# geobacter-rs/rav1e

Hardware: AMD Instinct MI355X
Metric: encoded frames/sec + Mpixels/sec, 4K 8-bit speed=10, 1/2/4/8 GPU vs host CPU (higher is better)
Workload: dtype u8

## Files before the change

### include/rav1e_hip.h

```cpp
#ifndef RAV1E_HIP_H
#define RAV1E_HIP_H

#include <stddef.h>
#include <stdint.h>

#ifdef __cplusplus
extern "C" {
#endif

#define RV_OK 0
#define RV_EINVAL (-1)
#define RV_EHIP (-2)
#define RV_ENOTSUP (-3)

typedef enum rv_cpu_feature_level {
  RV_CPU_NATIVE = 0,
  RV_CPU_SSE2 = 1,
  RV_CPU_SSSE3 = 2,
  RV_CPU_AVX2 = 3,
  RV_CPU_HIP = 4,
  RV_CPU_LEVELS = 5
} rv_cpu_feature_level;

int rv_cpu_feature_level_default(void);
// ... 293 lines not shown
} rv_fs_result;

typedef struct rv_mv_blk {
  int8_t ref[2];
  uint8_t n4_w, n4_h, newmv, pad[3];
  rv_mv mv[2];
} rv_mv_blk;
typedef struct rv_mv_cand {
  rv_mv this_mv, comp_mv;
  uint32_t weight;
} rv_mv_cand;
typedef struct rv_mvref_tile {
  int32_t cols, rows, mi_x, mi_y;
} rv_mvref_tile;
typedef struct rv_mvref_geom {
  int32_t n_tiles, grid_w, grid_h, frame_cols, frame_rows;
  uint32_t sign_bias;
} rv_mvref_geom;
typedef struct rv_mvref_query {
  int32_t tile, bx, by, bw4, bh4, ref[2], reserved;
} rv_mvref_query;
typedef struct rv_mvref_result {
  int32_t mode_context, n;
  rv_mv_cand stack[9];
} rv_mvref_result;
size_t rv_mvref_paint_scratch_bytes(rv_mvref_geom geom);
int rv_mvref_grid_paint(const rv_ec_mode_job *d_jobs, int n, rv_mvref_geom geom,
                        const rv_mvref_tile *d_tiles, rv_mv_blk *d_grid, void *d_scratch,
                        uint32_t *d_status, void *stream);
int rv_find_mvrefs_batch(const rv_mvref_query *d_queries, int n, rv_mvref_geom geom,
                         const rv_mvref_tile *d_tiles, const rv_mv_blk *d_grid,
                         rv_mvref_result *d_results, uint32_t *d_status, void *stream);
int rv_ec_mode_fill_stacks(rv_ec_mode_job *d_jobs, int n, rv_mvref_geom geom,
                           const rv_mvref_tile *d_tiles, const rv_mv_blk *d_grid,
                           rv_mvref_result *d_stacks, uint32_t *d_status, void *stream);

size_t rv_propagate_importances_scratch(int w_imp, int h_imp);
int rv_propagate_importances(const rv_plane *org, const rv_plane *ref, const rv_mv *d_mvs,
                             const uint32_t *d_intra_costs, const float *d_importances,
                             int n_unique, float *d_ref_importances, void *d_scratch,
                             size_t scratch_bytes, void *stream);
int rv_full_search_batch(const rv_plane *org, const rv_plane *ref,
                         const rv_fs_job *d_jobs, int n, int blk_w,
                         int blk_h, int step, int allow_hp,
                         rv_fs_result *d_out, void *stream);

int rv_plane_box_sums(const rv_plane *p, uint32_t *d_box, void *stream);

int rv_full_search_sea_batch(const rv_plane *org, const rv_plane *ref,
                             const uint32_t *d_ref_box, const rv_fs_job *d_jobs,
                             int n, int allow_hp, rv_fs_result *d_out,
                             void *stream);

#define RV_DS_MAX_PRED 17
#define RV_MAX_REFS 8
typedef struct rv_ds_job {
  int32_t po_x, po_y;
  int32_t mvx_min, mvx_max;
  int32_t mvy_min, mvy_max;
  rv_mv pmv[2];
  uint32_t lambda;
  int32_t n_pred;
  rv_mv pred[RV_DS_MAX_PRED];
} rv_ds_job;
int rv_diamond_search_batch(const rv_plane *org, const rv_plane *ref,
                            const rv_ds_job *d_jobs, int n, int blk_w,
                            int blk_h, int subpixel, int use_satd,
                            int allow_hp, int bit_depth,
                            rv_fs_result *d_out, void *stream);

int rv_telescopic_subpel_batch(const rv_plane *org, const rv_plane *ref,
                               const rv_ds_job *d_jobs,
                               const rv_fs_result *d_start, int n, int blk_w,
                               int blk_h, int use_satd, int allow_hp,
                               int bit_depth, rv_fs_result *d_out,
                               void *stream);

typedef struct rv_replay_cfg {
  int32_t width, height;
  int32_t xdec, ydec;
  int32_t bit_depth;
  int32_t tile_x0, tile_y0;
  int32_t tile_w, tile_h;
  int32_t n_refs;
  int32_t tile_w_sb, tile_h_sb;
  int32_t n_inputs;
  int32_t flags;
} rv_replay_cfg;
#define RV_REPLAY_EXHAUSTIVE_FS 4
#define RV_REPLAY_SPEED6 8
#define RV_REPLAY_DEBLOCK 16
#define RV_REPLAY_CDEF 32
#define RV_REPLAY_NO_INTRA 64
#define RV_REPLAY_ENTROPY 128
#define RV_REPLAY_MVREF_STANDIN 256
#define RV_REPLAY_LRF 512
typedef struct rv_replay_frame_info {
  int32_t display;
  int32_t me_range_scale;
  int32_t level;
  int32_t is_key;
  int32_t ref_display[2];
  int32_t compound;
} rv_replay_frame_info;
typedef struct rv_replay_level_params {
  int32_t base_q_idx;
  int32_t dc_delta_q[3];
  int32_t ac_delta_q[3];
  int32_t cdef_strengths;
  double lambda, me_lambda;
  double dist_scale[3];
} rv_replay_level_params;
typedef struct rv_replay rv_replay;
rv_replay *rv_replay_create(const rv_replay_cfg *cfg, void *stream);
void rv_replay_destroy(rv_replay *r);
rv_replay *rv_replay_create_twin(rv_replay *primary, void *stream);
int rv_replay_seek(rv_replay *r, long n);
void *rv_replay_stream(rv_replay *r);
int rv_replay_set_level_params(rv_replay *r, int level, const rv_replay_level_params *p);
int rv_replay_synth_inputs(rv_replay *r, int t0);
int rv_replay_set_input(rv_replay *r, int idx, const void *host_yuv);
int rv_replay_get_input(rv_replay *r, int idx, void *host_yuv);
int rv_replay_get_recon(rv_replay *r, int display, void *host_yuv);
int rv_replay_set_importances(rv_replay *r, const float *host, int n);
int rv_replay_set_imp_window(rv_replay *r, int window, long limit);
int rv_replay_set_inputs_ready(rv_replay *r, long displays);
typedef struct rv_la_hub rv_la_hub;
rv_la_hub *rv_la_hub_create(int n_groups);
void rv_la_hub_destroy(rv_la_hub *hub);
int rv_replay_set_la_exchange(rv_replay *r, void *comm, rv_la_hub *hub);
int rv_replay_get_importances(rv_replay *r, float *host, int n);
int rv_replay_frame(rv_replay *r, rv_replay_frame_info *info);
int rv_replay_set_groups(rv_replay *r, int n_groups, const int32_t *rects, int my_group,
                         void *comm);
int rv_replay_exchange_buffers(rv_replay *r, void **send, void **recv, size_t *bytes_per_group);
int rv_replay_import(rv_replay *r);
int rv_comm_unique_id(uint8_t *out, int cap);
void *rv_comm_create(const uint8_t *id, int nranks, int rank);
void rv_comm_destroy(void *comm);
int rv_replay_results(rv_replay *r, uint64_t *host_out, int cap);
int rv_replay_entropy_stats(rv_replay *r, uint64_t *out, int cap);
int rv_replay_set_timing(rv_replay *r, int stride, int block);
int rv_replay_stage_times(rv_replay *r, float *ms_out, int cap);
int rv_replay_stage_times_sum(rv_replay *r, int last_frames, float *ms_out,
                              int cap);
int rv_replay_set_kernel_probe(rv_replay *r, int on);
int rv_round_ring_slots(uint32_t q, int32_t *out, int cap);
int rv_replay_lrf_units(rv_replay *r, int plane, int8_t *out, int cap);
int rv_replay_la_refs(long m, int R, int32_t *out);
int rv_replay_kernel_probe(rv_replay *r, double *out, int cap);
int rv_ds_phase_dump(void);
int rv_rdo_phase_dump(void);
int rv_replay_counters(rv_replay *r, uint64_t *out, int cap);

int rv_replay_dpb_slots(void);


void rv_shims_release(void);
void rv_shims_shutdown(void);

#define RV_DIST_SIZES(X) \
  X(4, 4) X(4, 8) X(8, 4) X(8, 8) X(8, 16) X(16, 8) X(16, 16) X(16, 32) \
  X(32, 16) X(32, 32) X(32, 64) X(64, 32) X(64, 64) X(64, 128) X(128, 64) \
  X(128, 128) X(4, 16) X(16, 4) X(8, 32) X(32, 8) X(16, 64) X(64, 16)

#define RV_DECL_DIST(W, H)                                                   \
  uint32_t rav1e_sad##W##x##H##_hip(const uint8_t *src, ptrdiff_t src_stride, \
                                    const uint8_t *dst, ptrdiff_t dst_stride); \
  uint32_t rav1e_sad##W##x##H##_hbd_hip(const uint16_t *src,                  \
                                        ptrdiff_t src_stride,                 \
                                        const uint16_t *dst,                  \
                                        ptrdiff_t dst_stride);                \
  uint32_t rav1e_satd_##W##x##H##_hip(const uint8_t *src,                     \
                                      ptrdiff_t src_stride,                   \
                                      const uint8_t *dst,                     \
                                      ptrdiff_t dst_stride);                  \
  uint32_t rav1e_satd_##W##x##H##_hbd_hip(const uint16_t *src,                \
                                          ptrdiff_t src_stride,               \
                                          const uint16_t *dst,                \
                                          ptrdiff_t dst_stride);
RV_DIST_SIZES(RV_DECL_DIST)
#undef RV_DECL_DIST

#define RV_FILTER_PAIRS(X)                                                  \
  X(regular, regular, 0, 0) X(smooth, regular, 1, 0)                       \
  X(sharp, regular, 2, 0) X(bilinear, regular, 3, 0)                       \
  X(regular, smooth, 0, 1) X(smooth, smooth, 1, 1) X(sharp, smooth, 2, 1)  \
  X(bilinear, smooth, 3, 1) X(regular, sharp, 0, 2) X(smooth, sharp, 1, 2) \
  X(sharp, sharp, 2, 2) X(bilinear, sharp, 3, 2)                           \
  X(regular, bilinear, 0, 3) X(smooth, bilinear, 1, 3)                     \
  X(sharp, bilinear, 2, 3) X(bilinear, bilinear, 3, 3)

#define RV_DECL_MC(NX, NY, MX, MY)                                            \
  void rav1e_put_8tap_##NX##_##NY##_hip(                                      \
      uint8_t *dst, ptrdiff_t dst_stride, const uint8_t *src,                 \
      ptrdiff_t src_stride, int32_t w, int32_t h, int32_t mx, int32_t my);    \
  void rav1e_put_8tap_##NX##_##NY##_16bpc_hip(                                \
      uint16_t *dst, ptrdiff_t dst_stride, const uint16_t *src,               \
      ptrdiff_t src_stride, int32_t w, int32_t h, int32_t mx, int32_t my,     \
      int32_t bit_depth);                                                     \
  void rav1e_prep_8tap_##NX##_##NY##_hip(int16_t *tmp, const uint8_t *src,    \
                                         ptrdiff_t src_stride, int32_t w,     \
                                         int32_t h, int32_t mx, int32_t my);  \
  void rav1e_prep_8tap_##NX##_##NY##_16bpc_hip(                               \
      int16_t *tmp, const uint16_t *src, ptrdiff_t src_stride, int32_t w,     \
      int32_t h, int32_t mx, int32_t my, int32_t bit_depth);
RV_FILTER_PAIRS(RV_DECL_MC)
#undef RV_DECL_MC

void rav1e_avg_hip(uint8_t *dst, ptrdiff_t dst_stride, const int16_t *tmp1,
                   const int16_t *tmp2, int32_t w, int32_t h);
void rav1e_avg_16bpc_hip(uint16_t *dst, ptrdiff_t dst_stride,
                         const int16_t *tmp1, const int16_t *tmp2, int32_t w,
                         int32_t h, int32_t bit_depth);

int rav1e_fwd_txfm_hip(const int16_t *residual, int32_t *coeffs,
                       int32_t tx_size, int32_t tx_type, int32_t bit_depth);
int rav1e_inv_txfm_add_hip(const int32_t *coeffs, void *dst,
                           ptrdiff_t dst_stride, int32_t tx_size,
                           int32_t tx_type, int32_t bit_depth);

typedef uint32_t (*rv_dist_fn)(const void *src, ptrdiff_t src_stride,
                               const void *dst, ptrdiff_t dst_stride);
rv_dist_fn rv_sad_fn(int cpu_level, int bsize, int hbd);
rv_dist_fn rv_satd_fn(int cpu_level, int bsize, int hbd);
typedef void (*rv_put_fn)(void *dst, ptrdiff_t dst_stride, const void *src,
                          ptrdiff_t src_stride, int32_t w, int32_t h,
                          int32_t mx, int32_t my);
rv_put_fn rv_put_fn_get(int cpu_level, int mode_x, int mode_y);

#ifdef __cplusplus
}
#endif
#endif
```

### rav1e_amd/__init__.py

```python
from __future__ import annotations

import ctypes as C
import enum
import os

import numpy as np

_ROOT = os.path.dirname(os.path.abspath(__file__))
LIB_PATH = os.environ.get("RAV1E_HIP_LIB") or os.path.join(_ROOT, "lib", "librav1e_hip.so")
HEADER_PATH = os.path.join(os.path.dirname(_ROOT), "include", "rav1e_hip.h")

RV_OK, RV_EINVAL, RV_EHIP, RV_ENOTSUP = 0, -1, -2, -3


class Rav1eHipError(RuntimeError):
    pass


class RvPlane(C.Structure):
    _fields_ = [("data", C.c_void_p), ("stride", C.c_int32),
                ("alloc_height", C.c_int32), ("width", C.c_int32),
                ("height", C.c_int32), ("xorigin", C.c_int32),
                ("yorigin", C.c_int32), ("xdec", C.c_int32),
                ("ydec", C.c_int32), ("hbd", C.c_int32),
# ... 130 lines not shown
        return int(self.name.split("_")[1].split("X")[0])

    def height(self) -> int:
        return int(self.name.split("X")[-1])


class TxType(enum.IntEnum):
    DCT_DCT = 0
    ADST_DCT = 1
    DCT_ADST = 2
    ADST_ADST = 3
    FLIPADST_DCT = 4
    DCT_FLIPADST = 5
    FLIPADST_FLIPADST = 6
    ADST_FLIPADST = 7
    FLIPADST_ADST = 8
    IDTX = 9
    V_DCT = 10
    H_DCT = 11
    V_ADST = 12
    H_ADST = 13
    V_FLIPADST = 14
    H_FLIPADST = 15


class FilterMode(enum.IntEnum):
    REGULAR = 0
    SMOOTH = 1
    SHARP = 2
    BILINEAR = 3


_lib = None


class RvEcModeParams(C.Structure):
    _fields_ = [(n, C.c_int32) for n in ("frame_type", "reference_mode", "force_integer_mv",
                                         "allow_high_precision_mv", "seg_enabled",
                                         "last_active_segid")]


class RvMvrefGeom(C.Structure):
    _fields_ = [(n, C.c_int32) for n in ("n_tiles", "grid_w", "grid_h", "frame_cols",
                                         "frame_rows")] + [("sign_bias", C.c_uint32)]


def _declare(L):
    vp, i32, sz = C.c_void_p, C.c_int, C.c_size_t
    P = C.POINTER(RvPlane)
    sig = {
        "rv_cpu_feature_level_default": (i32, []),
        "rv_cpu_feature_level_index": (i32, [i32]),
        "rv_device_count": (i32, []),
        "rv_set_device": (i32, [i32]),
        "rv_last_error": (C.c_char_p, []),
        "rv_version": (C.c_char_p, []),
        "rv_malloc": (vp, [sz]),
        "rv_free": (None, [vp]),
        "rv_host_alloc": (vp, [sz]),
        "rv_host_free": (None, [vp]),
        "rv_memcpy_h2d": (i32, [vp, vp, sz, vp]),
        "rv_memcpy_d2h": (i32, [vp, vp, sz, vp]),
        "rv_memcpy_d2d": (i32, [vp, vp, sz, vp]),
        "rv_memset": (i32, [vp, i32, sz, vp]),
        "rv_stream_create": (vp, []),
        "rv_stream_create_priority": (vp, [i32]),
        "rv_stream_destroy": (i32, [vp]),
        "rv_stream_sync": (i32, [vp]),
        "rv_device_sync": (i32, []),
        "rv_trace_marker": (i32, [vp]),
        "rv_event_create": (vp, []),
        "rv_event_destroy": (i32, [vp]),
        "rv_event_record": (i32, [vp, vp]),
        "rv_event_sync": (i32, [vp]),
        "rv_stream_wait_event": (i32, [vp, vp]),
        "rv_event_elapsed_ms": (C.c_float, [vp, vp]),
        "rv_plane_geometry": (sz, [P, i32, i32, i32, i32, i32, i32, i32]),
        "rv_plane_pad": (i32, [P, vp]),
        "rv_plane_downsample": (i32, [P, P, vp]),
        "rv_sad_batch": (i32, [P, P, vp, i32, i32, i32, vp, vp]),
        "rv_satd_batch": (i32, [P, P, vp, i32, i32, i32, vp, vp]),
        "rv_sse_batch": (i32, [P, P, vp, i32, i32, i32, vp, vp]),
        "rv_lookahead_intra_costs": (i32, [P, i32, vp, vp]),
        "rv_propagate_importances_scratch": (sz, [i32, i32]),
        "rv_propagate_importances": (i32, [P, P, vp, vp, vp, i32, vp, vp, sz, vp]),
        "rv_cdef_moments_batch": (i32, [P, P, vp, i32, i32, i32, vp, vp]),
        "rv_put_8tap_batch": (i32, [P, P, vp, i32, i32, i32, i32, i32, i32, vp]),
        "rv_predict_intra_batch": (i32, [P, vp, vp, i32, i32, i32, vp]),
        "rv_intra_edges_batch": (i32, [P, vp, i32, vp, i32, i32, i32, i32, i32, vp, vp]),
        "rv_intra_screen_batch": (i32, [P, P, vp, i32, vp, i32, i32, i32, vp, i32, i32, vp, vp, vp,
                                        vp]),
        "rv_cfl_luma_ac_batch": (i32, [P, vp, i32, i32, i32, i32, vp, vp]),
        "rv_predict_cfl_batch": (i32, [P, vp, vp, vp, vp, i32, i32, i32, vp]),
        "rv_cfl_alpha_search_batch": (i32, [P, P, vp, i32, i32, i32, vp, vp, vp]),
        "rv_frame_delta_batch": (i32, [P, i32, i32, vp, i32, vp, vp]),
        "rv_deblock_plane": (i32, [P, i32, i32, i32, vp, vp, i32, vp, i32, vp]),
        "rv_deblock_fast_level": (i32, [i32, i32, i32]),
        "rv_deblock_sse": (i32, [P, P, i32, i32, vp, vp, i32, vp, vp, i32, vp]),
        "rv_deblock_frame": (i32, [P, i32, i32, vp, vp, i32, vp, i32, vp]),
        "rv_cdef_find_dirs": (i32, [P, i32, i32, vp, i32, vp, vp, i32, vp]),
        "rv_lrf_stripe_filter": (i32, [P, P] + [i32] * 10 + [vp, vp]),
        "rv_y4m_parse_header": (i32, [C.c_char_p, vp]),
        "rv_y4m_open": (vp, [C.c_char_p]),
        "rv_y4m_get_info": (i32, [vp, vp]),
        "rv_y4m_frame_bytes": (sz, [vp]),
        "rv_y4m_read_frame": (i32, [vp, vp]),
        "rv_y4m_close": (None, [vp]),
        "rv_ivf_create": (vp, [C.c_char_p, i32, i32, i32, i32]),
        "rv_ivf_write_frame": (i32, [vp, C.c_uint64, vp, sz]),
        "rv_ivf_close": (i32, [vp]),
        "rv_cdef_filter_plane": (i32, [P, P, i32, i32, i32, vp, i32, vp, vp, vp, vp, vp, i32, i32,
                                       vp]),
        "rv_prep_8tap_batch": (i32, [vp, P, vp, i32, i32, i32, i32, i32, i32, vp]),
        "rv_mc_avg_batch": (i32, [P, vp, vp, vp, i32, i32, i32, i32, vp]),
        "rv_mc_dist_batch": (i32, [P, P, vp, i32, i32, i32, i32, i32, i32, i32, vp, vp]),
        "rv_fwd_txfm_batch": (i32, [vp, vp, i32, i32, i32, i32, vp]),
        "rv_diff_fwd_txfm_batch": (i32, [P, P, vp, i32, i32, i32, i32, vp, vp]),
        "rv_inv_txfm_add_batch": (i32, [vp, P, vp, i32, i32, i32, i32, vp]),
        "rv_quantize_batch": (i32, [vp, i32, i32, i32, i32, i32, i32, i32, i32, i32, vp, vp, vp,
                                    vp]),
        "rv_dequantize_batch": (i32, [vp, i32, i32, i32, i32, i32, i32, vp, vp]),
        "rv_estimate_rate_batch": (i32, [vp, i32, i32, i32, vp, vp]),
        "rv_full_search_batch": (i32, [P, P, vp, i32, i32, i32, i32, i32, vp, vp]),
        "rv_full_search_sea_batch": (i32, [P, P, vp, vp, i32, i32, vp, vp]),
        "rv_plane_box_sums": (i32, [P, vp, vp]),
        "rv_replay_create": (vp, [C.POINTER(RvReplayCfg), vp]),
        "rv_replay_create_twin": (vp, [vp, vp]),
        "rv_replay_seek": (i32, [vp, C.c_long]),
        "rv_replay_stream": (vp, [vp]),
        "rv_replay_destroy": (None, [vp]),
        "rv_q_lookup": (i32, [i32, i32, i32]),
        "rv_replay_synth_inputs": (i32, [vp, i32]),
        "rv_replay_set_level_params": (i32, [vp, i32, C.POINTER(RvReplayLevelParams)]),
        "rv_replay_set_input": (i32, [vp, i32, vp]),
        "rv_replay_get_input": (i32, [vp, i32, vp]),
        "rv_replay_get_recon": (i32, [vp, i32, vp]),
        "rv_replay_set_importances": (i32, [vp, vp, i32]),
        "rv_replay_set_imp_window": (i32, [vp, i32, C.c_long]),
        "rv_replay_set_inputs_ready": (i32, [vp, C.c_long]),
        "rv_replay_get_importances": (i32, [vp, vp, i32]),
        "rv_replay_frame": (i32, [vp, C.POINTER(RvReplayFrameInfo)]),
        "rv_replay_set_groups": (i32, [vp, i32, vp, i32, vp]),
        "rv_replay_exchange_buffers": (i32, [vp, C.POINTER(C.c_void_p), C.POINTER(C.c_void_p),
                                             C.POINTER(C.c_size_t)]),
        "rv_replay_import": (i32, [vp]),
        "rv_comm_unique_id": (i32, [vp, i32]),
        "rv_comm_create": (vp, [vp, i32, i32]),
        "rv_comm_destroy": (None, [vp]),
        "rv_replay_results": (i32, [vp, vp, i32]),
        "rv_replay_entropy_stats": (i32, [vp, vp, i32]),
        "rv_replay_stage_times": (i32, [vp, vp, i32]),
        "rv_replay_stage_times_sum": (i32, [vp, i32, vp, i32]),
        "rv_replay_counters": (i32, [vp, vp, i32]),
        "rv_replay_dpb_slots": (i32, []),
        "rv_replay_set_kernel_probe": (i32, [vp, i32]),
        "rv_replay_kernel_probe": (i32, [vp, vp, i32]),
        "rv_round_ring_slots": (i32, [C.c_uint32, vp, i32]),
        "rv_replay_lrf_units": (i32, [vp, i32, vp, i32]),
        "rv_replay_la_refs": (i32, [C.c_long, i32, vp]),
        "rv_la_hub_create": (vp, [i32]),
        "rv_la_hub_destroy": (None, [vp]),
        "rv_replay_set_la_exchange": (i32, [vp, vp, vp]),
        "rv_replay_set_timing": (i32, [vp, i32, i32]),
        "rv_diamond_search_batch": (i32, [P, P, vp, i32, i32, i32, i32, i32, i32, i32, vp, vp]),
        "rv_telescopic_subpel_batch": (i32, [P, P, vp, vp, i32, i32, i32, i32, i32, i32, vp, vp]),
        "rv_tx_dist_batch": (i32, [vp, i32, vp, i32, i32, vp, vp]),
        "rav1e_fwd_txfm_hip": (i32, [vp, vp, i32, i32, i32]),
        "rav1e_inv_txfm_add_hip": (i32, [vp, vp, C.c_ssize_t, i32, i32, i32]),
        "rv_ec_scratch_bytes": (C.c_size_t, [i32]),
        "rv_ec_tokenize": (i32, [vp, i32, i32, i32, i32, i32, i32, vp, vp, vp, vp, C.c_uint32, vp,
                                 vp]),
        "rv_ec_code_tokens": (C.c_long, [vp, C.c_size_t, vp, vp, C.c_size_t]),
        "rv_ec_count_tokens": (C.c_long, [vp, C.c_size_t, vp, vp]),
        "rv_ec_rate_batch": (i32, [vp, vp, vp, i32, vp, i32, vp, vp, vp, vp, vp]),
        "rv_ec_cdf_total": (i32, []),
        "rv_ec_default_cdf": (i32, [i32, vp]),
        "rv_ec_reset_counts": (None, [vp]),
        "rv_ec_mode_scratch_bytes": (C.c_size_t, [i32]),
        "rv_ec_mode_tokenize": (i32, [vp, i32, RvEcModeParams, i32, vp, i32, i32, vp, vp, vp, vp,
                                      C.c_uint32, vp, vp]),
        "rv_ec_code_stream": (C.c_long, [vp, C.c_size_t, vp, vp, C.c_size_t]),
        "rv_ec_count_stream": (C.c_long, [vp, C.c_size_t, vp, vp]),
        "rv_ec_cdf_total_all": (i32, []),
        "rv_ec_default_cdf_all": (i32, [i32, vp]),
        "rv_ec_reset_counts_all": (None, [vp]),
        "rv_ec_partition_gather": (i32, [vp, i32]),
        "rv_ec_rate_stream_batch": (i32, [vp, vp, vp, i32, vp, i32, vp, vp, vp, vp, vp]),
        "rv_ec_rate_stream_batch_waves": (i32, [vp, vp, vp, i32, vp, i32, vp, vp, vp, vp, i32, vp]),
        "rv_ec_cand_scratch_bytes": (C.c_size_t, [i32, i32]),
        "rv_ec_cand_tokenize": (i32, [vp, i32, vp, i32, vp, i32, RvEcModeParams, i32, vp, i32, i32,
                                      i32, i32, vp, i32, i32, vp, vp, vp, vp, C.c_uint32, vp, vp]),
        "rv_ec_cand_rates": (i32, [vp, i32, vp, i32, vp, i32, RvEcModeParams, i32, vp, i32, i32,
                                   i32, i32, vp, i32, i32, vp, vp, vp, vp, C.c_uint32, vp, i32, vp,
                                   vp, vp, vp, vp]),
        "rv_mvref_paint_scratch_bytes": (C.c_size_t, [RvMvrefGeom]),
        "rv_mvref_grid_paint": (i32, [vp, i32, RvMvrefGeom, vp, vp, vp, vp, vp]),
        "rv_find_mvrefs_batch": (i32, [vp, i32, RvMvrefGeom, vp, vp, vp, vp, vp]),
        "rv_ec_mode_fill_stacks": (i32, [vp, i32, RvMvrefGeom, vp, vp, vp, vp, vp]),
        "rv_sad_fn": (vp, [i32, i32, i32]),
        "rv_satd_fn": (vp, [i32, i32, i32]),
        "rv_put_fn_get": (vp, [i32, i32, i32]),
    }
    for name, (res, args) in sig.items():
        f = getattr(L, name)
        f.restype = res
        f.argtypes = args


def lib():
    global _lib
    if _lib is None:
        if not os.path.exists(LIB_PATH):
            raise Rav1eHipError(
                f"{LIB_PATH} missing: run `python -c 'import __graft_entry__ as g; g.build()'`")
        L = C.CDLL(LIB_PATH, mode=C.RTLD_GLOBAL)
        _declare(L)
        _lib = L
    return _lib


def _check(rc, what):
    if rc != RV_OK:
        raise Rav1eHipError(f"{what} failed ({rc}): {lib().rv_last_error().decode()}")


def require_device(device: int = 0):
    L = lib()
    if L.rv_device_count() <= device:
        raise Rav1eHipError("no HIP device visible: the HIP level needs a gfx950 GPU")
    _check(L.rv_set_device(device), "rv_set_device")


class DeviceBuffer:

    def __init__(self, nbytes: int):
        self.nbytes = int(nbytes)
        self.ptr = lib().rv_malloc(max(1, self.nbytes))
        if not self.ptr:
            raise Rav1eHipError(f"rv_malloc({nbytes}): {lib().rv_last_error().decode()}")

    @classmethod
    def from_array(cls, a: np.ndarray) -> "DeviceBuffer":
        a = np.ascontiguousarray(a)
        b = cls(a.nbytes)
        b.upload(a)
        return b

    def upload(self, a: np.ndarray, stream=None):
        a = np.ascontiguousarray(a)
        assert a.nbytes <= self.nbytes
        if a.nbytes:
            _check(lib().rv_memcpy_h2d(self.ptr, a.ctypes.data, a.nbytes, stream), "rv_memcpy_h2d")

    def download(self, dtype, count=None, stream=None) -> np.ndarray:
        dt = np.dtype(dtype)
        n = self.nbytes // dt.itemsize if count is None else int(count)
        out = np.empty(n, dtype=dt)
        if out.nbytes:
            _check(lib().rv_memcpy_d2h(out.ctypes.data, self.ptr, out.nbytes, stream),
                   "rv_memcpy_d2h")
        return out

    def zero(self, stream=None):
        _check(lib().rv_memset(self.ptr, 0, self.nbytes, stream), "rv_memset")
        _check(lib().rv_stream_sync(stream), "rv_stream_sync")

    def free(self):
        if self.ptr:
            lib().rv_free(self.ptr)
            self.ptr = None

    def __del__(self):
        try:
            self.free()
        except Exception:
            pass


class DevicePlane:

    def __init__(self, width, height, xdec=0, ydec=0, xpad=0, ypad=0, hbd=False,
                 bit_depth=None):
        self.desc = RvPlane()
        nbytes = lib().rv_plane_geometry(C.byref(self.desc), width, height, xdec, ydec,
                                         xpad, ypad, 1 if hbd else 0)
        if bit_depth is not None:
            self.desc.bit_depth = int(bit_depth)
        self.buf = DeviceBuffer(nbytes)
        self.desc.data = self.buf.ptr
        self.dtype = np.uint16 if hbd else np.uint8

    @classmethod
    def from_array(cls, a: np.ndarray, xpad=0, ypad=0, xdec=0, ydec=0, pad=True,
                   bit_depth=None):
        p = cls(a.shape[1], a.shape[0], xdec, ydec, xpad, ypad, a.dtype == np.uint16,
                bit_depth)
        p.upload_visible(a, pad=pad)
        return p

    @classmethod
    def from_full(cls, full: np.ndarray, xorigin, yorigin, width, height, bit_depth=None):
        p = cls.__new__(cls)
        p.desc = RvPlane()
        p.desc.stride, p.desc.alloc_height = full.shape[1], full.shape[0]
        p.desc.width, p.desc.height = width, height
        p.desc.xorigin, p.desc.yorigin = xorigin, yorigin
# ... 1846 lines not shown
```

### rav1e_amd/csrc/rv_rdo.h

```cpp
#pragma once

#include "rv_chain.h"
#include "rv_device.h"
#include "rv_quant.h"

namespace rv {

struct RdoPlane {
  rv_plane org;
  rv_plane ref[2];
  rv_plane dst;
  int32_t *levels;
  uint64_t *out;
  QCtx q;
};

struct RdoWinner {
  int32_t c;
  int32_t skip;
  double cost;
  uint64_t dist;
};

struct RdoArgs {
  RdoPlane p[2];
  CandGeo g;
  const rv_fs_result *sub;
  const RdoWinner *win;
  const float *imp;
  int w_in_b, h_in_b, w_imp;
  int n_tx;
  int cand_base;
  const int32_t *list;
  const int32_t *count;
  int commit;
  int ntx_per_cand;
  int bd;
  int bsize;
  int mb_w, mb_h;
  int sub_w, sub_h;
  int xdec, ydec;
  int q_tx_index;
  int tx_size, qindex;
  const void *iedges;
  const uint8_t *imodes;
  const uint8_t *iwin;
};

}

int rv_quant_ctx(int qindex, int tx_area, int is_intra, int bit_depth, int dc_delta_q,
                 int ac_delta_q, rv::QCtx *out);

int rv_rdo_candidates(const rv::RdoArgs &luma, const rv::RdoArgs &chroma, int hbd,
                      hipStream_t s, bool compound = false);

int rv_rdo_blocks2(const rv::RdoArgs &l, const rv::RdoArgs &c, int nl, int nc, int hbd,
                   hipStream_t s, int mode);
int rv_rdo_blocks(const rv::RdoArgs &a, bool luma, int nplanes, int n_tx_size, int hbd,
                  hipStream_t s, int mode);

int rv_rdo_args_put(const rv::RdoArgs *h, int n, rv::RdoArgs *dev, hipStream_t s);
int rv_rdo_candidates_list(const rv::RdoArgs *h, const rv::RdoArgs *dev, int nsets, int mode_a,
                           int hbd, hipStream_t s, int max_grid = 0, uint32_t *kp_cnt = nullptr,
                           unsigned long long *kp_t = nullptr);

int rv_rdo_intra(const rv::RdoArgs &luma, const rv::RdoArgs &chroma, int hbd, hipStream_t s);
```

### rav1e_amd/csrc/rv_rdo.hip

```cpp
#include <stdio.h>
#include <stdlib.h>
#include <string.h>

#include <type_traits>

#include "rv_distortion.h"
#include "rv_intra.h"
#include "rv_rdo.h"
#include "rv_tx.h"

namespace rv {


__constant__ int8_t kRdoReg[2][16][8] = {
    {{0, 0, 0, 127, 0, 0, 0, 0}, {0, 2, -6, 126, 8, -2, 0, 0},
     {0, 2, -10, 122, 18, -4, 0, 0}, {0, 2, -12, 116, 28, -8, 2, 0},
     {0, 2, -14, 110, 38, -10, 2, 0}, {0, 2, -14, 102, 48, -12, 2, 0},
     {0, 2, -16, 94, 58, -12, 2, 0}, {0, 2, -14, 84, 66, -12, 2, 0},
     {0, 2, -14, 76, 76, -14, 2, 0}, {0, 2, -12, 66, 84, -14, 2, 0},
     {0, 2, -12, 58, 94, -16, 2, 0}, {0, 2, -12, 48, 102, -14, 2, 0},
     {0, 2, -10, 38, 110, -14, 2, 0}, {0, 2, -8, 28, 116, -12, 2, 0},
     {0, 0, -4, 18, 122, -10, 2, 0}, {0, 0, -2, 8, 126, -6, 2, 0}},
    {{0, 0, 0, 127, 0, 0, 0, 0}, {0, 0, -4, 126, 8, -2, 0, 0},
     {0, 0, -8, 122, 18, -4, 0, 0}, {0, 0, -10, 116, 28, -6, 0, 0},
// ... 59 lines not shown
    mode = (kc & 1) ? 0 : a.imodes[sb * 4 + 1 + (kc >> 1)];
    j.oi = sb * 6 + kc;
  }
  const int sx = sb % a.g.tw, sy = sb / a.g.tw;
  const int fx = a.g.tx0 + sx, fy = a.g.ty0 + sy;
  const int tsx = fx % a.g.tws, tsy = fy % a.g.ths;
  j.ivar = tsx == 0 && tsy == 0 ? 0 : tsy == 0 ? 1 : tsx == 0 ? 2 : 3;
  j.imode = mode;
  j.iedge = (const uint8_t *)a.iedges + ((size_t)sb * 3 + plane) * kIntraEdge * sizeof(Px);
  j.bx = (fx * a.bsize) >> a.xdec;
  j.by = (fy * a.bsize) >> a.ydec;
  j.ox = j.oy = 0;
  j.src_x = j.src_y = j.cf = j.rf = j.ref = 0;
  j.src2_x = j.src2_y = j.cf2 = j.rf2 = 0;
  j.comp = false;
  j.zero = false;
  return j;
}

template <typename Px, int N, int G>
__device__ __forceinline__ void intra_fill(const RdoJob &jb, int32_t *e, Px *pred, int bd, int lane) {
  const Px *eg = (const Px *)jb.iedge;
  for (int i = lane; i < kIntraEdge; i += G) e[i] = eg[i];
  wave_sync();
  IntraSetup st = intra_setup(jb.imode, jb.ivar);
  if (st.mode == 0) st.dcv = intra_dc<G>(e, jb.ivar, N, N, bd, lane);
  const int maxv = (1 << bd) - 1;
  for (int i = lane; i < N * N; i += G) {
    const int r = i / N, c = i - r * N;
    pred[i] = (Px)intra_px(st, e, N, N, r, c, maxv);
  }
  wave_sync();
}

__device__ __forceinline__ int rdo_ntx(const RdoArgs &a) {
  return a.count ? __builtin_amdgcn_readfirstlane(*a.count) * a.ntx_per_cand : a.n_tx;
}

template <int N>
__device__ __forceinline__ RdoJob rdo_job(const RdoArgs &a, const RdoPlane &pl, int t) {
  const int ci = t / a.ntx_per_cand, sub = t - ci * a.ntx_per_cand;
  const int cand = a.list ? a.list[ci] : a.cand_base + ci;
  int sb, c;
  RdoJob j;
  j.zero = false;
  j.oi = cand * a.ntx_per_cand + sub;
  if (a.commit) {
    sb = cand;
    c = a.win[sb].c;
    j.zero = a.win[sb].skip != 0;
  } else {
    c = cand / a.g.nsb;
    sb = cand - c * a.g.nsb;
  }
  rv_mv mv, mv1{0, 0};
  j.comp = c >= a.g.R * a.g.M;
  if (j.comp) {
    comp_mvs(a.g, a.sub, sb, c - a.g.R * a.g.M, &mv, &mv1);
    j.ref = 0;
  } else {
    (void)cand_mv(a.g, a.sub, sb, c, &mv);
    j.ref = c / a.g.M;
  }
  const int sx = sb % a.g.tw, sy = sb / a.g.tw;
  j.bx = ((a.g.tx0 + sx) * a.bsize) >> a.xdec;
  j.by = ((a.g.ty0 + sy) * a.bsize) >> a.ydec;
  const int txc = a.mb_w / N;
  j.ox = (sub % txc) * N;
  j.oy = (sub / txc) * N;
  const rv_mc_job m = mc_job_for(pl.ref[j.ref], j.bx, j.by, mv, 0, 0);
  j.src_x = m.src_x;
  j.src_y = m.src_y;
  j.cf = m.col_frac;
  j.rf = m.row_frac;
  j.src2_x = j.src2_y = j.cf2 = j.rf2 = 0;
  if (j.comp) {
    const rv_mc_job m1 = mc_job_for(pl.ref[1], j.bx, j.by, mv1, 0, 0);
    j.src2_x = m1.src_x;
    j.src2_y = m1.src_y;
    j.cf2 = m1.col_frac;
    j.rf2 = m1.row_frac;
  }
  return j;
}

struct McF {
  uint32_t xp[3];
  int xsum;
  int yt[8];
  int cf, rf;
};
template <typename Px>
__device__ __forceinline__ McF mc_setup(int cf, int rf, int w, int h) {
  McF f;
  f.cf = cf;
  f.rf = rf;
  const int8_t *xf = kRdoReg[w <= 4][cf];
  const int8_t *yf = kRdoReg[h <= 4][rf];
#pragma unroll
  for (int k = 0; k < 8; k++) f.yt[k] = yf[k];
  f.xsum = 0;
  if constexpr (sizeof(Px) == 1) {
#pragma unroll
    for (int q = 0; q < 2; q++)
      f.xp[q] = (uint32_t)(uint8_t)xf[4 * q] | ((uint32_t)(uint8_t)xf[4 * q + 1] << 8) |
                ((uint32_t)(uint8_t)xf[4 * q + 2] << 16) | ((uint32_t)(uint8_t)xf[4 * q + 3] << 24);
#pragma unroll
    for (int k = 0; k < 8; k++) f.xsum += xf[k];
    f.xp[2] = 0;
  } else {
#pragma unroll
    for (int q = 0; q < 3; q++)
      f.xp[q] = (uint32_t)(uint16_t)(int16_t)xf[2 * q + 1] |
                ((uint32_t)(uint16_t)(int16_t)xf[2 * q + 2] << 16);
  }
  return f;
}
template <typename Px>
__device__ __forceinline__ int32_t mc_h(const McF &f, const uint32_t *row, int col, int ib) {
  if constexpr (sizeof(Px) == 1) {
    const int d0 = col >> 2, sh = col & 3;
    const uint32_t w0 = row[d0], w1 = row[d0 + 1], w2 = row[d0 + 2];
    const uint32_t lo = __builtin_amdgcn_alignbyte(w1, w0, sh);
    const uint32_t hi = __builtin_amdgcn_alignbyte(w2, w1, sh);
    if (!f.cf) return (int32_t)((lo >> 24) ^ 0x80u);
    int32_t s = dot4_i8(lo, f.xp[0], 128 * f.xsum);
    s = dot4_i8(hi, f.xp[1], s);
    return (int32_t)(int16_t)round_shift(s, 7 - ib);
  } else {
    const int c1 = col + 1, d0 = c1 >> 1, sh = (c1 & 1) * 2;
    uint32_t w[4];
#pragma unroll
    for (int k = 0; k < 4; k++) w[k] = row[d0 + k];
    uint32_t pp[3];
#pragma unroll
    for (int k = 0; k < 3; k++) pp[k] = __builtin_amdgcn_alignbyte(w[k + 1], w[k], sh);
    if (!f.cf) return (int32_t)(pp[1] & 0xffffu);
    int32_t s = 0;
#pragma unroll
    for (int k = 0; k < 3; k++) s = dot2_i16(pp[k], f.xp[k], s);
    return (int32_t)(int16_t)round_shift(s, 7 - ib);
  }
}
__device__ __forceinline__ int32_t mc_prep_v(const McF &f, const int32_t *ring, int u, int ib) {
  if (f.rf) {
    int32_t s = 0;
#pragma unroll
    for (int k = 1; k < 7; k++) s += __mul24(f.yt[k], ring[(u + k) & 7]);
    return round_shift(s, f.cf ? 7 : 7 - ib);
  }
  return f.cf ? ring[(u + 3) & 7] : ring[(u + 3) & 7] << ib;
}

template <typename Px, int N, int RB>
__device__ __forceinline__ void mc_compound(const RdoArgs &a, const RdoPlane &pl, const RdoJob &jb,
                                            uint32_t *win, Px *pred) {
  constexpr int B = (int)sizeof(Px);
  constexpr int P = B == 1 ? ((N + 8 + 15) / 16) * 16 : ((2 * (N + 8) + 15) / 16) * 16;
  constexpr int kRowDw = ((N + 7) * B + 3) / 4, kTot = (RB + 7) * kRowDw;
  static_assert((RB % 8 == 0 || RB < 8) && N % RB == 0, "bands of whole 8-row groups");
  constexpr int U = RB < 8 ? RB : 8;
  const int col = rv_tid() & (N - 1);
  const int ib = a.bd == 12 ? 2 : 4, maxv = (1 << a.bd) - 1;
  const McF f0 = mc_setup<Px>(jb.cf, jb.rf, a.mb_w, a.mb_h);
  const McF f1 = mc_setup<Px>(jb.cf2, jb.rf2, a.mb_w, a.mb_h);
  uint32_t *w0 = win, *w1 = win + (RB + 7) * (P / 4);
  const uint8_t *sp0 = (const uint8_t *)plane_ptr<Px>(pl.ref[0], jb.src_x + jb.ox - 3, jb.src_y + jb.oy - 3);
  const uint8_t *sp1 =
      (const uint8_t *)plane_ptr<Px>(pl.ref[1], jb.src2_x + jb.ox - 3, jb.src2_y + jb.oy - 3);
  const int64_t rs0 = (int64_t)pl.ref[0].stride * B, rs1 = (int64_t)pl.ref[1].stride * B;
#pragma unroll 1
  for (int band = 0; band < N / RB; band++) {
    if (band) wave_sync();
#pragma unroll 2
    for (int i = col; i < kTot; i += N) {
      const int r = i / kRowDw, d = i - r * kRowDw;
      uint32_t v0, v1;
      __builtin_memcpy(&v0, sp0 + (band * RB + r) * rs0 + 4 * d, 4);
      __builtin_memcpy(&v1, sp1 + (band * RB + r) * rs1 + 4 * d, 4);
      w0[r * (P / 4) + d] = B == 1 ? v0 ^ 0x80808080u : v0;
      w1[r * (P / 4) + d] = B == 1 ? v1 ^ 0x80808080u : v1;
    }
    wave_sync();
    int32_t g0[8], g1[8];
#pragma unroll
    for (int k = 1; k < 6; k++) {
      g0[k] = mc_h<Px>(f0, w0 + k * (P / 4), col, ib);
      g1[k] = mc_h<Px>(f1, w1 + k * (P / 4), col, ib);
    }
    g0[0] = g0[6] = g0[7] = g1[0] = g1[6] = g1[7] = 0;
#pragma unroll 1
    for (int r0 = 0; r0 < RB; r0 += U) {
#pragma unroll
      for (int u = 0; u < U; u++) {
        const int r = r0 + u;
        g0[(u + 6) & 7] = mc_h<Px>(f0, w0 + (r + 6) * (P / 4), col, ib);
        g1[(u + 6) & 7] = mc_h<Px>(f1, w1 + (r + 6) * (P / 4), col, ib);
        const int32_t t = mc_prep_v(f0, g0, u, ib) + mc_prep_v(f1, g1, u, ib);
        pred[(band * RB + r) * N + col] = (Px)clamp_med3(round_shift(t, ib + 1), 0, maxv);
      }
    }
  }
  wave_sync();
}

__device__ __forceinline__ double rdo_bias(const RdoArgs &a, int mi_x, int mi_y, int m = 2) {
  return distortion_bias(a.imp, a.w_imp, a.w_in_b, a.h_in_b, mi_x, mi_y, m);
}

template <typename Px>
__device__ __forceinline__ uint64_t rdo_cdef_8x8(const Px *o, int64_t os, const Px *d, int dp,
                                                 int bd) {
  int32_t ss = 0, sd = 0;
  uint32_t ss2 = 0, sd2 = 0, ssd = 0;
#pragma unroll
  for (int j = 0; j < 8; j++)
#pragma unroll
    for (int i = 0; i < 8; i++) {
      const int32_t s = o[(int64_t)j * os + i];
      const int32_t e = d[j * dp + i];
      ss += s;
      sd += e;
      ss2 += (uint32_t)wmul24(s, s);
      sd2 += (uint32_t)wmul24(e, e);
      ssd += (uint32_t)wmul24(s, e);
    }
  return cdef_dist_finish(ss, sd, ss2, sd2, ssd, bd);
}

template <typename Px, int N, int LPB>
__device__ __forceinline__ uint64_t rdo_sse_biased(const RdoArgs &a, const RdoJob &j, const Px *o,
                                                   int64_t os, const Px *d) {
  const int bw = a.sub_w, bh = a.sub_h, nbx = N / bw, nby = N / bh;
  const int lane = rv_tid() & (LPB - 1);
  uint64_t acc = 0;
  for (int k = lane; k < nbx * nby; k += LPB) {
    const int by = k / nbx, bx = k - by * nbx;
    uint64_t value = 0;
    for (int jj = 0; jj < bh; jj++) {
      uint32_t row = 0;
      for (int i = 0; i < bw; i++) {
        const int32_t c = (int32_t)(int16_t)o[(int64_t)(by * bh + jj) * os + bx * bw + i] -
                          (int32_t)(int16_t)d[(by * bh + jj) * N + bx * bw + i];
        row += (uint32_t)wmul24(c, c);
      }
      value += row;
    }
    const int px = j.bx + j.ox + bx * bw, py = j.by + j.oy + by * bh;
    acc += distortion_biased(
        value, rdo_bias(a, (px << a.xdec) >> 2, (py << a.ydec) >> 2, (N < 8 ? N : 8) / 4));
  }
  return acc;
}

template <typename Px, int N, int LPB, bool LUMA>
__device__ __forceinline__ uint64_t rdo_dist_biased(const RdoArgs &a, const RdoJob &j, const Px *o,
                                                    int64_t os, const Px *d) {
  if constexpr (LUMA) {
    constexpr int NB = N / 8, ROWS = NB * NB * 8;
    static_assert(LPB % 8 == 0 && ROWS % LPB == 0, "rows of 8x8 blocks over the lanes");
    const int lane = rv_tid() & (LPB - 1);
    uint64_t acc = 0;
#pragma unroll
    for (int k0 = 0; k0 < ROWS; k0 += LPB) {
      const int k = k0 + lane, blk = k >> 3, row = k & 7;
      const int by = blk / NB, bx = blk - by * NB;
      const Px *op = o + (int64_t)(by * 8 + row) * os + bx * 8;
      const Px *dp = d + (by * 8 + row) * N + bx * 8;
      int32_t ss = 0, sd = 0;
      uint32_t ss2 = 0, sd2 = 0, ssd = 0;
#pragma unroll
      for (int i = 0; i < 8; i++) {
        const int32_t sv = op[i], e = dp[i];
        ss += sv;
        sd += e;
        ss2 += (uint32_t)wmul24(sv, sv);
        sd2 += (uint32_t)wmul24(e, e);
        ssd += (uint32_t)wmul24(sv, e);
      }
#pragma unroll
      for (int m = 1; m < 8; m <<= 1) {
        ss += __shfl_xor(ss, m, 64);
        sd += __shfl_xor(sd, m, 64);
        ss2 += __shfl_xor(ss2, m, 64);
        sd2 += __shfl_xor(sd2, m, 64);
        ssd += __shfl_xor(ssd, m, 64);
      }
      if (row == 0) {
        const uint64_t v = cdef_dist_finish(ss, sd, ss2, sd2, ssd, a.bd);
        const int px = j.bx + j.ox + bx * 8, py = j.by + j.oy + by * 8;
        acc += distortion_biased(v, rdo_bias(a, px >> 2, py >> 2));
      }
    }
    return acc;
  } else {
    return rdo_sse_biased<Px, N, LPB>(a, j, o, os, d);
  }
}

template <typename Px, int N>
__host__ __device__ constexpr int rdo_slab_bytes() {
  constexpr int B = (int)sizeof(Px);
  constexpr int P = B == 1 ? ((N + 8 + 15) / 16) * 16 : ((2 * (N + 8) + 15) / 16) * 16;
  constexpr int RB = N < 16 ? N : 16;
  constexpr int a = N * (N + 1) * 4, b = (N + 7) * P, c = 2 * (RB + 7) * P;
  return ((a > b ? a : b) > c ? (a > b ? a : b) : c);
}

template <typename Px, int N, int LPB, int MODE, bool LUMA = false>
__device__ __forceinline__ void rdo_cand_body(const RdoArgs &a, const RdoPlane &pl, int t,
                                              bool valid, int32_t *buf, Px *pred,
                                              const uint16_t *scan) {
  constexpr int B = (int)sizeof(Px);
  constexpr int S = N + 1;
  constexpr int G = LPB / N, RG = N / G;
  constexpr int U = RG < 8 ? RG : 8;
  constexpr int P = B == 1 ? ((N + 8 + 15) / 16) * 16 : ((2 * (N + 8) + 15) / 16) * 16;
  constexpr int C32 = N < 32 ? N : 32;
  static_assert(!LUMA || N >= 8, "cdef distortion runs on 8x8 blocks");
  const int lane = rv_tid() & (LPB - 1);
  RdoJob jb;
  if constexpr (MODE == 3)
    jb = rdo_job_intra<Px, N>(a, &pl == &a.p[1] ? 2 : 1, t);
  else
    jb = rdo_job<N>(a, pl, t);
  const rv_plane &ref = pl.ref[jb.ref];
  const int ox = jb.ox, oy = jb.oy;
  const int bd = a.bd, ib = bd == 12 ? 2 : 4, maxv = (1 << bd) - 1;
  const int sx0 = jb.bx + ox, sy0 = jb.by + oy;
  auto wave_sync = [] {
    __builtin_amdgcn_fence(__ATOMIC_RELEASE, "wavefront");
    __builtin_amdgcn_wave_barrier();
    __builtin_amdgcn_fence(__ATOMIC_ACQUIRE, "wavefront");
  };

  if constexpr (MODE == 3) {
    intra_fill<Px, N, LPB>(jb, buf, pred, a.bd, lane);
  } else if (MODE == 1 || (MODE == 2 && jb.comp)) {
    static_assert(2 * (16 + 7) * (sizeof(Px) == 1 ? 48 : 80) <= N * (N + 1) * 4 || N != 32,
                  "compound windows must fit the coefficient slab");
    mc_compound<Px, N, (N < 16 ? N : 16)>(a, pl, jb, reinterpret_cast<uint32_t *>(buf), pred);
  } else
  {
    uint32_t *win = reinterpret_cast<uint32_t *>(buf);
    const uint8_t *sp = (const uint8_t *)plane_ptr<Px>(ref, jb.src_x + ox - 3, jb.src_y + oy - 3);
    const int64_t rs = (int64_t)ref.stride * B;
    constexpr int kRowDw = ((N + 7) * B + 3) / 4;
    constexpr int kTot = (N + 7) * kRowDw;
#pragma unroll 4
    for (int i = lane; i < kTot; i += LPB) {
      const int r = i / kRowDw, d = i - r * kRowDw;
      uint32_t v;
// ... 77 lines not shown
      }
    }
    wave_sync();
  }
  const Px *o = plane_ptr<Px>(pl.org, sx0, sy0);
  const int64_t ost = pl.org.stride;
  if (!a.commit) {
    const uint64_t d = group_sum<LPB>(rdo_dist_biased<Px, N, LPB, LUMA>(a, jb, o, ost, pred));
    if (valid && lane == 0) pl.out[(int64_t)jb.oi * 3 + 0] = d;
  }

  int s0, s1, s2;
  fwd_shifts<N>((bd - 8) / 2, s0, s1, s2);
  {
    constexpr int PPD = 4 / B;
    constexpr int DPR = N / PPD;
    const uint8_t *op = (const uint8_t *)o;
    const int64_t os = (int64_t)pl.org.stride * B;
#pragma unroll 8
    for (int i = lane; i < N * DPR; i += LPB) {
      const int r = i / DPR, c = (i - r * DPR) * PPD;
      uint32_t ov, pv;
      __builtin_memcpy(&ov, op + r * os + c * B, 4);
      __builtin_memcpy(&pv, pred + r * N + c, 4);
#pragma unroll
      for (int k = 0; k < PPD; k++) {
        const int sh = 8 * B * k, m = B == 1 ? 0xff : 0xffff;
        const int16_t d = (int16_t)((int16_t)((ov >> sh) & m) - (int16_t)((pv >> sh) & m));
        buf[r * S + c + k] = rdo_rsa((int32_t)d, -s0);
      }
    }
    wave_sync();
  }
  if (lane < N) {
    int32_t v[N];
#pragma unroll
    for (int r = 0; r < N; r++) v[r] = buf[r * S + lane];
    tx::fwd1d<1, N>(v, v);
#pragma unroll
    for (int r = 0; r < N; r++) buf[r * S + lane] = rdo_rsa(v[r], -s1);
  }
  wave_sync();
  constexpr int CA = C32 * C32, RR = CA / N;
  if (lane < RR) {
    int32_t v[N];
#pragma unroll
    for (int c = 0; c < N; c++) v[c] = buf[lane * S + c];
    tx::fwd1d<1, N>(v, v);
#pragma unroll
    for (int c = 0; c < N; c++) buf[lane * S + c] = rdo_rsa(v[c], -s2);
  }
  wave_sync();
  uint64_t txd = 0;
  quantize_block<CA, LPB>(
      pl.q, scan, [&](int pos) { return buf[(pos / N) * S + (pos % N)]; },
      [&](int pos, int32_t q, int32_t r) {
        int32_t *e = buf + (pos / N) * S + (pos % N);
        const int32_t dd = wsub(*e, r);
        txd += (uint64_t)(int64_t)wmul(dd, dd);
        *e = jb.zero ? 0 : q;
      });
  wave_sync();
  if (!a.commit) {
    txd = group_sum<LPB>(txd);
    const int bits = 2 * (3 - pl.q.log_tx_scale);
    if (valid && lane == 0)
      pl.out[(int64_t)jb.oi * 3 + 2] =
          q_estimate_rate(a.qindex, a.tx_size, (txd + (1ull << (bits - 1))) >> bits);
  }
  {
    int32_t *pk = pl.levels + (int64_t)jb.oi * CA;
#pragma unroll 4
    for (int i = lane; i < CA; i += LPB) {
      int32_t *e = buf + (i / N) * S + (i % N);
      const int32_t q = *e;
      if (valid && a.commit) pk[i] = q;
      *e = q_dequant(pl.q, q, i);
    }
  }
  wave_sync();
  const int range = bd + 8;
  {
    int32_t v[N];
    if (lane < C32) {
#pragma unroll
      for (int c = 0; c < N; c++) {
        const int i = lane * C32 + c;
        v[c] = c < C32 ? tx::clampv(buf[(i / N) * S + (i % N)], range) : 0;
      }
    }
    wave_sync();
    if (lane < C32) {
      tx::inv1d<1, N>(v, range);
#pragma unroll
      for (int c = 0; c < N; c++) buf[lane * S + c] = v[c];
    }
  }
  wave_sync();
  if (lane < N) {
    const int crange = bd + 6 > 16 ? bd + 6 : 16;
    int32_t v[N];
#pragma unroll
    for (int r = 0; r < N; r++)
      v[r] = r < C32 ? tx::clampv(round_shift(buf[r * S + lane], inv_mid_shift<N>()), crange) : 0;
    tx::inv1d<1, N>(v, crange);
#pragma unroll
    for (int r = 0; r < N; r++) {
      Px *q = pred + r * N + lane;
      *q = (Px)clamp_med3(wadd((int32_t)*q, round_shift(v[r], 4)), 0, maxv);
    }
  }
  wave_sync();
  if (a.commit) {
    constexpr int PPD = 4 / B, DPR = N / PPD;
    uint8_t *dp = (uint8_t *)plane_ptr_mut<Px>(pl.dst, sx0, sy0);
    const int64_t ds = (int64_t)pl.dst.stride * B;
#pragma unroll 8
    for (int i = lane; i < N * DPR; i += LPB) {
      const int r = i / DPR, c = (i - r * DPR) * PPD;
      uint32_t v;
      __builtin_memcpy(&v, pred + r * N + c, 4);
      if (valid) __builtin_memcpy(dp + r * ds + c * B, &v, 4);
    }
    return;
  }
  const uint64_t d = group_sum<LPB>(rdo_dist_biased<Px, N, LPB, LUMA>(a, jb, o, ost, pred));
  if (valid && lane == 0) pl.out[(int64_t)jb.oi * 3 + 1] = d;
}

__host__ __device__ constexpr int cmax(int a, int b) { return a > b ? a : b; }

template <typename Px, typename Mid, int NPART>
struct LumaLds {
  static constexpr int kWinP = sizeof(Px) == 1 ? 80 : 144;
  static constexpr int kWinRows = 64 / NPART + 7;
  static constexpr int kCompRows = sizeof(Px) == 1 ? 16 : 8;
  static constexpr int kScr =
      cmax(cmax(cmax(kWinRows * kWinP, 16 * 65 * 4), 32 * 66 * (int)sizeof(Mid)),
           2 * (kCompRows + 7) * kWinP);
  static constexpr int kSlot = (kScr + 64 * 64 * (int)sizeof(Px) + 15) / 16 * 16;
};


template <typename Px>
__device__ __forceinline__ uint64_t luma_dist(const RdoArgs &a, const RdoJob &j, const Px *o,
                                              int64_t os, const Px *pred) {
  const int lane = rv_tid() & 63, by = lane >> 3, bx = lane & 7;
  const uint64_t v =
      rdo_cdef_8x8<Px>(o + (int64_t)(by * 8) * os + bx * 8, os, pred + by * 8 * 64 + bx * 8, 64, a.bd);
  const int px = j.bx + bx * 8, py = j.by + by * 8;
  return group_sum<64>(distortion_biased(v, rdo_bias(a, px >> 2, py >> 2)));
}

template <typename Px, int NPART, int MODE>
__device__ __forceinline__ void luma_front(const RdoArgs &a, const RdoPlane &pl, int t,
                                           const RdoJob &jb, bool valid, uint8_t *scr, Px *pred,
                                           bool skip_dist = true) {
  constexpr int N = 64, B = (int)sizeof(Px);
  constexpr int P = LumaLds<Px, int16_t, NPART>::kWinP;
  constexpr int RP = N / NPART;
  static_assert(RP % 8 == 0, "MC rows run in groups of 8");
  const int lane = rv_tid() & 63;
  const rv_plane &ref = pl.ref[jb.ref];
  const int ox = 0, oy = 0;
  const int bd = a.bd, ib = bd == 12 ? 2 : 4, maxv = (1 << bd) - 1;

  if constexpr (MODE == 3) {
    intra_fill<Px, 64, 64>(jb, reinterpret_cast<int32_t *>(scr), pred, bd, lane);
  } else if (MODE == 1 || (MODE == 2 && jb.comp)) {
    mc_compound<Px, 64, LumaLds<Px, int16_t, NPART>::kCompRows>(
        a, pl, jb, reinterpret_cast<uint32_t *>(scr), pred);
  } else
  {
    uint32_t *win = reinterpret_cast<uint32_t *>(scr);
    const int cf = jb.cf, rf = jb.rf;
    const int8_t *xf = kRdoReg[a.mb_w <= 4][cf];
    const int8_t *yf = kRdoReg[a.mb_h <= 4][rf];
    int yt[8];
#pragma unroll
    for (int k = 0; k < 8; k++) yt[k] = yf[k];
    uint32_t xp[4];
    int xsum = 0;
    if constexpr (B == 1) {
#pragma unroll
      for (int h = 0; h < 2; h++)
        xp[h] = (uint32_t)(uint8_t)xf[4 * h] | ((uint32_t)(uint8_t)xf[4 * h + 1] << 8) |
                ((uint32_t)(uint8_t)xf[4 * h + 2] << 16) | ((uint32_t)(uint8_t)xf[4 * h + 3] << 24);
#pragma unroll
      for (int k = 0; k < 8; k++) xsum += xf[k];
      xp[2] = xp[3] = 0;
    } else {
#pragma unroll
      for (int h = 0; h < 3; h++)
        xp[h] = (uint32_t)(uint16_t)(int16_t)xf[2 * h + 1] |
                ((uint32_t)(uint16_t)(int16_t)xf[2 * h + 2] << 16);
      xp[3] = 0;
    }
    const int col = lane;
    auto hval = [&](int tr) __attribute__((always_inline)) -> int32_t {
      const uint32_t *row = win + tr * (P / 4);
      if constexpr (B == 1) {
        const int d0 = col >> 2, sh = col & 3;
        const uint32_t w0 = row[d0], w1 = row[d0 + 1], w2 = row[d0 + 2];
        const uint32_t lo = __builtin_amdgcn_alignbyte(w1, w0, sh);
        const uint32_t hi = __builtin_amdgcn_alignbyte(w2, w1, sh);
        if (!cf) return (int32_t)((lo >> 24) ^ 0x80u);
        int32_t s = dot4_i8(lo, xp[0], 128 * xsum);
        s = dot4_i8(hi, xp[1], s);
        return (int32_t)(int16_t)round_shift(s, 7 - ib);
      } else {
        const int c1 = col + 1, d0 = c1 >> 1, sh = (c1 & 1) * 2;
        uint32_t w[4];
#pragma unroll
        for (int k = 0; k < 4; k++) w[k] = row[d0 + k];
        uint32_t pp[3];
#pragma unroll
        for (int k = 0; k < 3; k++) pp[k] = __builtin_amdgcn_alignbyte(w[k + 1], w[k], sh);
        if (!cf) return (int32_t)(pp[1] & 0xffffu);
        int32_t s = 0;
#pragma unroll
        for (int k = 0; k < 3; k++)
          s = dot2_i16(pp[k], xp[k], s);
        return (int32_t)(int16_t)round_shift(s, 7 - ib);
      }
    };
    const int vshift = cf ? 7 + ib : 7;
    constexpr int kRowDw = ((N + 7) * B + 3) / 4;
    constexpr int kTot = (RP + 7) * kRowDw;
    const int64_t rs = (int64_t)ref.stride * B;
#pragma unroll 1
    for (int half = 0; half < NPART; half++) {
      const uint8_t *sp =
          (const uint8_t *)plane_ptr<Px>(ref, jb.src_x + ox - 3, jb.src_y + oy - 3 + RP * half);
      if (half) wave_sync();
#pragma unroll 4
      for (int i = lane; i < kTot; i += 64) {
        const int r = i / kRowDw, d = i - r * kRowDw;
        uint32_t v;
        __builtin_memcpy(&v, sp + r * rs + 4 * d, 4);
        win[r * (P / 4) + d] = B == 1 ? v ^ 0x80808080u : v;
      }
      wave_sync();
      int32_t ring[8];
#pragma unroll
      for (int k = 1; k < 6; k++) ring[k] = hval(k);
      ring[0] = ring[6] = ring[7] = 0;
#pragma unroll 1
      for (int r0 = 0; r0 < RP; r0 += 8) {
#pragma unroll
        for (int u = 0; u < 8; u++) {
          const int r = r0 + u;
          ring[(u + 6) & 7] = hval(r + 6);
          int32_t v;
          if (rf) {
            int32_t s = 0;
#pragma unroll
            for (int k = 1; k < 7; k++) s += __mul24(yt[k], ring[(u + k) & 7]);
            v = round_shift(s, vshift);
          } else {
            v = cf ? round_shift(ring[(u + 3) & 7], ib) : ring[(u + 3) & 7];
          }
          pred[(RP * half + r) * N + col] = (Px)clamp_med3(v, 0, maxv);
        }
      }
    }
    wave_sync();
  }

  const Px *o = plane_ptr<Px>(pl.org, jb.bx, jb.by);
  if (!a.commit && skip_dist) {
    const uint64_t d = luma_dist<Px>(a, jb, o, pl.org.stride, pred);
    if (valid && lane == 0) pl.out[(int64_t)jb.oi * 3 + 0] = d;
  }
  int s0, s1, s2;
  fwd_shifts<N>((bd - 8) / 2, s0, s1, s2);
  int32_t *fmid = reinterpret_cast<int32_t *>(scr);
  {
    int32_t v[N];
#pragma unroll
    for (int r = 0; r < N; r++) {
      const int16_t d = (int16_t)((int16_t)o[(int64_t)r * pl.org.stride + lane] -
                                  (int16_t)pred[r * N + lane]);
      v[r] = rdo_rsa((int32_t)d, -s0);
    }
    tx::fwd1d<1, N>(v, v);
#pragma unroll
    for (int r = 0; r < 16; r++) fmid[r * 65 + lane] = rdo_rsa(v[r], -s1);
  }
}

__device__ __forceinline__ void luma_fwd_row(int32_t *row, int bd) {
  int s0, s1, s2;
  fwd_shifts<64>((bd - 8) / 2, s0, s1, s2);
  int32_t v[64];
#pragma unroll
  for (int c = 0; c < 64; c++) v[c] = row[c];
  tx::fwd1d<1, 64>(v, v);
#pragma unroll
  for (int c = 0; c < 64; c++) row[c] = rdo_rsa(v[c], -s2);
}

__device__ __forceinline__ void luma_quantize(const RdoArgs &a, const RdoPlane &pl, int t,
                                              const RdoJob &jb, bool valid, int32_t *fmid,
                                              const uint16_t *scan) {
  uint64_t txd = 0;
  quantize_block<1024, 64>(
      pl.q, scan, [&](int pos) { return fmid[(pos >> 6) * 65 + (pos & 63)]; },
      [&](int pos, int32_t q, int32_t r) {
        int32_t *e = fmid + (pos >> 6) * 65 + (pos & 63);
        const int32_t dd = wsub(*e, r);
        txd += (uint64_t)(int64_t)wmul(dd, dd);
        *e = jb.zero ? 0 : q;
      });
  const int lane = rv_tid() & 63;
  if (!a.commit) {
    txd = group_sum<64>(txd);
    const int bits = 2 * (3 - pl.q.log_tx_scale);
    if (valid && lane == 0)
      pl.out[(int64_t)jb.oi * 3 + 2] =
          q_estimate_rate(a.qindex, a.tx_size, (txd + (1ull << (bits - 1))) >> bits);
  }
  wave_sync();
  int32_t *pk = pl.levels + (int64_t)jb.oi * 1024;
#pragma unroll 4
  for (int i = lane; i < 1024; i += 64) {
    int32_t *e = fmid + (i >> 6) * 65 + (i & 63);
    const int32_t q = *e;
    if (a.commit) pk[i] = q;
    *e = q_dequant(pl.q, q, i);
  }
}

__device__ __forceinline__ void luma_inv_row_load(const int32_t *fmid, int rr, int32_t *v,
                                                  int range, int32_t *pk) {
  const int32_t *src = fmid + (rr >> 1) * 65 + (rr & 1) * 32;
#pragma unroll
  for (int c = 0; c < 32; c++) {
    const int32_t x = src[c];
    if (pk) pk[c] = x;
    v[c] = tx::clampv(x, range);
  }
#pragma unroll
  for (int c = 32; c < 64; c++) v[c] = 0;
}
template <typename Mid>
__device__ __forceinline__ void luma_inv_row_tx(int32_t *v, Mid *dst, int range, int crange) {
  tx::inv1d<1, 64>(v, range);
#pragma unroll
  for (int c = 0; c < 64; c++) dst[c] = (Mid)tx::clampv(round_shift(v[c], 2), crange);
}

template <typename Px, typename Mid>
__device__ __forceinline__ void luma_back(const RdoArgs &a, const RdoPlane &pl, int t,
                                          const RdoJob &jb, bool valid, const Mid *imid,
                                          Px *pred) {
  constexpr int N = 64, B = (int)sizeof(Px);
  const int lane = rv_tid() & 63;
  const int bd = a.bd, maxv = (1 << bd) - 1;
  const int crange = bd + 6 > 16 ? bd + 6 : 16;
  {
    int32_t v[N];
#pragma unroll
    for (int r = 0; r < N; r++) v[r] = r < 32 ? (int32_t)imid[r * 66 + lane] : 0;
    tx::inv1d<1, N>(v, crange);
#pragma unroll
    for (int r = 0; r < N; r++) {
      Px *q = pred + r * N + lane;
      *q = (Px)clamp_med3(wadd((int32_t)*q, round_shift(v[r], 4)), 0, maxv);
    }
  }
  wave_sync();
  if (a.commit) {
    constexpr int PPD = 4 / B, DPR = N / PPD;
    uint8_t *dp = (uint8_t *)plane_ptr_mut<Px>(pl.dst, jb.bx, jb.by);
    const int64_t ds = (int64_t)pl.dst.stride * B;
#pragma unroll 8
    for (int i = lane; i < N * DPR; i += 64) {
      const int r = i / DPR, c = (i - r * DPR) * PPD;
      uint32_t v;
      __builtin_memcpy(&v, pred + r * N + c, 4);
      if (valid) __builtin_memcpy(dp + r * ds + c * B, &v, 4);
    }
    return;
  }
  const uint64_t d = luma_dist<Px>(a, jb, plane_ptr<Px>(pl.org, jb.bx, jb.by), pl.org.stride, pred);
  if (valid && lane == 0) pl.out[(int64_t)jb.oi * 3 + 1] = d;
}

template <typename Px, typename Mid, int NPART, int MODE>
__device__ __forceinline__ void rdo_luma_body(const RdoArgs &a, const RdoPlane &pl, int t,
                                              uint8_t *scr, Px *pred, const uint16_t *scan) {
  const int lane = rv_tid() & 63;
  RdoJob jb;
  if constexpr (MODE == 3)
    jb = rdo_job_intra<Px, 64>(a, 0, t);
  else
    jb = rdo_job<64>(a, pl, t);
  luma_front<Px, NPART, MODE>(a, pl, t, jb, true, scr, pred);
  wave_sync();
  int32_t *fmid = reinterpret_cast<int32_t *>(scr);
  if (lane < 16) luma_fwd_row(fmid + lane * 65, a.bd);
  wave_sync();
  luma_quantize(a, pl, t, jb, true, fmid, scan);
  wave_sync();
  const int range = a.bd + 8, crange = a.bd + 6 > 16 ? a.bd + 6 : 16;
  Mid *imid = reinterpret_cast<Mid *>(scr);
  {
    int32_t v[64];
    if (lane < 32) luma_inv_row_load(fmid, lane, v, range, nullptr);
    wave_sync();
    if (lane < 32) luma_inv_row_tx(v, imid + lane * 66, range, crange);
  }
  wave_sync();
  luma_back<Px, Mid>(a, pl, t, jb, true, imid, pred);
}

template <typename Px, int MODE>
__device__ __forceinline__ void rdo_chroma_pair(const RdoArgs &chroma, int b, int32_t *buf,
                                                Px *pred, const uint16_t *scan, int pairs = -1) {
  if (pairs < 0) pairs = (chroma.n_tx + 1) / 2;
  const int plane = b / pairs;
  const int half = (rv_tid() & 63) >> 5;
  const int n = rdo_ntx(chroma);
  int i = 2 * (b - plane * pairs) + half;
  if (i - half >= n) return;
  const bool valid = i < n;
  if (!valid) i -= 1;
  rdo_cand_body<Px, 32, 32, MODE>(chroma, chroma.p[plane], i, valid, buf + half * 32 * 33,
                            pred + half * 32 * 32, scan);
}

__device__ __forceinline__ void stage_scan(uint16_t *dst, int tx_index) {
  const uint16_t *src = RV_SCANS + RV_SCAN_OFF[tx_index];
  for (int i = rv_tid(); i < 1024; i += blockDim.x) dst[i] = src[i];
  __syncthreads();
}

template <typename Px>
using SingleLds = LumaLds<Px, typename std::conditional<sizeof(Px) == 1, int16_t, int32_t>::type, 2>;
constexpr int kChromaPair(int pxb) { return 2 * 32 * 33 * 4 + 2 * 32 * 32 * pxb; }

template <typename Px, int MODE>
__global__ __launch_bounds__(64) __attribute__((amdgpu_waves_per_eu(4))) void rdo_frame_kernel(
    RdoArgs luma, RdoArgs chroma) {
  using L = SingleLds<Px>;
  using Mid = typename std::conditional<sizeof(Px) == 1, int16_t, int32_t>::type;
  __shared__ __align__(16) uint8_t lds[cmax(L::kSlot, kChromaPair(sizeof(Px)))];
  __shared__ uint16_t scan[1024];
  const int b = blockIdx.x;
  stage_scan(scan, b < luma.n_tx ? luma.q_tx_index : chroma.q_tx_index);
  if (b < luma.n_tx && b >= rdo_ntx(luma)) return;
  if (b < luma.n_tx)
    rdo_luma_body<Px, Mid, 2, MODE>(luma, luma.p[0], b, lds,
                              reinterpret_cast<Px *>(lds + L::kScr), scan);
  else
    rdo_chroma_pair<Px, MODE>(chroma, b - luma.n_tx, reinterpret_cast<int32_t *>(lds),
                        reinterpret_cast<Px *>(lds + 2 * 32 * 33 * 4), scan);
}

template <typename Px>
struct QuadLds {
  using L = LumaLds<Px, int16_t, sizeof(Px) == 1 ? 2 : 4>;
  static constexpr int kBytes = cmax(4 * L::kSlot, 3 * kChromaPair(sizeof(Px)));
};

#ifndef RV_RDO_PHASES
#define RV_RDO_PHASES 0
#endif
__device__ unsigned long long g_rdo_ph[3][8];
struct QuadPh {
  unsigned long long t[5];
};

template <typename Px, int MODE>
__device__ __forceinline__ void rdo_quad_luma(const RdoArgs &luma, int b, int n, int var,
                                              uint8_t *lds, const uint16_t *scan,
                                              QuadPh *ph = nullptr) {
  using L = typename QuadLds<Px>::L;
  constexpr int NPART = sizeof(Px) == 1 ? 2 : 4;
  const int wave = __builtin_amdgcn_readfirstlane(rv_tid() >> 6), lane = rv_tid() & 63;
  auto slot = [&](int q) __attribute__((always_inline)) { return lds + q * L::kSlot; };
  auto fmid = [&](int q) __attribute__((always_inline)) {
    return reinterpret_cast<int32_t *>(slot(q));
  };
  auto imid = [&](int q) __attribute__((always_inline)) {
    return reinterpret_cast<int16_t *>(slot(q));
  };
  auto pred = [&](int q) __attribute__((always_inline)) {
    return reinterpret_cast<Px *>(slot(q) + L::kScr);
  };
  const int t0 = 4 * b, t = t0 + wave;
  if (t0 >= n) return;
  const bool valid = t < n;
  RdoJob jb;
  if constexpr (MODE == 3)
    jb = rdo_job_intra<Px, 64>(luma, 0, valid ? t : n - 1);
  else
    jb = rdo_job<64>(luma, luma.p[0], valid ? t : n - 1);
  const bool late_dist = (var & 1) && !luma.commit;
  const bool prio = (var & 2) != 0;
  if (valid)
    luma_front<Px, NPART, MODE>(luma, luma.p[0], t, jb, true, slot(wave), pred(wave), !late_dist);
  __syncthreads();
  if (RV_RDO_PHASES && ph) ph->t[1] = wall_clock64();
  if (wave == 0) {
    if (prio) __builtin_amdgcn_s_setprio(2);
    const int q = lane >> 4;
    if (t0 + q < n) luma_fwd_row(fmid(q) + (lane & 15) * 65, luma.bd);
    if (prio) __builtin_amdgcn_s_setprio(0);
  } else if (late_dist && valid) {
    const uint64_t d = luma_dist<Px>(luma, jb, plane_ptr<Px>(luma.p[0].org, jb.bx, jb.by),
                                     luma.p[0].org.stride, pred(wave));
    if (lane == 0) luma.p[0].out[(int64_t)jb.oi * 3 + 0] = d;
  }
  __syncthreads();
  if (RV_RDO_PHASES && ph) ph->t[2] = wall_clock64();
  if (valid) luma_quantize(luma, luma.p[0], t, jb, true, fmid(wave), scan);
  __syncthreads();
  if (RV_RDO_PHASES && ph) ph->t[3] = wall_clock64();
  if (wave < 2) {
    if (prio) __builtin_amdgcn_s_setprio(2);
    const int q = 2 * wave + (lane >> 5), rr = lane & 31;
    const bool vq = t0 + q < n;
    const int range = luma.bd + 8, crange = luma.bd + 6 > 16 ? luma.bd + 6 : 16;
    int32_t v[64];
    if (vq) luma_inv_row_load(fmid(q), rr, v, range, nullptr);
    wave_sync();
    if (vq) luma_inv_row_tx(v, imid(q) + rr * 66, range, crange);
    if (prio) __builtin_amdgcn_s_setprio(0);
  } else if (wave == 2 && late_dist) {
    RdoJob j0;
    if constexpr (MODE == 3)
      j0 = rdo_job_intra<Px, 64>(luma, 0, t0);
    else
      j0 = rdo_job<64>(luma, luma.p[0], t0);
    const uint64_t d = luma_dist<Px>(luma, j0, plane_ptr<Px>(luma.p[0].org, j0.bx, j0.by),
                                     luma.p[0].org.stride, pred(0));
    if (lane == 0) luma.p[0].out[(int64_t)j0.oi * 3 + 0] = d;
  }
  __syncthreads();
  if (RV_RDO_PHASES && ph) ph->t[4] = wall_clock64();
  if (valid) luma_back<Px, int16_t>(luma, luma.p[0], t, jb, true, imid(wave), pred(wave));
}

template <typename Px, int MODE>
__device__ __forceinline__ void rdo_quad_chroma(const RdoArgs &chroma, int c, int pairs,
                                                uint8_t *lds, const uint16_t *scan) {
  const int wave = __builtin_amdgcn_readfirstlane(rv_tid() >> 6);
  const int pair = 3 * c + wave;
  if (wave == 3 || pair >= 2 * pairs) return;
  uint8_t *w = lds + wave * kChromaPair(sizeof(Px));
  rdo_chroma_pair<Px, MODE>(chroma, pair, reinterpret_cast<int32_t *>(w),
                            reinterpret_cast<Px *>(w + 2 * 32 * 33 * 4), scan, pairs);
}

template <typename Px, int MODE>
__device__ __forceinline__ void rdo_quad_chroma4(const RdoArgs &chroma, int c, int n, uint8_t *lds,
                                                 const uint16_t *scan) {
  constexpr int kSlab = rdo_slab_bytes<Px, 32>();
  static_assert(4 * (kSlab + 32 * 32 * (int)sizeof(Px)) <= QuadLds<Px>::kBytes, "4 chroma slabs");
  const int wave = __builtin_amdgcn_readfirstlane(rv_tid() >> 6);
  const int k = 4 * c + wave;
  if (k >= 2 * n) return;
  const int plane = k >= n ? 1 : 0, i = k - plane * n;
  uint8_t *w = lds + wave * (kSlab + 32 * 32 * (int)sizeof(Px));
  rdo_cand_body<Px, 32, 64, MODE>(chroma, chroma.p[plane], i, true, reinterpret_cast<int32_t *>(w),
                                  reinterpret_cast<Px *>(w + kSlab), scan);
}

template <typename Px, int MODE>
__device__ __forceinline__ void rdo_quad_wg(RdoArgs luma, RdoArgs chroma, int nquads,
                                            int var, int b, uint8_t *lds, uint16_t *scan) {
  if (b >= nquads) {
    const int pairs = (chroma.n_tx + 1) / 2, nc = rdo_ntx(chroma);
    bool any = false;
    for (int w = 0; w < 3; w++) {
      const int p = 3 * (b - nquads) + w;
      if (p < 2 * pairs) any |= 2 * (p - (p / pairs) * pairs) < nc;
    }
    if (!any) return;
  } else if (4 * b >= rdo_ntx(luma)) {
    return;
  }
  stage_scan(scan, b >= nquads ? chroma.q_tx_index : luma.q_tx_index);
  if (b >= nquads)
    rdo_quad_chroma<Px, MODE>(chroma, b - nquads, (chroma.n_tx + 1) / 2, lds, scan);
  else
    rdo_quad_luma<Px, MODE>(luma, b, rdo_ntx(luma), var, lds, scan);
}

template <typename Px, int MODE>
__global__ __launch_bounds__(256) __attribute__((amdgpu_waves_per_eu(4))) void rdo_quad_kernel(
    RdoArgs luma, RdoArgs chroma, int nquads, int var) {
  __shared__ __align__(16) uint8_t lds[QuadLds<Px>::kBytes];
  __shared__ uint16_t scan[1024];
  rdo_quad_wg<Px, MODE>(luma, chroma, nquads, var, blockIdx.x, lds, scan);
}

template <typename Px, int MA, int MB>
__global__ __launch_bounds__(256) __attribute__((amdgpu_waves_per_eu(4))) void rdo_quad_list_kernel(
    const RdoArgs *__restrict__ A, int nsets, int var, uint32_t *kp_cnt, unsigned long long *kp_t) {
  __shared__ __align__(16) uint8_t lds[QuadLds<Px>::kBytes];
  __shared__ uint16_t scan[1024];
  if (kp_t && threadIdx.x == 0) atomicMin(kp_t, (unsigned long long)wall_clock64());
  const RdoArgs &la = A[0], &ca = A[1], &lb = A[2], &cb = A[3];
  const int na = rdo_ntx(la), ma = rdo_ntx(ca);
  const int nb = nsets > 1 ? rdo_ntx(lb) : 0, mb = nsets > 1 ? rdo_ntx(cb) : 0;
  if (kp_cnt && blockIdx.x == 0 && threadIdx.x == 0) {
    atomicAdd(kp_cnt + (MA ? 1 : 0), (uint32_t)na);
    atomicAdd(kp_cnt + (MA ? 3 : 2), (uint32_t)ma);
    if (nsets > 1) {
      atomicAdd(kp_cnt + (MB ? 1 : 0), (uint32_t)nb);
      atomicAdd(kp_cnt + (MB ? 3 : 2), (uint32_t)mb);
    }
  }
  const int pa = (ma + 1) / 2, pb = (mb + 1) / 2;
  const bool c4 = (var & 32) != 0;
  const int e0 = (na + 3) / 4, e1 = e0 + (c4 ? (2 * ma + 3) / 4 : (2 * pa + 2) / 3);
  const int e2 = e1 + (nb + 3) / 4, e3 = e2 + (c4 ? (2 * mb + 3) / 4 : (2 * pb + 2) / 3);
  const bool phd = RV_RDO_PHASES && (var & 16) && rv_tid() == 0;
  for (int b = blockIdx.x; b < e3; b += gridDim.x) {
    QuadPh ph;
    ph.t[0] = phd ? wall_clock64() : 0;
    QuadPh *pp = phd ? &ph : nullptr;
    int set = 2;
    if (b < e0) {
      stage_scan(scan, la.q_tx_index);
      rdo_quad_luma<Px, MA>(la, b, na, var, lds, scan, pp);
      set = MA;
    } else if (b < e1) {
      stage_scan(scan, ca.q_tx_index);
      if (c4)
        rdo_quad_chroma4<Px, MA>(ca, b - e0, ma, lds, scan);
      else
        rdo_quad_chroma<Px, MA>(ca, b - e0, pa, lds, scan);
    } else if (b < e2) {
      stage_scan(scan, lb.q_tx_index);
      rdo_quad_luma<Px, MB>(lb, b - e1, nb, var, lds, scan, pp);
      set = MB;
    } else {
      stage_scan(scan, cb.q_tx_index);
      if (c4)
        rdo_quad_chroma4<Px, MB>(cb, b - e2, mb, lds, scan);
      else
        rdo_quad_chroma<Px, MB>(cb, b - e2, pb, lds, scan);
    }
    __syncthreads();
    if (phd) {
      const unsigned long long te = wall_clock64();
      if (set < 2) {
        for (int k = 0; k < 4; k++) atomicAdd(&g_rdo_ph[set][k], ph.t[k + 1] - ph.t[k]);
        atomicAdd(&g_rdo_ph[set][4], te - ph.t[4]);
      } else {
        atomicAdd(&g_rdo_ph[2][0], te - ph.t[0]);
      }
      atomicAdd(&g_rdo_ph[set][5], 1ull);
    }
  }
  if (kp_t && threadIdx.x == 0) atomicMax(kp_t + 1, (unsigned long long)wall_clock64());
}

__global__ __launch_bounds__(256) void rdo_args_store_kernel(RdoArgs a0, RdoArgs a1, RdoArgs a2,
                                                              RdoArgs a3, int n, RdoArgs *out) {
  static_assert(sizeof(RdoArgs) % 4 == 0, "word copy");
  constexpr int W = (int)(sizeof(RdoArgs) / 4);
  for (int i = threadIdx.x; i < n * W; i += blockDim.x) {
    const int k = i / W, w = i - k * W;
    const RdoArgs *s = k == 0 ? &a0 : k == 1 ? &a1 : k == 2 ? &a2 : &a3;
    uint32_t v;
    __builtin_memcpy(&v, reinterpret_cast<const uint8_t *>(s) + 4 * w, 4);
    __builtin_memcpy(reinterpret_cast<uint8_t *>(out + k) + 4 * w, &v, 4);
  }
}

constexpr unsigned kF4Pool = 1024;
constexpr int kRdoVariant = 3;

}

using namespace rv;

template <typename Px, int N, int MODE, bool LUMA>
__global__ __launch_bounds__(256) void rdo_small_kernel(RdoArgs a, int nplanes) {
  constexpr int TPW = 64 / N;
  constexpr int SLAB = rdo_slab_bytes<Px, N>();
  constexpr int PER = (SLAB + N * N * (int)sizeof(Px) + 15) / 16 * 16;
  __shared__ __align__(16) uint8_t lds[4 * TPW * PER];
  __shared__ uint16_t scan[1024];
  stage_scan(scan, a.q_tx_index);
  const int wave = rv_tid() >> 6, g = (rv_tid() & 63) / N;
  const int n = rdo_ntx(a), total = n * nplanes;
  const int w0 = (blockIdx.x * 4 + wave) * TPW;
  if (w0 >= total) return;
  const int i = w0 + g;
  const bool valid = i < total;
  const int ii = valid ? i : total - 1;
  const int plane = ii / n, t = ii - plane * n;
  uint8_t *mine = lds + (wave * TPW + g) * PER;
  rdo_cand_body<Px, N, N, MODE, LUMA>(a, a.p[plane], t, valid, reinterpret_cast<int32_t *>(mine),
                                       reinterpret_cast<Px *>(mine + SLAB), scan);
}

template <typename Px, int N, int MODE, bool LUMA>
__device__ __forceinline__ void rdo_small_part(const RdoArgs &a, int nplanes, int blk,
                                               uint8_t *lds, uint16_t *scan) {
  constexpr int TPW = 64 / N;
  constexpr int SLAB = rdo_slab_bytes<Px, N>();
  constexpr int PER = (SLAB + N * N * (int)sizeof(Px) + 15) / 16 * 16;
  stage_scan(scan, a.q_tx_index);
  const int wave = rv_tid() >> 6, g = (rv_tid() & 63) / N;
  const int n = rdo_ntx(a), total = n * nplanes;
  const int w0 = (blk * 4 + wave) * TPW;
  if (w0 >= total) return;
  const int i = w0 + g;
  const bool valid = i < total;
  const int ii = valid ? i : total - 1;
  const int plane = ii / n, t = ii - plane * n;
  uint8_t *mine = lds + (wave * TPW + g) * PER;
  rdo_cand_body<Px, N, N, MODE, LUMA>(a, a.p[plane], t, valid, reinterpret_cast<int32_t *>(mine),
                                       reinterpret_cast<Px *>(mine + SLAB), scan);
}

template <typename Px, int N>
constexpr int rdo_small_lds() {
  return 4 * (64 / N) * ((rdo_slab_bytes<Px, N>() + N * N * (int)sizeof(Px) + 15) / 16 * 16);
}

template <typename Px, int NL, int NC, int MODE>
__global__ __launch_bounds__(256) void rdo_small2_kernel(RdoArgs l, RdoArgs c, int lgrid) {
  constexpr int BL = rdo_small_lds<Px, NL>(), BC = rdo_small_lds<Px, NC>();
  __shared__ __align__(16) uint8_t lds[BL > BC ? BL : BC];
  __shared__ uint16_t scan[1024];
  if ((int)blockIdx.x < lgrid)
    rdo_small_part<Px, NL, MODE, true>(l, 1, blockIdx.x, lds, scan);
  else
    rdo_small_part<Px, NC, MODE, false>(c, 2, blockIdx.x - lgrid, lds, scan);
}

template <int NL, int NC>
static void rdo_small2_launch(const RdoArgs &l, const RdoArgs &c, int hbd, hipStream_t s,
                              int mode) {
  const int lg = (l.n_tx + 4 * (64 / NL) - 1) / (4 * (64 / NL));
  const int cg = (c.n_tx * 2 + 4 * (64 / NC) - 1) / (4 * (64 / NC));
  const unsigned grid = (unsigned)(lg + cg);
  if (grid == 0) return;
#define RV_SMALL2(PX, M) rdo_small2_kernel<PX, NL, NC, M><<<grid, 256, 0, s>>>(l, c, lg)
  if (hbd) {
    if (mode == 0) RV_SMALL2(uint16_t, 0); else if (mode == 1) RV_SMALL2(uint16_t, 1); else RV_SMALL2(uint16_t, 2);
  } else {
    if (mode == 0) RV_SMALL2(uint8_t, 0); else if (mode == 1) RV_SMALL2(uint8_t, 1); else RV_SMALL2(uint8_t, 2);
  }
#undef RV_SMALL2
}

template <int N, bool LUMA>
static void rdo_small_launch(const RdoArgs &a, int nplanes, int hbd, hipStream_t s, int mode) {
  constexpr int TPW = 64 / N;
  const unsigned grid = (unsigned)((a.n_tx * nplanes + 4 * TPW - 1) / (4 * TPW));
  if (grid == 0) return;
#define RV_SMALL(PX, M) rdo_small_kernel<PX, N, M, LUMA><<<grid, 256, 0, s>>>(a, nplanes)
  if (hbd) {
    if (mode == 0) RV_SMALL(uint16_t, 0); else if (mode == 1) RV_SMALL(uint16_t, 1); else RV_SMALL(uint16_t, 2);
  } else {
    if (mode == 0) RV_SMALL(uint8_t, 0); else if (mode == 1) RV_SMALL(uint8_t, 1); else RV_SMALL(uint8_t, 2);
  }
#undef RV_SMALL
}

template <int MODE>
static void rdo_launch(const RdoArgs &luma, const RdoArgs &chroma, int hbd, hipStream_t s,
                       unsigned cpairs) {
  if (luma.bd == 12) {
    const unsigned grid = (unsigned)luma.n_tx + cpairs;
    if (grid == 0) return;
    if (hbd)
      rdo_frame_kernel<uint16_t, MODE><<<grid, 64, 0, s>>>(luma, chroma);
    else
      rdo_frame_kernel<uint8_t, MODE><<<grid, 64, 0, s>>>(luma, chroma);
    return;
  }
  const int nquads = (luma.n_tx + 3) / 4;
  const unsigned grid = (unsigned)nquads + (cpairs + 2) / 3;
  if (grid == 0) return;
  if (hbd)
    rdo_quad_kernel<uint16_t, MODE><<<grid, 256, 0, s>>>(luma, chroma, nquads, kRdoVariant);
  else
    rdo_quad_kernel<uint8_t, MODE><<<grid, 256, 0, s>>>(luma, chroma, nquads, kRdoVariant);
}

int rv_rdo_candidates(const RdoArgs &luma, const RdoArgs &chroma, int hbd, hipStream_t s,
                      bool compound) {
  const unsigned cpairs = (unsigned)(2 * ((chroma.n_tx + 1) / 2));
  if (luma.commit)
    rdo_launch<2>(luma, chroma, hbd, s, cpairs);
  else if (compound)
    rdo_launch<1>(luma, chroma, hbd, s, cpairs);
  else
    rdo_launch<0>(luma, chroma, hbd, s, cpairs);
  RV_HIP_CHECK_LAUNCH();
  return RV_OK;
}

int rv_rdo_args_put(const RdoArgs *h, int n, RdoArgs *dev, hipStream_t s) {
  if (!h || !dev || n < 1 || n > 4) return rv_set_error(RV_EINVAL, "rv_rdo_args_put: bad arguments");
  rdo_args_store_kernel<<<1, 256, 0, s>>>(h[0], h[n > 1 ? 1 : 0], h[n > 2 ? 2 : 0], h[n > 3 ? 3 : 0],
                                          n, dev);
  RV_HIP_CHECK_LAUNCH();
  return RV_OK;
}

int rv_rdo_candidates_list(const RdoArgs *h, const RdoArgs *dev, int nsets, int mode_a, int hbd,
                           hipStream_t s, int max_grid, uint32_t *kp_cnt, unsigned long long *kp_t) {
  if (!h || !dev || nsets < 1 || nsets > 2 || mode_a < 0 || mode_a > 1 || (nsets == 2 && mode_a) ||
      h[0].commit || h[0].bd == 12)
    return rv_set_error(RV_EINVAL, "rv_rdo_candidates_list: bad arguments");
  for (int k = 0; k < 2 * nsets; k++)
    if (!h[k].list || !h[k].count)
      return rv_set_error(RV_EINVAL, "rv_rdo_candidates_list: the sets must be list-driven");
  static const bool phases = getenv("RAV1E_HIP_RDO_PHASES") && getenv("RAV1E_HIP_RDO_PHASES")[0] == '1';
  const int var = kRdoVariant | (phases && max_grid > 0 ? 16 : 0) | (max_grid > 0 ? 32 : 0);
  unsigned full = 0;
  for (int k = 0; k < nsets; k++)
    full += (unsigned)((h[2 * k].n_tx + 3) / 4) +
            ((var & 32) ? (unsigned)(2 * h[2 * k + 1].n_tx + 3) / 4
                        : (unsigned)(2 * ((h[2 * k + 1].n_tx + 1) / 2) + 2) / 3);
  unsigned grid = std::min(full, kF4Pool);
  if (max_grid > 0) grid = std::min(grid, (unsigned)max_grid);
  if (grid == 0) return RV_OK;
#define RV_LIST(PX, MA, MB) \
  rdo_quad_list_kernel<PX, MA, MB><<<grid, 256, 0, s>>>(dev, nsets, var, kp_cnt, kp_t)
  if (hbd) {
    if (nsets == 2) RV_LIST(uint16_t, 0, 1); else if (mode_a) RV_LIST(uint16_t, 1, 1); else RV_LIST(uint16_t, 0, 0);
  } else {
    if (nsets == 2) RV_LIST(uint8_t, 0, 1); else if (mode_a) RV_LIST(uint8_t, 1, 1); else RV_LIST(uint8_t, 0, 0);
  }
#undef RV_LIST
  RV_HIP_CHECK_LAUNCH();
  return RV_OK;
}

int rv_rdo_intra(const RdoArgs &luma, const RdoArgs &chroma, int hbd, hipStream_t s) {
  const unsigned cpairs = (unsigned)(2 * ((chroma.n_tx + 1) / 2));
  rdo_launch<3>(luma, chroma, hbd, s, cpairs);
  RV_HIP_CHECK_LAUNCH();
  return RV_OK;
}

int rv_rdo_blocks2(const RdoArgs &l, const RdoArgs &c, int nl, int nc, int hbd, hipStream_t s,
                   int mode) {
  if (nl == 32 && nc == 16) rdo_small2_launch<32, 16>(l, c, hbd, s, mode);
  else if (nl == 16 && nc == 8) rdo_small2_launch<16, 8>(l, c, hbd, s, mode);
  else if (nl == 8 && nc == 4) rdo_small2_launch<8, 4>(l, c, hbd, s, mode);
  else if (nl == 32 && nc == 32) rdo_small2_launch<32, 32>(l, c, hbd, s, mode);
  else if (nl == 16 && nc == 16) rdo_small2_launch<16, 16>(l, c, hbd, s, mode);
  else if (nl == 8 && nc == 8) rdo_small2_launch<8, 8>(l, c, hbd, s, mode);
  else return rv_set_error(RV_EINVAL, "rv_rdo_blocks2: sizes");
  RV_HIP_CHECK_LAUNCH();
  return RV_OK;
}

int rv_rdo_blocks(const RdoArgs &a, bool luma, int nplanes, int n_tx_size, int hbd,
                  hipStream_t s, int mode) {
  if (luma) {
    if (n_tx_size == 32) rdo_small_launch<32, true>(a, nplanes, hbd, s, mode);
    else if (n_tx_size == 16) rdo_small_launch<16, true>(a, nplanes, hbd, s, mode);
    else if (n_tx_size == 8) rdo_small_launch<8, true>(a, nplanes, hbd, s, mode);
    else return rv_set_error(RV_EINVAL, "rv_rdo_blocks: luma size");
  } else {
    if (n_tx_size == 32) rdo_small_launch<32, false>(a, nplanes, hbd, s, mode);
    else if (n_tx_size == 16) rdo_small_launch<16, false>(a, nplanes, hbd, s, mode);
    else if (n_tx_size == 8) rdo_small_launch<8, false>(a, nplanes, hbd, s, mode);
    else if (n_tx_size == 4) rdo_small_launch<4, false>(a, nplanes, hbd, s, mode);
    else return rv_set_error(RV_EINVAL, "rv_rdo_blocks: chroma size");
  }
  RV_HIP_CHECK_LAUNCH();
  return RV_OK;
}

extern "C" int rv_rdo_phase_dump(void) {
  unsigned long long h[3][8];
  if (hipDeviceSynchronize() != hipSuccess || hipMemcpyFromSymbol(h, HIP_SYMBOL(g_rdo_ph), sizeof(h)) != hipSuccess)
    return rv_set_error(RV_EHIP, "rv_rdo_phase_dump");
  const double us = 0.01;
  static const char *kName[2] = {"single", "compound"};
  for (int m = 0; m < 2; m++) {
    const double n = h[m][5] ? (double)h[m][5] : 1.0;
    fprintf(stderr,
            "[f4 phases] %s luma quads %llu: front %.2f, row DCT %.2f, quantize %.2f, inverse rows %.2f, "
            "back %.2f us per quad\n",
            kName[m], h[m][5], h[m][0] * us / n, h[m][1] * us / n, h[m][2] * us / n, h[m][3] * us / n,
            h[m][4] * us / n);
  }
  fprintf(stderr, "[f4 phases] chroma triples %llu: %.2f us each\n", h[2][5],
          h[2][0] * us / (h[2][5] ? (double)h[2][5] : 1.0));
  memset(h, 0, sizeof(h));
  return hipMemcpyToSymbol(HIP_SYMBOL(g_rdo_ph), h, sizeof(h)) == hipSuccess ? RV_OK
                                                                           : rv_set_error(RV_EHIP, "rv_rdo_phase_dump");
}
```

### rav1e_amd/csrc/rv_replay.h

```cpp
#pragma once
#include <string.h>

#include <chrono>
#include <condition_variable>
#include <algorithm>
#include <deque>
#include <mutex>
#include <thread>
#include <vector>

#include "rv_cdef.h"
#include "rv_chain.h"
#include "rv_deblock.h"
#include "rv_device.h"
#include "rv_ec.h"
#include "rv_frame.h"
#include "rv_intra.h"
#include "rv_intra_pass.h"
#include "rv_me.h"
#include "rv_mvref.h"
#include "rv_owned.h"
#include "rv_impwin.h"
#include "rv_lrf.h"
#include "rv_rdo.h"
// ... 176 lines not shown
  int n = 0;
  std::mutex mu;
  std::condition_variable cv;
  std::vector<long> posted;
  std::vector<uint8_t *> buf[kRing];
  std::vector<hipEvent_t> ev[kRing];
};

struct RvLaEngine {
  static constexpr int kLaSlack = 28;
  int W = 0, RW = 0, dev = 0;
  long limit = 0;
  Owned own;
  hipStream_t las = nullptr;
  RoundRing rr;
  int32_t *la_list = nullptr;
  void *scratch = nullptr;
  size_t scratch_bytes = 0;
  struct Entry {
    LaOut o;
    ImpFrame f;
    long m = -1;
    long used_by = -1;
    rv_replay_frame_info fi{};
    LaRefs lr{};
    hipEvent_t ev_imp = nullptr, ev_used = nullptr;
    hipEvent_t ev_data = nullptr, ev_xchg = nullptr;
  };
  std::vector<Entry> ring;
  std::vector<long> pyr_display;
  std::thread th;
  std::mutex mu;
  std::condition_variable cv;
  long requested = 0;
  long inputs_ready = 0;
  long imp_ready = 0;
  long imp_next = 1;
  bool stop = false;
  int err = 0;
  std::string msg;
  long la_round_sum = 0, la_reeval = 0, la_frames = 0;
  void *comm = nullptr;
  uint8_t *psend = nullptr, *precv = nullptr;
  size_t pbytes = 0;
  long data_ready = 0, xchg_done = 0, xchg_next = 1;
  rv_la_hub *hub = nullptr;
  int hub_k = -1;
  Entry &at(long m) { return ring[(size_t)(m % RW)]; }
};

struct rv_replay {
  rv_replay_cfg cfg{};
  Geo g{};
  int RA = 1;
  CandGeo cg{};
  Owned own;
  hipStream_t stream = nullptr;
  template <class T>
  T *dev(size_t n, Fill fill = Fill::None) { return own.dev<T>(n, fill, stream); }
  hipEvent_t ev_ielig = nullptr;
  bool overlap = false;
  bool own_stream = false;
  bool sea = false;
  struct Level {
    bool set = false;
    int qidx = 0;
    QCtx ql{}, qu{}, qv{};
    QCtx qil{}, qiu{}, qiv{};
    QCtx qs[kLevels][3] = {};
    double lambda = 0.0, me_lambda = 0.0, ds[3] = {0.0, 0.0, 0.0};
  } lv[3] = {};
  struct PLevel {
    int B = 0, n = 0, gw = 0, gh = 0, bc = 0, bch = 0, txl = 0, txc = 0;
    CandGeo cg{};
    rv_ds_job *jobs_full[3] = {nullptr, nullptr, nullptr}, *jobs_sub[3] = {nullptr, nullptr, nullptr};
    rv_fs_result *full = nullptr, *sub = nullptr;
    uint64_t *l_out = nullptr, *c_out = nullptr;
    RdoWinner *win = nullptr;
    int32_t *cand_list = nullptr, *cand_count = nullptr;
    int32_t *l_lev = nullptr, *c_lev = nullptr;
    int32_t *leaf = nullptr;
    size_t woff = 0;
  } pl[kLevels] = {};
  bool s6 = false;
  bool lvl = false;
  int ex0 = 0, ey0 = 0, ew = 0, eh = 0;
  bool lv_used[kLevels] = {false, false, false, false};
  bool lv_me[kLevels] = {false, false, false, false};
  hipStream_t edge[kLevels] = {nullptr, nullptr, nullptr, nullptr};
  hipEvent_t ev_efork = nullptr, ev_l1me = nullptr, ev_epart = nullptr;
  hipEvent_t ev_ejoin[kLevels] = {nullptr, nullptr, nullptr, nullptr};
  hipEvent_t ev_ecommit[kLevels] = {nullptr, nullptr, nullptr, nullptr};
  bool deblock = false;
  uint8_t *mi_lg = nullptr, *mi_skip = nullptr;
  int mi_stride = 0, mi_cols = 0, mi_rows = 0;
  uint8_t db_level[3] = {0, 0, 0};
  int64_t *db_tally = nullptr;
  uint8_t *db_dlev = nullptr;
  bool cdef = false;
  bool lrf = false;
  uint64_t *lrf_err = nullptr;
  int8_t *lrf_xqd = nullptr, *lrf_units = nullptr;
  int lrf_fix_passes = 1 << 30;
  RvInput lrf_out{};
  RvInput cdef_pre{};
  uint8_t *cdef_dir = nullptr, *cdef_idx = nullptr;
  int32_t *cdef_var = nullptr;
  uint8_t cdef_str[3][2] = {};
  int32_t *leaf_count = nullptr;
  bool entropy = false;
  EcFrameBufs ecb{};
  EcHost *ech = nullptr;
  long ec_frames = 0;
  bool intra = false;
  uint8_t *i_elig = nullptr, *i_was = nullptr, *i_win = nullptr, *i_modes = nullptr;
  int32_t *i_mark = nullptr, *i_list[2] = {nullptr, nullptr}, *i_commit = nullptr,
          *i_revert = nullptr;
  int32_t *i_cnt = nullptr;
  int32_t *h_cnt = nullptr;
  void *i_edges = nullptr;
  uint64_t *i_lout = nullptr, *i_cout = nullptr;
  uint32_t *i_stats = nullptr;
  bool exact = false;
  MvStack *stk = nullptr;
  BlkDec *dec_lv[3] = {nullptr, nullptr, nullptr};
  uint8_t *mv_active = nullptr;
  static constexpr int kRoundsAhead = 2;
  RoundRing rr;
  int32_t *mv_list = nullptr;
  bool edge_tr = false;
  long mv_round_sum = 0, mv_reeval = 0, mv_run_sum = 0;
  long mv_frames = 0;
  size_t nwords = 0, wpart = 0;
  bool jobs_built = false;
  std::mutex jobs_mu;
  std::vector<RvSlot> slots;
  std::vector<RvInput> inputs;
  rv_fs_job *fs_jobs[3] = {nullptr, nullptr, nullptr};
  rv_fs_result *coarse = nullptr, *half = nullptr, *full = nullptr, *sub = nullptr, *look = nullptr;
  rv_fs_result *half_l = nullptr;
  rv_ds_job *jobs_half[3] = {}, *jobs_full[3] = {}, *jobs_sub[3] = {}, *jobs_look[3] = {};
  rv_ds_job *jobs_half_l[3] = {nullptr, nullptr, nullptr};
  int32_t *la_list = nullptr;
  long la_round_sum = 0, la_reeval = 0;
  long la_frames = 0;
  RvLaEngine *eng = nullptr;
  bool eng_owned = false;
  const float *imp_last = nullptr;
  int32_t *src_half = nullptr, *src_full = nullptr, *src_look = nullptr;
  uint64_t *l_out = nullptr, *c_out = nullptr;
  RdoWinner *win = nullptr;
  int32_t *cand_list = nullptr, *cand_count = nullptr;
  RdoArgs *f4_args = nullptr;
  CandKey *cand_key = nullptr;
  uint8_t *f3dirty = nullptr;
  uint8_t *f2dirty = nullptr;
  uint32_t *cand_evals = nullptr;
  int32_t *l_lev = nullptr, *c_lev = nullptr;
  uint64_t *words = nullptr;
  unsigned long long *tail = nullptr;
  float *imp = nullptr;
  int n_imp = 0, imp_bx = 0, imp_by = 0, ntx_c = 0;
  long coded = 0;
  rv_replay_frame_info last{};
  int n_groups = 1, my_group = 0;
  int32_t grects[4 * kMaxGroups] = {};
  size_t xbytes = 0;
  uint8_t *xsend = nullptr, *xrecv = nullptr;
  void *comm = nullptr;
  static constexpr int kRing = 64;
  hipEvent_t evs[kRing][kEvCount] = {};
  int timing_stride = 1, timing_block = 1;
  long timed = 0;
  uint32_t *ds_evals = nullptr;
  static constexpr int kProbes = 2, kKpCnt = 4;
  bool kprobe = false;
  static constexpr int kKp = 512;
  std::vector<hipEvent_t> kp_ev[kProbes];
  long kp_n[kProbes] = {0, 0}, kp_done[kProbes] = {0, 0}, kp_base[kProbes] = {0, 0};
  long kp_init[kProbes] = {0, 0};
  static constexpr int kKpInit = 256;
  double kp_ms[kProbes] = {0.0, 0.0}, kp_dev_ms[kProbes] = {0.0, 0.0};
  uint32_t *kp_cnt[kProbes] = {nullptr, nullptr};
  unsigned long long *kp_ts[kProbes] = {nullptr, nullptr};
  double kp_tick_ms = 0.0;
};

template <typename Check, typename Eval>
int run_rounds(RoundRing &rr, hipStream_t xs, int budget, Check &&check, Eval &&eval,
               long *nrounds, long *nre, bool *changed, const char *what, long frame, int level) {
  static const bool mv_trace = getenv("RAV1E_HIP_MV_TRACE") != nullptr;
  if (changed) *changed = false;
  rr.last_count = -1;
  const uint32_t first = rr.seq++;
  RV_R(check(first));
  int queued = 0;
  for (int seen = 0;; seen++) {
    while (queued < budget && queued < seen + rv_replay::kRoundsAhead) {
      RV_R(eval(first + (uint32_t)queued));
      RV_R(check(rr.seq++));
      queued++;
    }
    const uint32_t q = first + (uint32_t)seen;
    volatile unsigned long long *pub = rr.h_pub + q % RoundRing::kPub;
    const auto t0 = std::chrono::steady_clock::now();
    unsigned long long v;
    for (long spin = 0;; spin++) {
      v = *pub;
      if ((uint32_t)(v >> 32) == q) break;
      if ((spin & 1023) == 1023) {
        const hipError_t he = hipStreamQuery(xs);
        if (he != hipSuccess && he != hipErrorNotReady)
          return rv_set_error(RV_EHIP, "rv_replay_frame: a round failed");
        if (std::chrono::steady_clock::now() - t0 > std::chrono::seconds(30))
          return rv_set_error(RV_EHIP, "rv_replay_frame: a round's count never arrived");
        std::this_thread::yield();
      }
    }
    const int c = (int)(uint32_t)v;
    rr.last_count = c;
    if (mv_trace) fprintf(stderr, "%s frame %ld level %d check %d: %d\n", what, frame, level, seen, c);
    if (c == 0) return RV_OK;
    if (seen >= budget)
      return rv_set_error(RV_EHIP, "rv_replay_frame: rounds beyond the chain's dependency "
                                   "depth (internal error)");
    *nre += c;
    (*nrounds)++;
    if (changed) *changed = true;
  }
}

namespace rv {

inline bool groups_active(const rv_replay *r) { return r->n_groups >= 2 || r->comm; }

hipError_t kp_harvest(rv_replay *r, int p, long upto);
size_t plane_bytes(const rv_plane &p);
void round_ring_alloc(Owned &dev, Owned &host, RoundRing &q, hipStream_t st);
int ensure_jobs(rv_replay *r);
int group_rects(const rv_replay *r, int k, XRect out[9], int *n);
int xcopy(rv_replay *r, const RvSlot &s, const XRect *rects, int n, int to_plane, uint8_t *buf);
int lrf_decide_slot(rv_replay *r, const RvSlot &s, const RvInput &in, int lv, const LrfGeo &lg,
                    const int32_t *rect);
int filter_slot(rv_replay *r, const RvSlot &s, const RvInput &in, int lv);
void frame_info(long n, int R, rv_replay_frame_info *f);
LaRefs la_refs_of(long m, int R);

int lookahead_frame(rv_replay *r, RoundRing &rr, hipStream_t xs, const rv_replay_frame_info &fi,
                    const LaRefs &lr, long frame, const LaOut &o, int32_t *la_list, bool pyramid,
                    long *nrounds, long *nre, hipEvent_t *e);
void la_engine_destroy(rv_replay *r);
int la_encode_exchange(rv_replay *r, long n, hipStream_t st);
int la_engine_take(rv_replay *r, long n, hipStream_t st, const float **imp);
int la_engine_release(rv_replay *r, long n, hipStream_t st);

}
```

### rav1e_amd/csrc/rv_replay.hip

```cpp
#include "rv_replay.h"

namespace rv {

__global__ void coeff_checksum(const int32_t *packed, int64_t total, int per_block,
                               unsigned long long *out) {
  uint64_t s = 0;
  for (int64_t i = (int64_t)blockIdx.x * blockDim.x + threadIdx.x; i < total;
       i += (int64_t)gridDim.x * blockDim.x)
    s += (uint64_t)(int64_t)packed[i] * (uint64_t)(i % per_block + 1);
  block_atomic_add(s, out);
}

template <typename Px>
__global__ void sum_rect(rv_plane p, int x0, int y0, int w, int h, unsigned long long *out) {
  uint64_t s = 0;
  for (int64_t i = (int64_t)blockIdx.x * blockDim.x + threadIdx.x; i < (int64_t)w * h;
       i += (int64_t)gridDim.x * blockDim.x) {
    const int y = (int)(i / w), x = (int)(i - (int64_t)y * w);
    s += *plane_ptr<Px>(p, x0 + x, y0 + y);
  }
  block_atomic_add(s, out);
}

struct XArgs {
// ... 633 lines not shown
  P0.gh = g.th;
  for (int l = 1; l < kLevels; l++) {
    rv_replay::PLevel &P = r->pl[l];
    const int k = 1 << l;
    P.B = kSb >> l;
    P.gw = r->ew * k;
    P.gh = r->eh * k;
    P.n = P.gw * P.gh;
    P.bc = P.B >> g.xdec;
    P.bch = P.B >> g.ydec;
    P.txl = 4 - l;
    P.txc = P.bc == 32 ? 3 : P.bc == 16 ? 2 : P.bc == 8 ? 1 : 0;
    P.cg = CandGeo{P.n, P.gw, P.gh, (g.tx0 + r->ex0) * k, (g.ty0 + r->ey0) * k, g.tws * k,
                   g.ths * k, g.R, g.M, 0};
    P.woff = r->nwords;
    r->nwords += (size_t)P.n * (4 * g.R + 4);
  }
  r->wpart = r->nwords;
  r->nwords += (size_t)g.nsb;
  return RV_OK;
}

static int configure_stages(rv_replay *r) {
  const Geo &g = r->g;
  const uint32_t flags = r->cfg.flags;
  r->intra = !r->s6 && !(flags & RV_REPLAY_NO_INTRA) && g.xdec == 1 && g.ydec == 1;
  r->exact = !r->s6 && !(flags & RV_REPLAY_MVREF_STANDIN);
  for (int sb = 0; sb < g.nsb && r->exact && r->lvl; sb++) {
    const int fsx = g.tx0 + sb % g.tw, fsy = g.ty0 + sb / g.tw;
    const int t0x = fsx - fsx % g.tws;
    const int cols = std::min(g.tws * 16, g.w_in_b - t0x * 16);
    if ((fsx + 1) * 64 <= g.W && (fsy + 1) * 64 <= g.H && fsy % g.ths != 0 &&
        (fsx - t0x) * 16 + 16 < cols && (fsx + 2) * 64 > g.W)
      r->edge_tr = true;
  }
  if (flags & RV_REPLAY_CDEF) {
    if (!(flags & RV_REPLAY_DEBLOCK) || (g.W & 7) || (g.H & 7))
      return rv_set_error(RV_EINVAL, "rv_replay_create: RV_REPLAY_CDEF needs RV_REPLAY_DEBLOCK and a "
                                     "frame size that is a multiple of 8");
    r->cdef = true;
  }
  if (flags & RV_REPLAY_LRF) {
    LrfGeo lg;
    if (!r->cdef || g.xdec != g.ydec ||
        lrf_geometry(g.W, g.H, g.xdec, g.ydec, g.bd, 100, g.tws, g.ths, &lg) != RV_OK)
      return rv_set_error(RV_EINVAL, "rv_replay_create: RV_REPLAY_LRF needs RV_REPLAY_CDEF, 4:2:0 or 4:4:4 "
                                     "(rav1e's enable_restoration is off in 4:2:2) and units of one superblock");
    r->lrf = true;
    const char *fe = getenv("RAV1E_LRF_FIX"), *fp = getenv("RAV1E_LRF_FIX_PASSES");
    r->lrf_fix_passes = (fe && fe[0] == '0') ? 0 : fp ? std::max(atoi(fp), 1) : 1 << 30;
  }
  r->entropy = (flags & RV_REPLAY_ENTROPY) != 0;
  if (r->entropy && g.xdec != g.ydec)
    return rv_set_error(RV_EINVAL, "rv_replay_create: RV_REPLAY_ENTROPY needs xdec == ydec");
  r->deblock = (flags & RV_REPLAY_DEBLOCK) != 0;
  if (r->deblock || r->entropy) {
    r->mi_cols = (g.W + 3) / 4;
    r->mi_rows = (g.H + 3) / 4;
    r->mi_stride = (r->mi_cols + 15) / 16 * 16;
  }
  if (r->entropy) {
    EcFrameBufs &b = r->ecb;
    b.ntiles = ((g.tw + g.tws - 1) / g.tws) * ((g.th + g.ths - 1) / g.ths);
    b.max_jobs = ec_max_jobs(g.nsb, b.ntiles);
    b.map_w4 = g.tws * 16;
    b.map_h4 = g.ths * 16;
    b.cap = (uint32_t)((size_t)g.nsb * (1024 + 2 * r->ntx_c * 1024) + (size_t)b.max_jobs * 4);
  }
  const char *e = getenv("RAV1E_HIP_REPLAY_SERIAL");
  r->overlap = !(e && e[0] == '1');
  return RV_OK;
}

static int replay_configure(const rv_replay_cfg *cfg, rv_replay *r) {
  if (!cfg || cfg->width <= 0 || cfg->height <= 0 || (cfg->width & 7) || (cfg->height & 7) ||
      (cfg->bit_depth != 8 && cfg->bit_depth != 10 && cfg->bit_depth != 12) || cfg->xdec < 0 ||
      cfg->xdec > 1 || cfg->ydec < 0 || cfg->ydec > 1 || cfg->n_refs < 1 || cfg->n_refs > 2 ||
      cfg->n_inputs < 1 || cfg->tile_w_sb < 0 || cfg->tile_h_sb < 0)
    return rv_set_error(RV_EINVAL, "rv_replay_create: bad config");
  r->cfg = *cfg;
  Geo &g = r->g;
  g.W = cfg->width;
  g.H = cfg->height;
  g.xdec = cfg->xdec;
  g.ydec = cfg->ydec;
  g.bd = cfg->bit_depth;
  g.hbd = cfg->bit_depth > 8;
  g.w_in_b = 2 * ((g.W + 7) >> 3);
  g.h_in_b = 2 * ((g.H + 7) >> 3);
  const int sbc = (g.W + kSb - 1) / kSb, sbr = (g.H + kSb - 1) / kSb;
  g.tx0 = cfg->tile_x0;
  g.ty0 = cfg->tile_y0;
  g.tw = cfg->tile_w > 0 ? cfg->tile_w : sbc - g.tx0;
  g.th = cfg->tile_h > 0 ? cfg->tile_h : sbr - g.ty0;
  g.tws = cfg->tile_w_sb > 0 ? cfg->tile_w_sb : sbc;
  g.ths = cfg->tile_h_sb > 0 ? cfg->tile_h_sb : sbr;
  if (g.tx0 < 0 || g.ty0 < 0 || g.tw <= 0 || g.th <= 0 || g.tx0 + g.tw > sbc ||
      g.ty0 + g.th > sbr || g.tx0 % g.tws || g.ty0 % g.ths ||
      ((g.tx0 + g.tw) % g.tws && g.tx0 + g.tw != sbc) ||
      ((g.ty0 + g.th) % g.ths && g.ty0 + g.th != sbr))
    return rv_set_error(RV_EINVAL,
                        "rv_replay_create: the tile group is not a rectangle of whole tiles");
  g.vis_w = (g.W - g.tx0 * kSb) < g.tw * kSb ? g.W - g.tx0 * kSb : g.tw * kSb;
  g.vis_h = (g.H - g.ty0 * kSb) < g.th * kSb ? g.H - g.ty0 * kSb : g.th * kSb;
  g.nsb = g.tw * g.th;
  g.R = cfg->n_refs;
  r->RA = g.R == 2 ? kImpMaxRefs : g.R;
  g.M = kCandModes;
  g.C = g.R * g.M + (g.R == 2 ? kCompModes : 0);
  g.cw = kSb >> g.xdec;
  g.ch = kSb >> g.ydec;
  g.w_imp = g.w_in_b / 2;
  g.h_imp = g.h_in_b / 2;
  r->cg = CandGeo{g.nsb, g.tw, g.th, g.tx0, g.ty0, g.tws, g.ths, g.R, g.M, 0};
  r->sea = g.bd <= 10 && (cfg->flags & RV_REPLAY_EXHAUSTIVE_FS) == 0;
  r->ntx_c = (g.cw / 32) * (g.ch / 32);
  r->imp_bx = g.vis_w / 8;
  r->imp_by = g.vis_h / 8;
  r->n_imp = r->imp_bx * r->imp_by;
  const int32_t me[4] = {g.tx0, g.ty0, g.tw, g.th};
  memcpy(r->grects, me, sizeof(me));
  RV_R(configure_levels(r));
  return configure_stages(r);
}

static void alloc_dpb(rv_replay *r, const rv_replay *share) {
  r->slots = share ? share->slots : std::vector<RvSlot>(kSlots);
  r->inputs = share ? share->inputs : std::vector<RvInput>(r->cfg.n_inputs);
  if (share) return;
  for (auto &s : r->slots) alloc_slot(r, s);
  for (auto &in : r->inputs) alloc_input(r, in, true);
}

static void alloc_superblocks(rv_replay *r) {
  const Geo &g = r->g;
  const size_t nsb = (size_t)g.nsb, nr = nsb * g.R, nc = nsb * g.C;
  r->coarse = r->dev<rv_fs_result>(nr);
  r->half = r->dev<rv_fs_result>(nr * 4);
  r->look = r->dev<rv_fs_result>(nr * 16, Fill::Zero);
  r->half_l = r->dev<rv_fs_result>(nr * 4, Fill::Zero);
  r->la_list = r->dev<int32_t>(nr * 20);
  r->full = r->dev<rv_fs_result>(nr);
  r->sub = r->dev<rv_fs_result>(nr);
  r->ds_evals = r->dev<uint32_t>((size_t)rv_replay::kRing * 2 * nr, Fill::Zero);
  r->l_out = r->dev<uint64_t>(nc * 3);
  r->c_out = r->dev<uint64_t>(nc * r->ntx_c * 3 * 2);
  r->win = r->dev<RdoWinner>(nsb);
  r->cand_list = r->dev<int32_t>(nc);
  r->cand_key = r->dev<CandKey>(nsb * (g.R * g.M + kCompModes), Fill::Zero);
  r->f3dirty = r->dev<uint8_t>(nsb * g.R);
  r->f2dirty = r->dev<uint8_t>(nsb * g.R * 4);
  r->cand_count = r->dev<int32_t>(2, Fill::Zero);
  r->f4_args = r->dev<RdoArgs>(4);
  r->cand_evals = r->dev<uint32_t>((size_t)rv_replay::kRing * 2 * kLevels, Fill::Zero);
  r->l_lev = r->dev<int32_t>(nsb * 1024, Fill::Zero);
  r->c_lev = r->dev<int32_t>(nsb * r->ntx_c * 1024 * 2, Fill::Zero);
  r->words = r->dev<uint64_t>(r->nwords, Fill::Zero);
  r->tail = r->dev<unsigned long long>(5, Fill::Zero);
}

static void alloc_levels(rv_replay *r) {
  if (!r->lvl) return;
  size_t nleaf = (size_t)r->g.nsb;
  for (int l = 1; l < kLevels; l++) {
    rv_replay::PLevel &P = r->pl[l];
    const size_t n = (size_t)P.n, nr = n * r->g.R, nc = n * r->g.C;
    P.full = r->dev<rv_fs_result>(nr);
    P.sub = r->dev<rv_fs_result>(nr);
    P.l_out = r->dev<uint64_t>(nc * 3);
    P.c_out = r->dev<uint64_t>(nc * 3 * 2);
    P.win = r->dev<RdoWinner>(n);
    P.cand_list = r->dev<int32_t>(nc);
    P.cand_count = r->dev<int32_t>(2, Fill::Zero);
    P.l_lev = r->dev<int32_t>(n * P.B * P.B, Fill::Zero);
    P.c_lev = r->dev<int32_t>(n * P.bc * P.bch * 2, Fill::Zero);
    nleaf += n;
  }
  int32_t *lf = r->dev<int32_t>(nleaf);
  r->leaf_count = r->dev<int32_t>(kLevels, Fill::Zero);
  for (int l = 0; l < kLevels && lf; l++) {
    r->pl[l].leaf = lf;
    lf += r->pl[l].n;
  }
}

static void alloc_intra(rv_replay *r) {
  r->i_stats = r->dev<uint32_t>((size_t)rv_replay::kRing * 3, Fill::Zero);
  if (!r->intra) return;
  const size_t n = (size_t)r->g.nsb;
  r->i_elig = r->dev<uint8_t>(n);
  r->i_was = r->dev<uint8_t>(n, Fill::Zero);
  r->i_win = r->dev<uint8_t>(2 * n, Fill::Zero);
  r->i_modes = r->dev<uint8_t>(4 * n);
  for (int32_t **list : {&r->i_mark, &r->i_list[0], &r->i_list[1], &r->i_commit, &r->i_revert})
    *list = r->dev<int32_t>(n);
  r->i_cnt = r->dev<int32_t>(4);
  r->i_edges = r->dev<uint8_t>(n * 3 * kIntraEdge * (r->g.hbd ? 2 : 1));
  r->i_lout = r->dev<uint64_t>(n * 3 * 3);
  r->i_cout = r->dev<uint64_t>(n * 6 * 3 * 2);
  r->h_cnt = r->own.pinned<int32_t>(4, hipHostMallocDefault);
  r->ev_ielig = r->own.event(hipEventDisableTiming);
}

static void alloc_mvref(rv_replay *r) {
  round_ring_alloc(r->own, r->own, r->rr, r->stream);
  if (!r->exact) return;
  const size_t n = (size_t)r->g.nsb;
  r->stk = r->dev<MvStack>(n);
  for (int l = 0; l < 3; l++) r->dec_lv[l] = r->dev<BlkDec>(n, Fill::Zero);
  r->mv_active = r->dev<uint8_t>(n);
  r->mv_list = r->dev<int32_t>(2 * n);
}

static void alloc_filters(rv_replay *r) {
  const Geo &g = r->g;
  const size_t n8 = (size_t)(g.W / 8) * (g.H / 8), n64 = (size_t)((g.W + 63) / 64) * ((g.H + 63) / 64);
  if (r->cdef) {
    r->cdef_dir = r->dev<uint8_t>(n8);
    r->cdef_var = r->dev<int32_t>(n8);
    r->cdef_idx = r->dev<uint8_t>(n64, Fill::Zero);
    alloc_input(r, r->cdef_pre, false);
  }
  if (r->lrf) {
    r->lrf_err = r->dev<uint64_t>(3 * n64 * 17);
    r->lrf_xqd = r->dev<int8_t>(3 * n64 * 32);
    r->lrf_units = r->dev<int8_t>(3 * n64 * 3);
    alloc_input(r, r->lrf_out, false);
  }
  if (!r->deblock && !r->entropy) return;
  const size_t mb = (size_t)r->mi_stride * (r->mi_rows + 16);
  r->mi_lg = r->dev<uint8_t>(mb, Byte(4));
  r->mi_skip = r->dev<uint8_t>(mb, Fill::Zero);
  if (r->s6 && r->deblock) {
    r->db_tally = r->dev<int64_t>(3 * 130);
    r->db_dlev = r->dev<uint8_t>(4);
  }
}

static void alloc_sync(rv_replay *r) {
  for (int f = 0; f < rv_replay::kRing; f++)
    for (int i = 0; i < kEvCount; i++) r->evs[f][i] = r->own.event(hipEventDisableSystemFence);
  if (!r->overlap || !r->lvl || r->s6) return;
  for (hipEvent_t *ev : {&r->ev_efork, &r->ev_l1me, &r->ev_epart})
    *ev = r->own.event(hipEventDisableTiming);
  const hipStream_t es = r->own.stream();
  for (int l = 1; l < kLevels; l++) {
    r->edge[l] = es;
    r->ev_ejoin[l] = r->own.event(hipEventDisableTiming);
    r->ev_ecommit[l] = r->own.event(hipEventDisableTiming);
  }
}

static void alloc_entropy(rv_replay *r) {
  if (!r->entropy) return;
  EcFrameBufs &b = r->ecb;
  b.jobs = r->dev<rv_ec_job>((size_t)b.max_jobs);
  b.sb_off = r->dev<uint32_t>((size_t)r->g.nsb + 1);
  b.map = r->dev<uint8_t>((size_t)b.ntiles * 3 * b.map_w4 * b.map_h4);
  b.scratch = r->dev<uint8_t>(rv_ec_scratch_bytes(b.max_jobs));
  b.offsets = r->dev<uint32_t>((size_t)b.max_jobs + 1);
  b.dstat = r->dev<uint32_t>(4);
  EcHost *eh = r->ech = new EcHost();
  eh->ntiles = b.ntiles;
  for (int k = 0; k < 2; k++) {
    eh->tok_h[k] = r->own.pinned<uint32_t>(b.cap, hipHostMallocMapped | hipHostMallocCoherent);
    eh->stat_h[k] = r->own.pinned<uint32_t>((size_t)b.ntiles + 8, hipHostMallocMapped | hipHostMallocCoherent);
    eh->ev[k] = r->own.event(hipEventBlockingSync | hipEventDisableTiming);
  }
  if (!r->own.failed) eh->th = std::thread([eh] { eh->run(); });
}

}

extern "C" {

void rv_replay_destroy(rv_replay *r) {
  if (!r) return;
  la_engine_destroy(r);
  if (r->stream) (void)hipStreamSynchronize(r->stream);
  if (r->ech) {
    {
      std::lock_guard<std::mutex> lk(r->ech->mu);
      r->ech->stop = true;
    }
    r->ech->cv.notify_all();
    if (r->ech->th.joinable()) r->ech->th.join();
    delete r->ech;
  }
  if (r->edge[1]) (void)hipStreamSynchronize(r->edge[1]);
  r->own.release();
  delete r;
}

static rv_replay *create_impl(const rv_replay_cfg *cfg, void *stream, const rv_replay *share) {
  rv_replay *r = new rv_replay();
  if (replay_configure(cfg, r) != RV_OK) {
    delete r;
    return nullptr;
  }
  r->own_stream = !stream;
  r->stream = stream ? (hipStream_t)stream : r->own.stream();
  if (!r->stream) {
    rv_set_error(RV_EHIP, "rv_replay_create: stream");
    delete r;
    return nullptr;
  }
// ... 280 lines not shown
    RV_H(hipEventSynchronize(e[kEvF7]));
    n = 0;
    for (int i = kEvStart; i < kEvF7 && n < cap; i++) {
      float ms = 0.f;
      RV_H(hipEventElapsedTime(&ms, e[i], e[i + 1]));
      ms_out[n++] += ms;
    }
    for (int k = 0; k < nspans && n < cap; k++) {
      float ms = 0.f;
      RV_H(hipEventSynchronize(e[spans[k][1]]));
      RV_H(hipEventElapsedTime(&ms, e[spans[k][0]], e[spans[k][1]]));
      ms_out[n++] += ms;
    }
  }
  return n;
}

int rv_replay_entropy_stats(rv_replay *r, uint64_t *out, int cap) {
  if (!r || !out || cap < 4) return rv_set_error(RV_EINVAL, "rv_replay_entropy_stats: null / cap");
  if (!r->ech) return rv_set_error(RV_EINVAL, "rv_replay_entropy_stats: RV_REPLAY_ENTROPY off");
  r->ech->drain();
  if (r->ech->err) return rv_set_error(r->ech->err, "rv_replay_entropy_stats: token buffer overflow");
  const int n = cap < 5 ? cap : 5;
  for (int i = 0; i < n; i++) out[i] = r->ech->stat[i];
  return n;
}

int rv_replay_set_timing(rv_replay *r, int stride, int block) {
  if (!r || stride < 0 || block < 1)
    return rv_set_error(RV_EINVAL, "rv_replay_set_timing: bad stride / block");
  r->timing_stride = stride;
  r->timing_block = block;
  return RV_OK;
}

int rv_replay_stage_times(rv_replay *r, float *ms_out, int cap) {
  return stage_times(r, ms_out, cap, 1);
}
int rv_replay_stage_times_sum(rv_replay *r, int last_frames, float *ms_out, int cap) {
  return stage_times(r, ms_out, cap, last_frames);
}

int rv_replay_set_kernel_probe(rv_replay *r, int on) {
  if (!r) return rv_set_error(RV_EINVAL, "rv_replay_set_kernel_probe: null");
  constexpr int P = rv_replay::kProbes, C = rv_replay::kKpCnt;
  if (on && r->kp_ev[0].empty()) {
    for (int p = 0; p < P; p++) {
      r->kp_ev[p].assign(2 * rv_replay::kKp, nullptr);
      for (auto &ev : r->kp_ev[p]) ev = r->own.event(hipEventDefault);
      r->kp_cnt[p] = r->dev<uint32_t>(C);
      r->kp_ts[p] = r->dev<unsigned long long>(2 * rv_replay::kKp);
      if (r->own.failed)
        return rv_set_error(RV_EHIP, "rv_replay_set_kernel_probe: allocation failed");
    }
    int dev = 0, khz = 0;
    RV_H(hipGetDevice(&dev));
    RV_H(hipDeviceGetAttribute(&khz, hipDeviceAttributeWallClockRate, dev));
    r->kp_tick_ms = khz > 0 ? 1.0 / (double)khz : 0.0;
  }
  if (!r->kp_ev[0].empty()) {
    for (int p = 0; p < P; p++) RV_H(kp_harvest(r, p, r->kp_n[p]));
    RV_H(hipDeviceSynchronize());
    for (int p = 0; p < P; p++) RV_H(hipMemset(r->kp_cnt[p], 0, C * sizeof(uint32_t)));
    RV_H(hipDeviceSynchronize());
  }
  for (int p = 0; p < P; p++) {
    r->kp_ms[p] = 0.0;
    r->kp_dev_ms[p] = 0.0;
    r->kp_base[p] = r->kp_n[p];
  }
  r->kprobe = on != 0;
  return RV_OK;
}

int rv_replay_kernel_probe(rv_replay *r, double *out, int cap) {
  if (!r || !out || cap < 4) return rv_set_error(RV_EINVAL, "rv_replay_kernel_probe: null / cap");
  const int nout = cap >= 12 ? 12 : cap < 5 ? 4 : 5;
  for (int i = 0; i < nout; i++) out[i] = 0.0;
  if (r->kp_ev[0].empty()) return nout;
  for (int p = 0; p < rv_replay::kProbes; p++) RV_H(kp_harvest(r, p, r->kp_n[p]));
  uint32_t c[2][rv_replay::kKpCnt] = {{0}};
  RV_H(hipDeviceSynchronize());
  for (int p = 0; p < rv_replay::kProbes; p++)
    RV_H(hipMemcpy(c[p], r->kp_cnt[p], sizeof(c[p]), hipMemcpyDeviceToHost));
  out[0] = (double)(r->kp_n[0] - r->kp_base[0]);
  out[1] = r->kp_ms[0];
  out[2] = (double)c[0][0];
  out[3] = (double)c[0][1];
  if (nout > 4) out[4] = r->kp_dev_ms[0];
  if (nout >= 12) {
    out[5] = (double)(r->kp_n[1] - r->kp_base[1]);
    out[6] = r->kp_ms[1];
    out[7] = r->kp_dev_ms[1];
    for (int i = 0; i < 4; i++) out[8 + i] = (double)c[1][i];
  }
  return nout;
}
int rv_replay_dpb_slots(void) { return kSlots; }

int rv_replay_counters(rv_replay *r, uint64_t *out, int cap) {
  if (!r || !out || cap < 3) return rv_set_error(RV_EINVAL, "rv_replay_counters");
  const Geo &g = r->g;
  const int nj = g.nsb * g.R;
  const long nonkey = r->coded > 0 ? r->coded - 1 : 0;
  const int nf = nonkey < rv_replay::kRing ? (int)nonkey : rv_replay::kRing;
  RV_H(hipStreamSynchronize(r->stream));
  std::vector<uint32_t> h((size_t)nf * 2 * nj);
  if (nf) RV_H(hipMemcpy(h.data(), r->ds_evals, h.size() * 4, hipMemcpyDeviceToHost));
  out[0] = out[1] = 0;
  for (int f = 0; f < nf; f++)
    for (int k = 0; k < 2; k++)
      for (int j = 0; j < nj; j++) out[k] += h[((size_t)f * 2 + k) * nj + j];
  out[2] = (uint64_t)nf;
  if (cap < 5) return 3;
  const int nl = cap >= 11 ? kLevels : 1;
  std::vector<uint32_t> ce((size_t)nf * 2 * kLevels);
  if (nf) RV_H(hipMemcpy(ce.data(), r->cand_evals, ce.size() * 4, hipMemcpyDeviceToHost));
  for (int l = 0; l < nl; l++) {
    uint64_t &a = out[l ? 5 + 2 * (l - 1) : 3], &b = out[l ? 6 + 2 * (l - 1) : 4];
    a = b = 0;
    for (int f = 0; f < nf; f++) {
      a += ce[(size_t)(f * kLevels + l) * 2];
      b += ce[(size_t)(f * kLevels + l) * 2 + 1];
    }
  }
  if (cap < 14) return nl == 1 ? 5 : 11;
  std::vector<uint32_t> is((size_t)nf * 3);
  if (nf) RV_H(hipMemcpy(is.data(), r->i_stats, is.size() * 4, hipMemcpyDeviceToHost));
  out[11] = out[12] = out[13] = 0;
  for (int f = 0; f < nf; f++)
    for (int k = 0; k < 3; k++) out[11 + k] += is[(size_t)f * 3 + k];
  if (cap < 17) return 14;
  out[14] = (uint64_t)r->mv_round_sum;
  out[15] = (uint64_t)r->mv_reeval;
  out[16] = (uint64_t)r->mv_frames;
  if (cap < 18) return 17;
  out[17] = (uint64_t)r->mv_run_sum;
  if (cap < 20) return 18;
  const bool own_eng = r->eng && r->eng_owned;
  long er = 0, ere = 0, ef = 0;
  if (own_eng) {
    std::lock_guard<std::mutex> lk(r->eng->mu);
    er = r->eng->la_round_sum;
    ere = r->eng->la_reeval;
    ef = r->eng->la_frames;
  }
  out[18] = (uint64_t)(r->la_round_sum + er);
  out[19] = (uint64_t)(r->la_reeval + ere);
  if (cap < 21) return 20;
  out[20] = (uint64_t)(r->la_frames + ef);
  return 21;
}

int rv_round_ring_slots(uint32_t q, int32_t *out, int cap) {
  if (!out || cap < 6) return rv_set_error(RV_EINVAL, "rv_round_ring_slots: cap");
  static int32_t cnt[2 * RoundRing::kCnt + 1];
  static unsigned long long pub[RoundRing::kPub];
  RoundRing rr;
  rr.cnt = cnt;
  rr.d_pub = pub;
  const RoundPub p = rr.pub(q);
  out[0] = (int32_t)((p.cnt - cnt) / 2);
  out[1] = (int32_t)((p.next - cnt) / 2);
  out[2] = (int32_t)(p.host - pub);
  out[3] = rv_replay::kRoundsAhead;
  out[4] = RoundRing::kCnt;
  out[5] = RoundRing::kPub;
  return 6;
}

int rv_replay_lrf_units(rv_replay *r, int plane, int8_t *out, int cap) {
  if (!r || !out || plane < 0 || plane > 2) return rv_set_error(RV_EINVAL, "rv_replay_lrf_units: bad arguments");
  if (!r->lrf) return rv_set_error(RV_EINVAL, "rv_replay_lrf_units: RV_REPLAY_LRF is off");
  const Geo &g = r->g;
  const int nsb = ((g.W + 63) / 64) * ((g.H + 63) / 64);
  if (cap < 3 * nsb) return rv_set_error(RV_EINVAL, "rv_replay_lrf_units: cap < 3 * superblocks");
  RV_H(hipStreamSynchronize(r->stream));
  RV_H(hipMemcpy(out, r->lrf_units + (size_t)plane * nsb * 3, (size_t)nsb * 3, hipMemcpyDeviceToHost));
  return RV_OK;
}

int rv_replay_la_refs(long m, int R, int32_t *out) {
  if (!out || m < 1 || R < 1 || R > 2) return rv_set_error(RV_EINVAL, "rv_replay_la_refs");
  const LaRefs l = la_refs_of(m, R);
  out[0] = l.n;
  for (int k = 0; k < 3; k++) {
    out[1 + k] = k < l.n ? l.disp[k] : -1;
    out[4 + k] = k < l.n ? l.order[k] : -1;
  }
  return RV_OK;
}

int rv_comm_unique_id(uint8_t *out, int cap) {
#if RV_HAVE_RCCL
  if (!out || cap < (int)sizeof(ncclUniqueId)) return rv_set_error(RV_EINVAL, "rv_comm_unique_id");
  ncclUniqueId id;
  if (ncclGetUniqueId(&id) != ncclSuccess) return rv_set_error(RV_EHIP, "ncclGetUniqueId");
  memcpy(out, &id, sizeof(id));
  return (int)sizeof(id);
#else
  (void)out;
  (void)cap;
  return rv_set_error(RV_EINVAL, "rv_comm_unique_id: built without RCCL");
#endif
}

void *rv_comm_create(const uint8_t *id, int nranks, int rank) {
#if RV_HAVE_RCCL
  if (!id || nranks < 1 || rank < 0 || rank >= nranks) {
    rv_set_error(RV_EINVAL, "rv_comm_create");
    return nullptr;
  }
  ncclUniqueId u;
  memcpy(&u, id, sizeof(u));
  ncclComm_t c = nullptr;
  if (ncclCommInitRank(&c, nranks, u, rank) != ncclSuccess) {
    rv_set_error(RV_EHIP, "ncclCommInitRank");
    return nullptr;
  }
  return c;
#else
  (void)id;
  (void)nranks;
  (void)rank;
  rv_set_error(RV_EINVAL, "rv_comm_create: built without RCCL");
  return nullptr;
#endif
}

void rv_comm_destroy(void *comm) {
#if RV_HAVE_RCCL
  if (comm) (void)ncclCommDestroy((ncclComm_t)comm);
#else
  (void)comm;
#endif
}

}
```

### rav1e_amd/csrc/rv_replay_frame.hip

```cpp
#include "rv_replay.h"

namespace rv {

struct CandCost {
  double rs, rn;
  uint64_t ds, dn;
  int live;
};
__device__ inline CandCost cand_cost(const CandGeo &cg, double lambda, double ds_u, double ds_v,
                                     const rv_fs_result *sub, const uint64_t *lout,
                                     const uint64_t *uout, const uint64_t *vout, int ntx_c, int sb,
                                     int c) {
  CandCost k{0.0, 0.0, 0, 0, 0};
  const int ns = cg.R * cg.M;
  rv_mv mv;
  if (c < ns ? !cand_live(cg, sub, sb, c, &mv) : !comp_live(cg, sub, sb, c - ns)) return k;
  k.live = 1;
  const int64_t o = (int64_t)c * cg.nsb + sb;
  uint64_t su = 0, sv = 0, nu = 0, nv = 0;
  uint32_t rate = (uint32_t)lout[o * 3 + 2];
  for (int j = 0; j < ntx_c; j++) {
    const int64_t t = (o * ntx_c + j) * 3;
    su += uout[t];
    sv += vout[t];
// ... 884 lines not shown
    return lv_decide(st);
  }
  int fork_edge_levels() {
    if (place != LvPlace::kEdge) {
      RV_R(ev(kEvEdgeBegin));
      return ev(kEvEdgeEnd);
    }
    hipStream_t e1 = r->edge[1];
    RV_H(hipEventRecord(r->ev_efork, st));
    for (int l = 1; l < kLevels; l++) RV_H(hipStreamWaitEvent(r->edge[l], r->ev_efork, 0));
    RV_R(ev(kEvEdgeBegin, e1));
    RV_R(lv_me(e1, 1));
    RV_H(hipEventRecord(r->ev_l1me, e1));
    for (int l = 1; l < kLevels; l++) {
      hipStream_t es = r->edge[l];
      if (l > 1 && r->lv_me[l]) {
        RV_H(hipStreamWaitEvent(es, r->ev_l1me, 0));
        RV_R(lv_me(es, l));
      }
      if (!r->lv_used[l]) continue;
      RV_R(lv_decide(es, l));
      RV_H(hipEventRecord(r->ev_ejoin[l], es));
    }
    for (int l : used())
      if (l > 1) RV_H(hipStreamWaitEvent(e1, r->ev_ejoin[l], 0));
    return ev(kEvEdgeEnd, e1);
  }
  int join_edge_scores() {
    if (place != LvPlace::kEdge) return RV_OK;
    for (int l : used()) RV_H(hipStreamWaitEvent(st, r->ev_ejoin[l], 0));
    return RV_OK;
  }

  MvrefArgs mvref_args() const {
    MvrefArgs a;
    memset(&a, 0, sizeof(a));
    a.nsb = g.nsb;
    a.tw = g.tw;
    a.th = g.th;
    a.tx0 = g.tx0;
    a.ty0 = g.ty0;
    a.tws = g.tws;
    a.ths = g.ths;
    a.W = g.W;
    a.H = g.H;
    a.w_in_b = g.w_in_b;
    a.h_in_b = g.h_in_b;
    a.R = g.R;
    a.comp = cg.comp ? 1 : 0;
    for (int k = 0; k < g.R; k++) a.sign_bias |= (uint32_t)(fi.ref_display[k] > fi.display) << k;
    a.dec = r->dec_lv[lv];
    a.stk = r->stk;
    a.active = r->mv_active;
    a.jf = r->jobs_full[lv];
    a.js = r->jobs_sub[lv];
    a.init = 1;
    a.lvl = r->lvl ? 1 : 0;
    if (r->lvl)
      for (int l : used()) {
        a.lwin[l] = r->pl[l].win;
        a.lsub[l] = r->pl[l].sub;
        a.lcg[l] = r->pl[l].cg;
      }
    a.epzs = 1;
    a.eg = eg;
    a.jh = r->jobs_half[lv];
    a.coarse = r->coarse;
    a.hq = r->half_l;
    a.prev = r->slots[fi.ref_display[0] % kSlots].fmv;
    a.edge_ok = 0;
    a.f3dirty = r->f3dirty;
    a.f2dirty = r->f2dirty;
    return a;
  }
  int check(uint32_t q) {
    ma.count = slot_cnt(q);
    ma.pub = r->rr.pub(q);
    ma.list = mvl(q);
    return rv_mvref_round(ma, st);
  }
  int check0() {
    ma = mvref_args();
    if (r->edge_tr) RV_R(join_edge_scores());
    return check(r->rr.seq++);
  }

  int f2() {
    if (r->exact)
      return rv_diamond_search_multi(&cur.hres, refs_h, g.R, r->jobs_half[lv], nr * 4, 16, 16, 0, 0,
                                     0, g.bd, r->half, nullptr, nullptr, st);
    RV_H(hipMemcpyAsync(r->half, r->half_l, (size_t)nr * g.R * 4 * sizeof(rv_fs_result),
                        hipMemcpyDeviceToDevice, st));
    fill_preds_kernel<<<(nr * g.R + 255) / 256, 256, 0, st>>>(r->jobs_full[lv], r->src_full,
                                                              nr * g.R, r->coarse, r->half, 0);
    return RV_OK;
  }

  int round0() {
    const bool with_lv = place == LvPlace::kRound0;
    if (f4_list) RV_R(rv_rdo_args_put(f4h, cg.comp ? 4 : 2, r->f4_args, st));
    RV_R(rv_diamond_search_multi(&cur.y, refs_y, g.R, r->jobs_full[lv], nr, 64, 64, 0, 0, 0, g.bd,
                                 r->full, ev_full, &to_sub, st, act));
    RV_R(ev(kEvF3Full));
    RV_R(kp.open(st));
    RV_R(rv_diamond_search_multi(&cur.y, refs_y, g.R, r->jobs_sub[lv], nr, 64, 64, 1,
                                 r->s6 ? 1 : 0, 0, g.bd, r->sub, ev_sub, nullptr, st, act, nullptr,
                                 nullptr, 1, nullptr, 0, kp.acc(0), kp.ts()));
    RV_R(kp.close(st));
    if (with_lv) RV_R(lv_me(st));
    const CandKeys keys0{r->cand_key, (uint32_t)(r->coded + 1), 0};
    cand_list_kernel<<<(nsingle + 255) / 256, 256, 0, st>>>(cg, r->sub, nsingle, r->cand_list,
                                                            r->cand_count, act, keys0);
    if (with_lv) lv_lists(st, false);
    if (cg.comp) {
      comp_list_kernel<<<(g.nsb * cg.comp + 255) / 256, 256, 0, st>>>(
          cg, r->sub, nsingle, r->cand_list + nsingle, r->cand_count + 1, act, keys0);
      if (with_lv) lv_lists(st, true);
    }
    RV_R(ev(kEvF3Sub));
    if (f4_list) {
      RV_R(kp.open(st, 1));
      RV_R(rv_rdo_candidates_list(f4h, r->f4_args, 1, 0, g.hbd, st, 0, kp.acc(1), kp.ts(1)));
      RV_R(kp.close(st, 1));
    } else
      RV_R(rv_rdo_candidates(f4h[0], f4h[1], g.hbd, st));
    if (with_lv) RV_R(lv_rdo(st));
    RV_R(ev(kEvF4Single));
    if (cg.comp) {
      if (f4_list) {
        RV_R(kp.open(st, 1));
        RV_R(rv_rdo_candidates_list(f4h + 2, r->f4_args + 2, 1, 1, g.hbd, st, 0, kp.acc(1), kp.ts(1)));
        RV_R(kp.close(st, 1));
      } else
        RV_R(rv_rdo_candidates(f4h[2], f4h[3], g.hbd, st, true));
      if (with_lv) RV_R(lv_rdo_comp(st));
    }
    RV_R(ev(kEvF4Comp));
    score_wave_kernel<<<(g.nsb + 3) / 4, 256, 0, st>>>(
        g, cg, L.lambda, L.ds[1], L.ds[2], r->sub, r->l_out, r->c_out, r->c_out + nct * 3, ntx_c,
        r->win, r->coarse, r->half, r->full, r->look, r->half_l, r->words, r->cand_count,
        r->tail + 2, r->cand_evals + 2 * slot * kLevels, r->leaf_count, nullptr, nullptr,
        r->exact ? r->dec_lv[lv] : nullptr, 0);
    return RV_OK;
  }

  int round_of(uint32_t q) {
    const int32_t *acnt = slot_cnt(q);
    int lg = q == q_first ? nr * g.R : 0;
    const int hint = q == q_first ? -1 : r->rr.last_count;
    const int hsb = hint >= 0 ? std::max(2 * hint, 16) : 0;
    int f4_grid = 0;
    if (hsb) {
      lg = std::min(hsb * g.R, 512);
      f4_grid = std::min(6 * hsb, 1024);
    }
    RV_R(kp.open(st));
    RV_R(rv_diamond_f2_f3(&cur.hres, refs_h, r->jobs_half[lv], r->half, ma.f2dirty, &cur.y,
                          refs_y, r->jobs_full[lv], r->full, ma.f3dirty, &to_sub, g.R, nr, g.bd,
                          mvl(q), acnt, lg, st, r->jobs_sub[lv], r->sub, kp.acc(0), kp.ts()));
    RV_R(kp.close(st));
    const int rg = hsb ? std::min(kRoundGrid, std::max((14 * hsb + 255) / 256, (hsb + 3) / 4))
                       : kRoundGrid;
    round_lists_kernel<<<rg, 256, 0, st>>>(
        cg, r->sub, nsingle, r->cand_list, r->cand_count, mvl(q), acnt,
        CandKeys{r->cand_key, (uint32_t)(r->coded + 1), 1});
    if (f4_list) {
      RV_R(kp.open(st, 1));
      RV_R(rv_rdo_candidates_list(f4h, r->f4_args, cg.comp ? 2 : 1, 0, g.hbd, st, f4_grid,
                                  kp.acc(1), kp.ts(1)));
      RV_R(kp.close(st, 1));
    } else {
      RV_R(rv_rdo_candidates(f4h[0], f4h[1], g.hbd, st));
      if (cg.comp) RV_R(rv_rdo_candidates(f4h[2], f4h[3], g.hbd, st, true));
    }
    score_wave_kernel<<<rg, 256, 0, st>>>(
        g, cg, L.lambda, L.ds[1], L.ds[2], r->sub, r->l_out, r->c_out, r->c_out + nct * 3, ntx_c,
        r->win, r->coarse, r->half, r->full, r->look, r->half_l, r->words, r->cand_count, nullptr,
        nullptr, nullptr, mvl(q), acnt, r->dec_lv[lv], 1);
    return RV_OK;
  }

  int mv_rounds_run(const uint8_t *iwas, bool *changed) {
    mv_runs++;
    q_first = r->rr.seq;
    ma.init = 0;
    ma.iwas = iwas;
    return run_rounds(
        r->rr, st, budget, [this](uint32_t q) { return check(q); },
        [this](uint32_t q) { return round_of(q); }, &r->mv_round_sum, &r->mv_reeval, changed,
        "mvref", ncoded, lv);
  }
  int rounds() {
    RV_R(join_edge_scores());
    ma.hq = r->half;
    ma.edge_ok = 1;
    tr.r0 = HostTrace::now();
    RV_R(mv_rounds_run(nullptr, nullptr));
    tr.mv = HostTrace::now();
    return RV_OK;
  }

  PartArgs part_args() const {
    PartArgs pa;
    memset(&pa, 0, sizeof(pa));
    for (int l = 0; l < kLevels; l++) {
      const rv_replay::PLevel &P = r->pl[l];
      pa.win[l] = l ? P.win : r->win;
      pa.gw[l] = P.gw;
      pa.x0[l] = (g.tx0 + (l ? r->ex0 : 0)) * kSb;
      pa.y0[l] = (g.ty0 + (l ? r->ey0 : 0)) * kSb;
      pa.leaf[l] = P.leaf;
    }
    pa.ex0 = r->ex0;
    pa.ey0 = r->ey0;
    pa.ew = r->ew;
    pa.eh = r->eh;
    pa.forced = !r->s6;
    pa.leaf_count = r->leaf_count;
    pa.words = r->words + r->wpart;
    return pa;
  }
  int partition() {
    if (place == LvPlace::kNone) return RV_OK;
    RV_R(join_edge_scores());
    if (place == LvPlace::kRound0) lv_score(st);
    partition_kernel<<<(g.nsb + 63) / 64, 64, 0, st>>>(g, part_args());
    return RV_OK;
  }

  int commit() {
    const bool edge = place == LvPlace::kEdge;
    if (edge) {
      RV_H(hipEventRecord(r->ev_epart, st));
      for (int l : used()) {
        RV_H(hipStreamWaitEvent(r->edge[l], r->ev_epart, 0));
        RV_R(lv_commit(r->edge[l], l));
        RV_H(hipEventRecord(r->ev_ecommit[l], r->edge[l]));
      }
    }
    RV_R(rv_rdo_candidates(la, ca, g.hbd, st));
    if (edge) {
      for (int l : used()) RV_H(hipStreamWaitEvent(st, r->ev_ecommit[l], 0));
    } else if (place != LvPlace::kNone) {
      RV_R(lv_commit(st));
    }
    return RV_OK;
  }

  int intra_fixed_point() {
    int irounds = 0;
    if (r->intra) RV_R(intra_pass(r, la, ca, cur, S, L, slot, &irounds));
    tr.intra = HostTrace::now();
    for (int pass = 0; r->exact && r->intra; pass++) {
      if (pass > g.tws * g.ths)
        return rv_set_error(RV_EHIP, "rv_replay_frame: the MV / intra passes did not settle "
                                     "(internal error)");
      if (pass == 0 && irounds == 0) break;
      bool changed = false;
      RV_R(mv_rounds_run(r->i_was, &changed));
      if (!changed) break;
      RV_R(rv_rdo_candidates(la, ca, g.hbd, st));
      RV_R(intra_begin(r));
      RV_R(intra_pass(r, la, ca, cur, S, L, slot, &irounds));
    }
    return RV_OK;
  }

  int frame_mvs() {
    r->mv_round_sum++;
    r->mv_run_sum += mv_runs;
    r->mv_frames++;
    ma.iwas = r->intra ? r->i_was : nullptr;
    return rv_mvref_field(ma, S.fmv, st);
  }

  int f5_importance() {
    const unsigned nb = (unsigned)((r->n_imp + 255) / 256);
    if (g.hbd)
      importance_kernel<uint16_t><<<nb, 256, 0, st>>>(g, cur.y, refs_o[0], r->look, r->imp_bx,
                                                      r->imp_by, r->tail + 2);
    else
      importance_kernel<uint8_t><<<nb, 256, 0, st>>>(g, cur.y, refs_o[0], r->look, r->imp_bx,
                                                     r->imp_by, r->tail + 2);
    return RV_OK;
  }

  void block_map() {
    if (!r->lvl) {
      block_map_kernel<<<(g.nsb * 16 + 255) / 256, 256, 0, st>>>(
          nullptr, nullptr, g.nsb, g.tw, g.tx0, g.ty0, 0, r->win, r->mi_lg, r->mi_skip,
          r->mi_stride, r->mi_cols, r->mi_rows);
      return;
    }
    for (int l = 0; l < kLevels; l++) {
      const rv_replay::PLevel &P = r->pl[l];
      const int n4 = 16 >> l;
      block_map_kernel<<<(P.n * n4 + 255) / 256, 256, 0, st>>>(
          P.leaf, r->leaf_count + l, P.n, P.gw, l ? P.cg.tx0 : g.tx0, l ? P.cg.ty0 : g.ty0, l,
          l ? P.win : r->win, r->mi_lg, r->mi_skip, r->mi_stride, r->mi_cols, r->mi_rows);
    }
  }

  EcFrameArgs ec_frame_args() const {
    EcFrameArgs ea;
    ea.tx0 = g.tx0;
    ea.ty0 = g.ty0;
    ea.tw = g.tw;
    ea.th = g.th;
    ea.tws = g.tws;
    ea.ths = g.ths;
    ea.xdec = g.xdec;
    ea.ydec = g.ydec;
    ea.ntx_c = r->ntx_c;
    ea.nsb = g.nsb;
    ea.mi_lg = r->mi_lg;
    ea.mi_skip = r->mi_skip;
    ea.mi_stride = r->mi_stride;
    ea.mi_cols = r->mi_cols;
    ea.mi_rows = r->mi_rows;
    ea.lv[0].l_lev = r->l_lev;
    ea.lv[0].c_lev = r->c_lev;
    ea.lv[0].n = g.nsb;
// ... 138 lines not shown
```

### rav1e_amd/replay.py

```python
from __future__ import annotations

import ctypes as C

import os

import numpy as np

from . import RvReplayCfg, RvReplayFrameInfo, RvReplayLevelParams, _check, lib
from . import rate as _rate

DEFAULT_QUANTIZER = 100

RV_REPLAY_EXHAUSTIVE_FS = 4
RV_REPLAY_SPEED6 = 8
RV_REPLAY_DEBLOCK = 16
RV_REPLAY_CDEF = 32
RV_REPLAY_LRF = 512
RV_REPLAY_NO_INTRA = 64
RV_REPLAY_ENTROPY = 128
RV_REPLAY_MVREF_STANDIN = 256
N_STAGES = 16

GOP_SCALES = (4, 2, 1, 1)

# ... 202 lines not shown
            cfg.tile_x0, cfg.tile_y0, cfg.tile_w, cfg.tile_h = group
        self.cfg = cfg
        self.geom = (width, height, xdec, ydec, bit_depth)
        self.h = lib().rv_replay_create(C.byref(cfg), stream)
        if not self.h:
            raise RuntimeError(f"rv_replay_create: {lib().rv_last_error().decode()}")
        self.speed = 6 if flags & RV_REPLAY_SPEED6 else 10
        self.n_words = result_words(width, height, n_refs, cfg.tile_w, cfg.tile_h,
                                    cfg.tile_x0, cfg.tile_y0, self.speed, xdec, ydec)
        self.levels = _rate.level_params(quantizer, bit_depth)
        for lv, d in enumerate(self.levels):
            p = RvReplayLevelParams.from_dict(d)
            _check(lib().rv_replay_set_level_params(self.h, lv, C.byref(p)),
                   "rv_replay_set_level_params")
        self.imp_window = imp_window
        if imp_window:
            _check(lib().rv_replay_set_imp_window(self.h, int(imp_window), int(imp_limit)),
                   "rv_replay_set_imp_window")
        self.imp_shape = ((height + 7) // 8, (width + 7) // 8)

    def twin(self, stream=None):
        t = HipReplay.__new__(HipReplay)
        t.cfg, t.geom, t.speed, t.n_words, t.levels = self.cfg, self.geom, self.speed, \
            self.n_words, self.levels
        t.imp_window, t.imp_shape = self.imp_window, self.imp_shape
        t.h = lib().rv_replay_create_twin(self.h, stream)
        if not t.h:
            raise RuntimeError(f"rv_replay_create_twin: {lib().rv_last_error().decode()}")
        t.primary = self
        return t

    def seek(self, n: int):
        _check(lib().rv_replay_seek(self.h, int(n)), "rv_replay_seek")

    @property
    def stream(self):
        return lib().rv_replay_stream(self.h)

    def _frame_array(self):
        w, h, xd, yd, bd = self.geom
        n = frame_bytes(w, h, xd, yd, bd) // (2 if bd > 8 else 1)
        return np.zeros(n, dtype=np.uint16 if bd > 8 else np.uint8)

    def synth_inputs(self, t0: int = 0):
        _check(lib().rv_replay_synth_inputs(self.h, t0), "rv_replay_synth_inputs")

    def set_input(self, idx: int, yuv: np.ndarray):
        yuv = np.ascontiguousarray(yuv)
        _check(lib().rv_replay_set_input(self.h, idx, yuv.ctypes.data), "rv_replay_set_input")

    def get_input(self, idx: int) -> np.ndarray:
        out = self._frame_array()
        _check(lib().rv_replay_get_input(self.h, idx, out.ctypes.data), "rv_replay_get_input")
        return out

    def lrf_units(self, plane: int) -> np.ndarray:
        n = ((self.cfg.width + 63) // 64) * ((self.cfg.height + 63) // 64)
        out = np.zeros(3 * n, np.int8)
        _check(lib().rv_replay_lrf_units(self.h, plane, out.ctypes.data, out.size), "rv_replay_lrf_units")
        return out.reshape(n, 3)

    def get_recon(self, display: int) -> np.ndarray:
        out = self._frame_array()
        _check(lib().rv_replay_get_recon(self.h, display, out.ctypes.data), "rv_replay_get_recon")
        return out

    def set_inputs_ready(self, displays: int):
        _check(lib().rv_replay_set_inputs_ready(self.h, int(displays)),
               "rv_replay_set_inputs_ready")

    def set_importances(self, imp):
        if imp is None:
            _check(lib().rv_replay_set_importances(self.h, None, 0), "rv_replay_set_importances")
            return
        imp = np.ascontiguousarray(imp, dtype=np.float32)
        _check(lib().rv_replay_set_importances(self.h, imp.ctypes.data, imp.size),
               "rv_replay_set_importances")

    def importances(self) -> np.ndarray:
        out = np.zeros(self.imp_shape, np.float32)
        _check(lib().rv_replay_get_importances(self.h, out.ctypes.data, out.size),
               "rv_replay_get_importances")
        return out

    def frame(self) -> dict:
        fi = RvReplayFrameInfo()
        _check(lib().rv_replay_frame(self.h, C.byref(fi)), "rv_replay_frame")
        return {"display": fi.display, "me_range_scale": fi.me_range_scale, "level": fi.level,
                "is_key": fi.is_key, "ref_display": list(fi.ref_display),
                "compound": fi.compound}

    def set_la_exchange(self, comm=None, hub=None):
        _check(lib().rv_replay_set_la_exchange(self.h, comm, hub.h if hub else None),
               "rv_replay_set_la_exchange")

    def set_groups(self, rects, my_group, comm=None):
        arr = np.ascontiguousarray(np.asarray(rects, dtype=np.int32).ravel())
        _check(lib().rv_replay_set_groups(self.h, len(rects), arr.ctypes.data, my_group, comm),
               "rv_replay_set_groups")

    def exchange_buffers(self):
        s, r, n = C.c_void_p(), C.c_void_p(), C.c_size_t()
        _check(lib().rv_replay_exchange_buffers(self.h, C.byref(s), C.byref(r), C.byref(n)),
               "rv_replay_exchange_buffers")
        return s.value, r.value, n.value

    def import_(self):
        _check(lib().rv_replay_import(self.h), "rv_replay_import")

    def results(self) -> np.ndarray:
        out = np.zeros(self.n_words, dtype=np.uint64)
        n = lib().rv_replay_results(self.h, out.ctypes.data, out.size)
        if n < 0:
            _check(n, "rv_replay_results")
        return out[:n]

    def entropy_stats(self):
        out = np.zeros(5, np.uint64)
        n = lib().rv_replay_entropy_stats(self.h, out.ctypes.data, 5)
        if n < 0:
            _check(n, "rv_replay_entropy_stats")
        return [int(v) for v in out]

    def set_timing(self, stride: int, block: int = 1):
        _check(lib().rv_replay_set_timing(self.h, stride, block), "rv_replay_set_timing")

    def stage_ms(self) -> np.ndarray:
        out = np.zeros(N_STAGES, dtype=np.float32)
        n = lib().rv_replay_stage_times(self.h, out.ctypes.data, N_STAGES)
        if n < 0:
            _check(n, "rv_replay_stage_times")
        return out[:n]

    def stage_ms_sum(self, last_frames: int) -> np.ndarray:
        out = np.zeros(N_STAGES, dtype=np.float32)
        n = lib().rv_replay_stage_times_sum(self.h, last_frames, out.ctypes.data, N_STAGES)
        if n < 0:
            _check(n, "rv_replay_stage_times_sum")
        return out

    def set_kernel_probe(self, on: bool = True):
        _check(lib().rv_replay_set_kernel_probe(self.h, 1 if on else 0),
               "rv_replay_set_kernel_probe")

    def kernel_probe(self) -> np.ndarray:
        out = np.zeros(12, np.float64)
        _check(lib().rv_replay_kernel_probe(self.h, out.ctypes.data, 12) - 12,
               "rv_replay_kernel_probe")
        return out

    def counters(self) -> np.ndarray:
        out = np.zeros(21, dtype=np.uint64)
        _check(lib().rv_replay_counters(self.h, out.ctypes.data, 21) - 21, "rv_replay_counters")
        return out

    def close(self):
        if self.h:
            lib().rv_replay_destroy(self.h)
            self.h = None

    def __del__(self):
        try:
            self.close()
        except Exception:
            pass


def frame_info(n: int, n_refs: int = 2) -> dict:
    if n == 0:
        return {"display": 0, "me_range_scale": 0, "level": 0, "is_key": 1,
                "ref_display": [0, 0], "compound": 0}
    g, j = (n - 1) // 4, (n - 1) % 4
    rf = ((0, -4), (0, 4), (0, 2), (2, 4))[j]
    refs = [max(0, 4 * g + rf[k]) for k in range(n_refs)] + [0] * (2 - n_refs)
    return {"display": 4 * g + (4, 2, 1, 3)[j], "me_range_scale": (4, 2, 1, 1)[j],
            "level": (0, 1, 2, 2)[j], "is_key": 0, "ref_display": refs,
            "compound": int(n_refs == 2 and j in (1, 3))}


class PairedReplay:

    def __init__(self, primary: "HipReplay", twin_levels: str = None):
        import queue
        import threading
        self.twin_levels = twin_levels or os.environ.get("RAV1E_PAIRED_TWIN", "l2b")
        if self.twin_levels not in ("l2", "l2b", "alt"):
            raise ValueError(f"PairedReplay: twin_levels {self.twin_levels!r}")
        self.p = primary
        self.t = primary.twin()
        self.n = 0
        self.q = queue.Queue()
        self.err = None
        self._thr = threading
        self.ev_p = [lib().rv_event_create() for _ in range(8)]
        self.ev_t = [lib().rv_event_create() for _ in range(8)]
        self.ready_p, self.ready_t = {}, {}
        self.worker = threading.Thread(target=self._run, daemon=True)
        self.worker.start()

    def on_primary(self, f: int) -> bool:
        g, j = f // 4, f % 4
        if j < 2:
            return True
        if j == 3:
            return False
        return self.twin_levels == "l2b" or (self.twin_levels == "alt" and g % 2 == 0)

    def _flag(self, d, g):
        if g not in d:
            d[g] = self._thr.Event()
        return d[g]

    def frame(self) -> dict:
        n = self.n
        self.n += 1
        if n == 0:
            return self.p.frame()
        g, j = (n - 1) // 4, (n - 1) % 4
        if not self.on_primary(n - 1):
            self.q.put(n)
            return frame_info(n, self.p.cfg.n_refs)
        if j == 0 and g >= 2:
            self._flag(self.ready_t, g - 2).wait()
            self._raise()
            _check(lib().rv_stream_wait_event(self.p.stream, self.ev_t[(g - 2) % 8]),
                   "rv_stream_wait_event")
        self.p.seek(n)
        info = self.p.frame()
        if j == 1:
            _check(lib().rv_event_record(self.ev_p[g % 8], self.p.stream), "rv_event_record")
            self._flag(self.ready_p, g).set()
        return info

    def _run(self):
        while True:
            n = self.q.get()
            if n is None:
                self.q.task_done()
                return
            g, j = (n - 1) // 4, (n - 1) % 4
            try:
                if self.err is None:
                    self._flag(self.ready_p, g).wait()
                    _check(lib().rv_stream_wait_event(self.t.stream, self.ev_p[g % 8]),
                           "rv_stream_wait_event")
                    self.t.seek(n)
                    self.t.frame()
                    if j == 3:
                        _check(lib().rv_event_record(self.ev_t[g % 8], self.t.stream),
                               "rv_event_record")
            except Exception as e:
                self.err = e
            finally:
                if j == 3:
                    self._flag(self.ready_t, g).set()
                self.q.task_done()

    def _raise(self):
        if self.err is not None:
            e, self.err = self.err, None
            raise e

    def drain(self):
        self.q.join()
        self._raise()

    def results(self) -> np.ndarray:
        self.drain()
        return self.p.results()

    def set_timing(self, stride: int, block: int = 1):
        self.p.set_timing(stride, block)
        self.t.set_timing(stride, block)

    def entropy_stats(self):
        self.drain()
        a, b = self.p.entropy_stats(), self.t.entropy_stats()
        return [a[0], a[1], a[2], a[3] + b[3], a[4] + b[4]]

    def counters(self) -> np.ndarray:
        self.drain()
        a, b = self.p.counters(), self.t.counters()
        out = a + b
        out[2] = max(a[2], b[2])
        return out

    def stage_ms_sum(self, kp: int, kt: int) -> np.ndarray:
        self.drain()
        s = np.zeros(N_STAGES, np.float32)
        if kp:
            s = s + self.p.stage_ms_sum(kp)
        if kt:
            s = s + self.t.stage_ms_sum(kt)
        return s

    def close(self):
        if self.t is not None:
            self.q.put(None)
            self.worker.join()
            self.t.close()
            self.t = None
            for e in self.ev_p + self.ev_t:
                lib().rv_event_destroy(e)

    def __getattr__(self, name):
        return getattr(self.p, name)
# ... 260 lines not shown
```

Baseline: 178.9.

## Split luma RDO motion compensation across multiple wavefronts per candidate

```diff
diff --git a/include/rav1e_hip.h b/include/rav1e_hip.h
--- a/include/rav1e_hip.h
+++ b/include/rav1e_hip.h
@@ -469,6 +469,7 @@
 int rv_ds_phase_dump(void);
 int rv_rdo_phase_dump(void);
 int rv_replay_counters(rv_replay *r, uint64_t *out, int cap);
+int rv_replay_round_items(rv_replay *r, uint64_t out[4]);
 
 int rv_replay_dpb_slots(void);
 
diff --git a/rav1e_amd/__init__.py b/rav1e_amd/__init__.py
--- a/rav1e_amd/__init__.py
+++ b/rav1e_amd/__init__.py
@@ -306,6 +306,7 @@
         "rv_replay_stage_times": (i32, [vp, vp, i32]),
         "rv_replay_stage_times_sum": (i32, [vp, i32, vp, i32]),
         "rv_replay_counters": (i32, [vp, vp, i32]),
+        "rv_replay_round_items": (i32, [vp, vp]),
         "rv_replay_dpb_slots": (i32, []),
         "rv_replay_set_kernel_probe": (i32, [vp, i32]),
         "rv_replay_kernel_probe": (i32, [vp, vp, i32]),
diff --git a/rav1e_amd/csrc/rv_rdo.h b/rav1e_amd/csrc/rv_rdo.h
--- a/rav1e_amd/csrc/rv_rdo.h
+++ b/rav1e_amd/csrc/rv_rdo.h
@@ -63,6 +63,6 @@
 int rv_rdo_args_put(const rv::RdoArgs *h, int n, rv::RdoArgs *dev, hipStream_t s);
 int rv_rdo_candidates_list(const rv::RdoArgs *h, const rv::RdoArgs *dev, int nsets, int mode_a,
                            int hbd, hipStream_t s, int max_grid = 0, uint32_t *kp_cnt = nullptr,
-                           unsigned long long *kp_t = nullptr);
+                           unsigned long long *kp_t = nullptr, unsigned long long *items = nullptr);
 
 int rv_rdo_intra(const rv::RdoArgs &luma, const rv::RdoArgs &chroma, int hbd, hipStream_t s);
diff --git a/rav1e_amd/csrc/rv_rdo.hip b/rav1e_amd/csrc/rv_rdo.hip
--- a/rav1e_amd/csrc/rv_rdo.hip
+++ b/rav1e_amd/csrc/rv_rdo.hip
@@ -235,13 +235,14 @@
   return f.cf ? ring[(u + 3) & 7] : ring[(u + 3) & 7] << ib;
 }
 
-template <typename Px, int N, int RB>
+template <typename Px, int N, int RB, int NROWS = N>
 __device__ __forceinline__ void mc_compound(const RdoArgs &a, const RdoPlane &pl, const RdoJob &jb,
-                                            uint32_t *win, Px *pred) {
+                                            uint32_t *win, Px *pred, int row0 = 0) {
   constexpr int B = (int)sizeof(Px);
   constexpr int P = B == 1 ? ((N + 8 + 15) / 16) * 16 : ((2 * (N + 8) + 15) / 16) * 16;
   constexpr int kRowDw = ((N + 7) * B + 3) / 4, kTot = (RB + 7) * kRowDw;
-  static_assert((RB % 8 == 0 || RB < 8) && N % RB == 0, "bands of whole 8-row groups");
+  static_assert((RB % 8 == 0 || RB < 8) && NROWS % RB == 0 && NROWS <= N,
+                "bands of whole 8-row groups");
   constexpr int U = RB < 8 ? RB : 8;
   const int col = rv_tid() & (N - 1);
   const int ib = a.bd == 12 ? 2 : 4, maxv = (1 << a.bd) - 1;
@@ -253,14 +254,15 @@
       (const uint8_t *)plane_ptr<Px>(pl.ref[1], jb.src2_x + jb.ox - 3, jb.src2_y + jb.oy - 3);
   const int64_t rs0 = (int64_t)pl.ref[0].stride * B, rs1 = (int64_t)pl.ref[1].stride * B;
 #pragma unroll 1
-  for (int band = 0; band < N / RB; band++) {
+  for (int band = 0; band < NROWS / RB; band++) {
+    const int y0 = row0 + band * RB;
     if (band) wave_sync();
 #pragma unroll 2
     for (int i = col; i < kTot; i += N) {
       const int r = i / kRowDw, d = i - r * kRowDw;
       uint32_t v0, v1;
-      __builtin_memcpy(&v0, sp0 + (band * RB + r) * rs0 + 4 * d, 4);
-      __builtin_memcpy(&v1, sp1 + (band * RB + r) * rs1 + 4 * d, 4);
+      __builtin_memcpy(&v0, sp0 + (y0 + r) * rs0 + 4 * d, 4);
+      __builtin_memcpy(&v1, sp1 + (y0 + r) * rs1 + 4 * d, 4);
       w0[r * (P / 4) + d] = B == 1 ? v0 ^ 0x80808080u : v0;
       w1[r * (P / 4) + d] = B == 1 ? v1 ^ 0x80808080u : v1;
     }
@@ -280,7 +282,7 @@
         g0[(u + 6) & 7] = mc_h<Px>(f0, w0 + (r + 6) * (P / 4), col, ib);
         g1[(u + 6) & 7] = mc_h<Px>(f1, w1 + (r + 6) * (P / 4), col, ib);
         const int32_t t = mc_prep_v(f0, g0, u, ib) + mc_prep_v(f1, g1, u, ib);
-        pred[(band * RB + r) * N + col] = (Px)clamp_med3(round_shift(t, ib + 1), 0, maxv);
+        pred[(y0 + r) * N + col] = (Px)clamp_med3(round_shift(t, ib + 1), 0, maxv);
       }
     }
   }
@@ -664,14 +666,17 @@
   return group_sum<64>(distortion_biased(v, rdo_bias(a, px >> 2, py >> 2)));
 }
 
-template <typename Px, int NPART, int MODE>
-__device__ __forceinline__ void luma_front(const RdoArgs &a, const RdoPlane &pl, int t,
-                                           const RdoJob &jb, bool valid, uint8_t *scr, Px *pred,
-                                           bool skip_dist = true) {
+template <typename Px, int NPART, int MODE, int NROWS = 64>
+__device__ __forceinline__ void luma_mc(const RdoArgs &a, const RdoPlane &pl, const RdoJob &jb,
+                                        uint8_t *scr, Px *pred, int row0 = 0) {
   constexpr int N = 64, B = (int)sizeof(Px);
-  constexpr int P = LumaLds<Px, int16_t, NPART>::kWinP;
-  constexpr int RP = N / NPART;
-  static_assert(RP % 8 == 0, "MC rows run in groups of 8");
+  using L = LumaLds<Px, int16_t, NPART>;
+  constexpr int P = L::kWinP;
+  constexpr int RP = N / NPART < NROWS ? N / NPART : NROWS;
+  static_assert(RP % 8 == 0 && NROWS % RP == 0, "MC rows run in groups of 8");
+  static_assert(NROWS == N || MODE < 2, "a row range: scoring launches only");
+  static_assert((RP + 7) * P <= L::kScr && 2 * (L::kCompRows + 7) * P <= L::kScr,
+                "one wavefront's band windows fit its slot's scratch");
   const int lane = rv_tid() & 63;
   const rv_plane &ref = pl.ref[jb.ref];
   const int ox = 0, oy = 0;
@@ -680,8 +685,8 @@
   if constexpr (MODE == 3) {
     intra_fill<Px, 64, 64>(jb, reinterpret_cast<int32_t *>(scr), pred, bd, lane);
   } else if (MODE == 1 || (MODE == 2 && jb.comp)) {
-    mc_compound<Px, 64, LumaLds<Px, int16_t, NPART>::kCompRows>(
-        a, pl, jb, reinterpret_cast<uint32_t *>(scr), pred);
+    mc_compound<Px, 64, (L::kCompRows < NROWS ? L::kCompRows : NROWS), NROWS>(
+        a, pl, jb, reinterpret_cast<uint32_t *>(scr), pred, row0);
   } else
   {
     uint32_t *win = reinterpret_cast<uint32_t *>(scr);
@@ -741,9 +746,10 @@
     constexpr int kTot = (RP + 7) * kRowDw;
     const int64_t rs = (int64_t)ref.stride * B;
 #pragma unroll 1
-    for (int half = 0; half < NPART; half++) {
+    for (int half = 0; half < NROWS / RP; half++) {
+      const int y0 = row0 + RP * half;
       const uint8_t *sp =
-          (const uint8_t *)plane_ptr<Px>(ref, jb.src_x + ox - 3, jb.src_y + oy - 3 + RP * half);
+          (const uint8_t *)plane_ptr<Px>(ref, jb.src_x + ox - 3, jb.src_y + oy - 3 + y0);
       if (half) wave_sync();
 #pragma unroll 4
       for (int i = lane; i < kTot; i += 64) {
@@ -772,13 +778,21 @@
           } else {
             v = cf ? round_shift(ring[(u + 3) & 7], ib) : ring[(u + 3) & 7];
           }
-          pred[(RP * half + r) * N + col] = (Px)clamp_med3(v, 0, maxv);
+          pred[(y0 + r) * N + col] = (Px)clamp_med3(v, 0, maxv);
         }
       }
     }
     wave_sync();
   }
-
+}
+
+template <typename Px>
+__device__ __forceinline__ void luma_resid_col(const RdoArgs &a, const RdoPlane &pl,
+                                               const RdoJob &jb, bool valid, uint8_t *scr,
+                                               const Px *pred, bool skip_dist) {
+  constexpr int N = 64;
+  const int lane = rv_tid() & 63;
+  const int bd = a.bd;
   const Px *o = plane_ptr<Px>(pl.org, jb.bx, jb.by);
   if (!a.commit && skip_dist) {
     const uint64_t d = luma_dist<Px>(a, jb, o, pl.org.stride, pred);
@@ -799,6 +813,14 @@
 #pragma unroll
     for (int r = 0; r < 16; r++) fmid[r * 65 + lane] = rdo_rsa(v[r], -s1);
   }
+}
+
+template <typename Px, int NPART, int MODE>
+__device__ __forceinline__ void luma_front(const RdoArgs &a, const RdoPlane &pl, int t,
+                                           const RdoJob &jb, bool valid, uint8_t *scr, Px *pred,
+                                           bool skip_dist = true) {
+  luma_mc<Px, NPART, MODE>(a, pl, jb, scr, pred);
+  luma_resid_col<Px>(a, pl, jb, valid, scr, pred, skip_dist);
 }
 
 __device__ __forceinline__ void luma_fwd_row(int32_t *row, int bd) {
@@ -947,6 +969,14 @@
   for (int i = rv_tid(); i < 1024; i += blockDim.x) dst[i] = src[i];
   __syncthreads();
 }
+__device__ __forceinline__ void stage_scan(uint16_t *dst, int tx_index, int &staged) {
+  if (tx_index != staged) {
+    const uint16_t *src = RV_SCANS + RV_SCAN_OFF[tx_index];
+    for (int i = rv_tid(); i < 1024; i += blockDim.x) dst[i] = src[i];
+    staged = tx_index;
+  }
+  __syncthreads();
+}
 
 template <typename Px>
 using SingleLds = LumaLds<Px, typename std::conditional<sizeof(Px) == 1, int16_t, int32_t>::type, 2>;
@@ -979,31 +1009,38 @@
 #ifndef RV_RDO_PHASES
 #define RV_RDO_PHASES 0
 #endif
-__device__ unsigned long long g_rdo_ph[3][8];
+__device__ unsigned long long g_rdo_ph[5][8];
 struct QuadPh {
-  unsigned long long t[5];
+  unsigned long long t[5], mc;
 };
 
-template <typename Px, int MODE>
+template <typename Px, int MODE, int G = 1>
 __device__ __forceinline__ void rdo_quad_luma(const RdoArgs &luma, int b, int n, int var,
                                               uint8_t *lds, const uint16_t *scan,
-                                              QuadPh *ph = nullptr) {
+                                              QuadPh *ph = nullptr, bool split = false) {
   using L = typename QuadLds<Px>::L;
   constexpr int NPART = sizeof(Px) == 1 ? 2 : 4;
+  static_assert(G == 1 || ((G == 2 || G == 4) && MODE < 2), "split items: scoring launches");
+  const int g = G > 1 && split ? G : 1, gsh = g == 4 ? 2 : g == 2 ? 1 : 0;
+  const int K = 4 >> gsh;
   const int wave = __builtin_amdgcn_readfirstlane(rv_tid() >> 6), lane = rv_tid() & 63;
-  auto slot = [&](int q) __attribute__((always_inline)) { return lds + q * L::kSlot; };
-  auto fmid = [&](int q) __attribute__((always_inline)) {
-    return reinterpret_cast<int32_t *>(slot(q));
+  const int q = wave >> gsh, part = wave & (g - 1);
+  auto slot = [&](int c) __attribute__((always_inline)) {
+    return lds + (c << gsh) * L::kSlot;
   };
-  auto imid = [&](int q) __attribute__((always_inline)) {
-    return reinterpret_cast<int16_t *>(slot(q));
+  auto fmid = [&](int c) __attribute__((always_inline)) {
+    return reinterpret_cast<int32_t *>(slot(c));
   };
-  auto pred = [&](int q) __attribute__((always_inline)) {
-    return reinterpret_cast<Px *>(slot(q) + L::kScr);
+  auto imid = [&](int c) __attribute__((always_inline)) {
+    return reinterpret_cast<int16_t *>(slot(c));
   };
-  const int t0 = 4 * b, t = t0 + wave;
+  auto pred = [&](int c) __attribute__((always_inline)) {
+    return reinterpret_cast<Px *>(slot(c) + L::kScr);
+  };
+  const int t0 = K * b, t = t0 + q;
   if (t0 >= n) return;
   const bool valid = t < n;
+  const bool mine = valid && part == 0;
   RdoJob jb;
   if constexpr (MODE == 3)
     jb = rdo_job_intra<Px, 64>(luma, 0, valid ? t : n - 1);
@@ -1011,36 +1048,50 @@
     jb = rdo_job<64>(luma, luma.p[0], valid ? t : n - 1);
   const bool late_dist = (var & 1) && !luma.commit;
   const bool prio = (var & 2) != 0;
-  if (valid)
-    luma_front<Px, NPART, MODE>(luma, luma.p[0], t, jb, true, slot(wave), pred(wave), !late_dist);
+  if (g == 1) {
+    if (valid) luma_mc<Px, NPART, MODE>(luma, luma.p[0], jb, slot(q), pred(q));
+  } else if constexpr (G > 1) {
+    if (valid)
+      luma_mc<Px, NPART, MODE, 64 / G>(luma, luma.p[0], jb, lds + wave * L::kSlot, pred(q),
+                                       part * (64 / G));
+    __syncthreads();
+  }
+  if (RV_RDO_PHASES && ph) ph->mc = wall_clock64();
+  if (mine) {
+    luma_resid_col<Px>(luma, luma.p[0], jb, true, slot(q), pred(q), !late_dist);
+  } else if (valid && part == 1 && late_dist) {
+    const uint64_t d = luma_dist<Px>(luma, jb, plane_ptr<Px>(luma.p[0].org, jb.bx, jb.by),
+                                     luma.p[0].org.stride, pred(q));
+    if (lane == 0) luma.p[0].out[(int64_t)jb.oi * 3 + 0] = d;
+  }
   __syncthreads();
   if (RV_RDO_PHASES && ph) ph->t[1] = wall_clock64();
   if (wave == 0) {
     if (prio) __builtin_amdgcn_s_setprio(2);
-    const int q = lane >> 4;
-    if (t0 + q < n) luma_fwd_row(fmid(q) + (lane & 15) * 65, luma.bd);
+    const int c = lane >> 4;
+    if (c < K && t0 + c < n) luma_fwd_row(fmid(c) + (lane & 15) * 65, luma.bd);
     if (prio) __builtin_amdgcn_s_setprio(0);
-  } else if (late_dist && valid) {
+  } else if (g == 1 && late_dist && valid) {
     const uint64_t d = luma_dist<Px>(luma, jb, plane_ptr<Px>(luma.p[0].org, jb.bx, jb.by),
-                                     luma.p[0].org.stride, pred(wave));
+                                     luma.p[0].org.stride, pred(q));
     if (lane == 0) luma.p[0].out[(int64_t)jb.oi * 3 + 0] = d;
   }
   __syncthreads();
   if (RV_RDO_PHASES && ph) ph->t[2] = wall_clock64();
-  if (valid) luma_quantize(luma, luma.p[0], t, jb, true, fmid(wave), scan);
+  if (mine) luma_quantize(luma, luma.p[0], t, jb, true, fmid(q), scan);
   __syncthreads();
   if (RV_RDO_PHASES && ph) ph->t[3] = wall_clock64();
-  if (wave < 2) {
+  if (wave < (K + 1) / 2) {
     if (prio) __builtin_amdgcn_s_setprio(2);
-    const int q = 2 * wave + (lane >> 5), rr = lane & 31;
-    const bool vq = t0 + q < n;
+    const int c = 2 * wave + (lane >> 5), rr = lane & 31;
+    const bool vq = c < K && t0 + c < n;
     const int range = luma.bd + 8, crange = luma.bd + 6 > 16 ? luma.bd + 6 : 16;
     int32_t v[64];
-    if (vq) luma_inv_row_load(fmid(q), rr, v, range, nullptr);
+    if (vq) luma_inv_row_load(fmid(c), rr, v, range, nullptr);
     wave_sync();
-    if (vq) luma_inv_row_tx(v, imid(q) + rr * 66, range, crange);
+    if (vq) luma_inv_row_tx(v, imid(c) + rr * 66, range, crange);
     if (prio) __builtin_amdgcn_s_setprio(0);
-  } else if (wave == 2 && late_dist) {
+  } else if (g == 1 && wave == 2 && late_dist) {
     RdoJob j0;
     if constexpr (MODE == 3)
       j0 = rdo_job_intra<Px, 64>(luma, 0, t0);
@@ -1052,7 +1103,7 @@
   }
   __syncthreads();
   if (RV_RDO_PHASES && ph) ph->t[4] = wall_clock64();
-  if (valid) luma_back<Px, int16_t>(luma, luma.p[0], t, jb, true, imid(wave), pred(wave));
+  if (mine) luma_back<Px, int16_t>(luma, luma.p[0], t, jb, true, imid(q), pred(q));
 }
 
 template <typename Px, int MODE>
@@ -1109,9 +1160,12 @@
   rdo_quad_wg<Px, MODE>(luma, chroma, nquads, var, blockIdx.x, lds, scan);
 }
 
+constexpr int kSplitSingle = 2, kSplitComp = 4;
 template <typename Px, int MA, int MB>
 __global__ __launch_bounds__(256) __attribute__((amdgpu_waves_per_eu(4))) void rdo_quad_list_kernel(
-    const RdoArgs *__restrict__ A, int nsets, int var, uint32_t *kp_cnt, unsigned long long *kp_t) {
+    const RdoArgs *__restrict__ A, int nsets, int var, uint32_t *kp_cnt, unsigned long long *kp_t,
+    unsigned long long *items) {
+  constexpr int GA = MA ? kSplitComp : kSplitSingle, GB = MB ? kSplitComp : kSplitSingle;
   __shared__ __align__(16) uint8_t lds[QuadLds<Px>::kBytes];
   __shared__ uint16_t scan[1024];
   if (kp_t && threadIdx.x == 0) atomicMin(kp_t, (unsigned long long)wall_clock64());
@@ -1128,30 +1182,40 @@
   }
   const int pa = (ma + 1) / 2, pb = (mb + 1) / 2;
   const bool c4 = (var & 32) != 0;
-  const int e0 = (na + 3) / 4, e1 = e0 + (c4 ? (2 * ma + 3) / 4 : (2 * pa + 2) / 3);
-  const int e2 = e1 + (nb + 3) / 4, e3 = e2 + (c4 ? (2 * mb + 3) / 4 : (2 * pb + 2) / 3);
+  const int ia = c4 ? (2 * ma + 3) / 4 : (2 * pa + 2) / 3;
+  const int ib = c4 ? (2 * mb + 3) / 4 : (2 * pb + 2) / 3;
+  const int sa = (na * GA + 3) / 4, sb = (nb * GB + 3) / 4;
+  const bool split = c4 && sa + ia + sb + ib <= (int)gridDim.x;
+  var |= split ? 64 : 0;
+  if (items && blockIdx.x == 0 && threadIdx.x == 0) {
+    atomicAdd(items + (split ? 0 : 2) + (MA ? 1 : 0), (unsigned long long)na);
+    if (nsets > 1) atomicAdd(items + (split ? 0 : 2) + (MB ? 1 : 0), (unsigned long long)nb);
+  }
+  const int e0 = split ? sa : (na + 3) / 4, e1 = e0 + ia;
+  const int e2 = e1 + (split ? sb : (nb + 3) / 4), e3 = e2 + ib;
   const bool phd = RV_RDO_PHASES && (var & 16) && rv_tid() == 0;
+  int staged = -1;
   for (int b = blockIdx.x; b < e3; b += gridDim.x) {
     QuadPh ph;
     ph.t[0] = phd ? wall_clock64() : 0;
     QuadPh *pp = phd ? &ph : nullptr;
     int set = 2;
     if (b < e0) {
-      stage_scan(scan, la.q_tx_index);
-      rdo_quad_luma<Px, MA>(la, b, na, var, lds, scan, pp);
-      set = MA;
+      stage_scan(scan, la.q_tx_index, staged);
+      rdo_quad_luma<Px, MA, GA>(la, b, na, var, lds, scan, pp, (var & 64) != 0);
+      set = (var & 64) ? 3 + MA : MA;
     } else if (b < e1) {
-      stage_scan(scan, ca.q_tx_index);
+      stage_scan(scan, ca.q_tx_index, staged);
       if (c4)
         rdo_quad_chroma4<Px, MA>(ca, b - e0, ma, lds, scan);
       else
         rdo_quad_chroma<Px, MA>(ca, b - e0, pa, lds, scan);
     } else if (b < e2) {
-      stage_scan(scan, lb.q_tx_index);
-      rdo_quad_luma<Px, MB>(lb, b - e1, nb, var, lds, scan, pp);
-      set = MB;
+      stage_scan(scan, lb.q_tx_index, staged);
+      rdo_quad_luma<Px, MB, GB>(lb, b - e1, nb, var, lds, scan, pp, (var & 64) != 0);
+      set = (var & 64) ? 3 + MB : MB;
     } else {
-      stage_scan(scan, cb.q_tx_index);
+      stage_scan(scan, cb.q_tx_index, staged);
       if (c4)
         rdo_quad_chroma4<Px, MB>(cb, b - e2, mb, lds, scan);
       else
@@ -1160,9 +1224,10 @@
     __syncthreads();
     if (phd) {
       const unsigned long long te = wall_clock64();
-      if (set < 2) {
+      if (set != 2) {
         for (int k = 0; k < 4; k++) atomicAdd(&g_rdo_ph[set][k], ph.t[k + 1] - ph.t[k]);
         atomicAdd(&g_rdo_ph[set][4], te - ph.t[4]);
+        atomicAdd(&g_rdo_ph[set][6], ph.mc - ph.t[0]);
       } else {
         atomicAdd(&g_rdo_ph[2][0], te - ph.t[0]);
       }
@@ -1322,7 +1387,8 @@
 }
 
 int rv_rdo_candidates_list(const RdoArgs *h, const RdoArgs *dev, int nsets, int mode_a, int hbd,
-                           hipStream_t s, int max_grid, uint32_t *kp_cnt, unsigned long long *kp_t) {
+                           hipStream_t s, int max_grid, uint32_t *kp_cnt, unsigned long long *kp_t,
+                           unsigned long long *items) {
   if (!h || !dev || nsets < 1 || nsets > 2 || mode_a < 0 || mode_a > 1 || (nsets == 2 && mode_a) ||
       h[0].commit || h[0].bd == 12)
     return rv_set_error(RV_EINVAL, "rv_rdo_candidates_list: bad arguments");
@@ -1332,15 +1398,17 @@
   static const bool phases = getenv("RAV1E_HIP_RDO_PHASES") && getenv("RAV1E_HIP_RDO_PHASES")[0] == '1';
   const int var = kRdoVariant | (phases && max_grid > 0 ? 16 : 0) | (max_grid > 0 ? 32 : 0);
   unsigned full = 0;
-  for (int k = 0; k < nsets; k++)
-    full += (unsigned)((h[2 * k].n_tx + 3) / 4) +
+  for (int k = 0; k < nsets; k++) {
+    const int gl = (var & 32) ? (k || mode_a ? kSplitComp : kSplitSingle) : 1;
+    full += (unsigned)((h[2 * k].n_tx * gl + 3) / 4) +
             ((var & 32) ? (unsigned)(2 * h[2 * k + 1].n_tx + 3) / 4
                         : (unsigned)(2 * ((h[2 * k + 1].n_tx + 1) / 2) + 2) / 3);
+  }
   unsigned grid = std::min(full, kF4Pool);
   if (max_grid > 0) grid = std::min(grid, (unsigned)max_grid);
   if (grid == 0) return RV_OK;
 #define RV_LIST(PX, MA, MB) \
-  rdo_quad_list_kernel<PX, MA, MB><<<grid, 256, 0, s>>>(dev, nsets, var, kp_cnt, kp_t)
+  rdo_quad_list_kernel<PX, MA, MB><<<grid, 256, 0, s>>>(dev, nsets, var, kp_cnt, kp_t, items)
   if (hbd) {
     if (nsets == 2) RV_LIST(uint16_t, 0, 1); else if (mode_a) RV_LIST(uint16_t, 1, 1); else RV_LIST(uint16_t, 0, 0);
   } else {
@@ -1390,20 +1458,22 @@
 }
 
 extern "C" int rv_rdo_phase_dump(void) {
-  unsigned long long h[3][8];
+  unsigned long long h[5][8];
   if (hipDeviceSynchronize() != hipSuccess || hipMemcpyFromSymbol(h, HIP_SYMBOL(g_rdo_ph), sizeof(h)) != hipSuccess)
     return rv_set_error(RV_EHIP, "rv_rdo_phase_dump");
   const double us = 0.01;
-  static const char *kName[2] = {"single", "compound"};
-  for (int m = 0; m < 2; m++) {
+  static const char *kName[5] = {"single luma quads", "compound luma quads", "",
+                                 "single luma split items", "compound luma split items"};
+  for (int m = 0; m < 5; m++) {
+    if (m == 2) continue;
     const double n = h[m][5] ? (double)h[m][5] : 1.0;
     fprintf(stderr,
-            "[f4 phases] %s luma quads %llu: front %.2f, row DCT %.2f, quantize %.2f, inverse rows %.2f, "
-            "back %.2f us per quad\n",
-            kName[m], h[m][5], h[m][0] * us / n, h[m][1] * us / n, h[m][2] * us / n, h[m][3] * us / n,
-            h[m][4] * us / n);
-  }
-  fprintf(stderr, "[f4 phases] chroma triples %llu: %.2f us each\n", h[2][5],
+            "[f4 phases] %s %llu: front %.2f (MC %.2f), row DCT %.2f, quantize %.2f, inverse rows %.2f, "
+            "back %.2f us per item\n",
+            kName[m], h[m][5], h[m][0] * us / n, h[m][6] * us / n, h[m][1] * us / n, h[m][2] * us / n,
+            h[m][3] * us / n, h[m][4] * us / n);
+  }
+  fprintf(stderr, "[f4 phases] chroma items %llu: %.2f us each\n", h[2][5],
           h[2][0] * us / (h[2][5] ? (double)h[2][5] : 1.0));
   memset(h, 0, sizeof(h));
   return hipMemcpyToSymbol(HIP_SYMBOL(g_rdo_ph), h, sizeof(h)) == hipSuccess ? RV_OK
diff --git a/rav1e_amd/csrc/rv_replay.h b/rav1e_amd/csrc/rv_replay.h
--- a/rav1e_amd/csrc/rv_replay.h
+++ b/rav1e_amd/csrc/rv_replay.h
@@ -352,6 +352,7 @@
   RdoWinner *win = nullptr;
   int32_t *cand_list = nullptr, *cand_count = nullptr;
   RdoArgs *f4_args = nullptr;
+  unsigned long long *round_items = nullptr;
   CandKey *cand_key = nullptr;
   uint8_t *f3dirty = nullptr;
   uint8_t *f2dirty = nullptr;
diff --git a/rav1e_amd/csrc/rv_replay.hip b/rav1e_amd/csrc/rv_replay.hip
--- a/rav1e_amd/csrc/rv_replay.hip
+++ b/rav1e_amd/csrc/rv_replay.hip
@@ -809,6 +809,7 @@
   r->f2dirty = r->dev<uint8_t>(nsb * g.R * 4);
   r->cand_count = r->dev<int32_t>(2, Fill::Zero);
   r->f4_args = r->dev<RdoArgs>(4);
+  r->round_items = r->dev<unsigned long long>(4, Fill::Zero);
   r->cand_evals = r->dev<uint32_t>((size_t)rv_replay::kRing * 2 * kLevels, Fill::Zero);
   r->l_lev = r->dev<int32_t>(nsb * 1024, Fill::Zero);
   r->c_lev = r->dev<int32_t>(nsb * r->ntx_c * 1024 * 2, Fill::Zero);
@@ -1395,6 +1396,15 @@
   return 21;
 }
 
+int rv_replay_round_items(rv_replay *r, uint64_t out[4]) {
+  if (!r || !out) return rv_set_error(RV_EINVAL, "rv_replay_round_items");
+  RV_H(hipStreamSynchronize(r->stream));
+  unsigned long long h[4];
+  RV_H(hipMemcpy(h, r->round_items, sizeof(h), hipMemcpyDeviceToHost));
+  for (int k = 0; k < 4; k++) out[k] = (uint64_t)h[k];
+  return RV_OK;
+}
+
 int rv_round_ring_slots(uint32_t q, int32_t *out, int cap) {
   if (!out || cap < 6) return rv_set_error(RV_EINVAL, "rv_round_ring_slots: cap");
   static int32_t cnt[2 * RoundRing::kCnt + 1];
diff --git a/rav1e_amd/csrc/rv_replay_frame.hip b/rav1e_amd/csrc/rv_replay_frame.hip
--- a/rav1e_amd/csrc/rv_replay_frame.hip
+++ b/rav1e_amd/csrc/rv_replay_frame.hip
@@ -1060,7 +1060,7 @@
     int f4_grid = 0;
     if (hsb) {
       lg = std::min(hsb * g.R, 512);
-      f4_grid = std::min(6 * hsb, 1024);
+      f4_grid = std::min(9 * hsb, 1024);
     }
     RV_R(kp.open(st));
     RV_R(rv_diamond_f2_f3(&cur.hres, refs_h, r->jobs_half[lv], r->half, ma.f2dirty, &cur.y,
@@ -1075,7 +1075,7 @@
     if (f4_list) {
       RV_R(kp.open(st, 1));
       RV_R(rv_rdo_candidates_list(f4h, r->f4_args, cg.comp ? 2 : 1, 0, g.hbd, st, f4_grid,
-                                  kp.acc(1), kp.ts(1)));
+                                  kp.acc(1), kp.ts(1), r->round_items));
       RV_R(kp.close(st, 1));
     } else {
       RV_R(rv_rdo_candidates(f4h[0], f4h[1], g.hbd, st));
diff --git a/rav1e_amd/replay.py b/rav1e_amd/replay.py
--- a/rav1e_amd/replay.py
+++ b/rav1e_amd/replay.py
@@ -378,6 +378,11 @@
     def counters(self) -> np.ndarray:
         out = np.zeros(21, dtype=np.uint64)
         _check(lib().rv_replay_counters(self.h, out.ctypes.data, 21) - 21, "rv_replay_counters")
+        return out
+
+    def round_items(self) -> np.ndarray:
+        out = np.zeros(4, dtype=np.uint64)
+        _check(lib().rv_replay_round_items(self.h, out.ctypes.data), "rv_replay_round_items")
         return out
 
     def close(self):
```

New measurement: 178.6, median of 2. No clear change (-0.2%).
